# ratt-ru/tricolour

Hardware: AMD Instinct MI355X
Metric: Mvis/s flagged (bl x time x chan x corr) (higher is better)
Workload: dtype f32 data / f64 accumulators / u8 flags; 1 GPU; MeerKAT-64 slab: 252 of 2016 bl x 4 corr x 1024 time x 4096 chan per GPU (BASELINE configs[1] processed as HBM-resident baseline slabs), sum_threshold_flagger kwargs=stage1; params=stage1

## Files before the change

### tricolour_amd/csrc/kernels_boxline.hpp

```cpp
#pragma once

struct BoxDenom { float b, y; };
__device__ __forceinline__ float box_divide(float a, const BoxDenom dn, unsigned long long& okmask) {
    float q = a * dn.y;
    okmask &= __builtin_amdgcn_ballot_w64(__builtin_amdgcn_classf(q, 0x148));
    float r = __builtin_fmaf(-dn.b, q, a);
    q = __builtin_fmaf(r, dn.y, q);
    r = __builtin_fmaf(-dn.b, q, a);
    q = __builtin_fmaf(r, dn.y, q);
    return q;
}
__device__ __forceinline__ float box_divide_ieee(float a, const BoxDenom dn) { return a / dn.b; }
__device__ __forceinline__ float box_divide_checked(float a, const BoxDenom dn) {
    unsigned long long ok = ~0ull;
    const float q = box_divide(a, dn, ok);
    return ((ok >> (threadIdx.x & 63)) & 1ull) ? q : box_divide_ieee(a, dn);
}

template <int KS, typename V, typename A>
struct BoxLine {
    V R1[KS], R2[KS], R3[KS], R4[KS];
    A s1, s2, s3, s4;
    V o1, o2, o3;
    V old1, old2, old3, old4;
    __device__ __forceinline__ void init() {
#pragma unroll
        for (int k = 0; k < KS; k++) { R1[k] = 0; R2[k] = 0; R3[k] = 0; R4[k] = 0; }
        s1 = 0; s2 = 0; s3 = 0; s4 = 0;
        o1 = 0; o2 = 0; o3 = 0;
        old1 = 0; old2 = 0; old3 = 0; old4 = 0;
    }
};

template <int KS, typename V, typename A, bool HASL, bool FAST>
__device__ __forceinline__ float boxline_step(BoxLine<KS, V, A>& L, const int slot, const int m, const V xin,
                                              const int n, const int R2x, V* cell, const V* ncell, const int BT) {
    const V in4 = (FAST || m - 3 >= R2x) ? L.o3 : (V)0;
    const V in3 = L.o2;
    const V in2 = (FAST || m - 1 < n + R2x) ? L.o1 : (V)0;
    const V in1 = xin;
    V t1 = L.R1[slot], t2 = L.R2[slot], t3 = L.R3[slot], t4 = L.R4[slot];
    L.R1[slot] = in1; L.R2[slot] = in2; L.R3[slot] = in3; L.R4[slot] = in4;
    if (HASL) {
        const V n1 = ncell[0], n2 = ncell[BT], n3 = ncell[2 * (size_t)BT], n4 = ncell[3 * (size_t)BT];
        cell[0] = t1; cell[BT] = t2; cell[2 * (size_t)BT] = t3; cell[3 * (size_t)BT] = t4;
        t1 = L.old1; t2 = L.old2; t3 = L.old3; t4 = L.old4;
        L.old1 = n1; L.old2 = n2; L.old3 = n3; L.old4 = n4;
    }
    L.s4 += (A)in4;
    const float out = (float)L.s4;
    L.s4 -= (A)t4;
    L.s3 += (A)in3;
    L.o3 = (V)L.s3;
    L.s3 -= (A)t3;
    L.s2 += (A)in2;
    L.o2 = (V)L.s2;
    L.s2 -= (A)t2;
    L.s1 += (A)in1;
    L.o1 = (V)L.s1;
    L.s1 -= (A)t1;
    return out;
}

#ifndef BOXR_PF_SMALL
#define BOXR_PF_SMALL 16
#endif
#ifndef BOXR_PF_32
#define BOXR_PF_32 16
#endif
#ifndef BOXR_SCHED_EVERY
#define BOXR_SCHED_EVERY 1
#endif
#ifndef BOXR_WAVES_32
#define BOXR_WAVES_32 2
#endif
#ifndef BOXR_WAVES_16
#define BOXR_WAVES_16 3
#endif
#define BOXR_KS_MAX 80
#ifndef BOXR_WAVES_20
#define BOXR_WAVES_20 2
#endif
__host__ __device__ constexpr int boxr_pf(int ks) { return ks >= 64 ? 16 : (ks == 32 ? BOXR_PF_32 : (ks == 20 ? 20 : BOXR_PF_SMALL)); }
__host__ __device__ constexpr int boxr_waves(int ks) { return ks <= 16 ? BOXR_WAVES_16 : (ks == 20 ? BOXR_WAVES_20 : (ks <= 32 ? BOXR_WAVES_32 : 1)); }
#ifndef BOXR_WAVES_F32
#define BOXR_WAVES_F32 2
#endif
#ifndef BOXF_PF_SMALL
#define BOXF_PF_SMALL 16
#endif
__host__ __device__ constexpr int boxr_pf_f(int ks) { return ks <= 16 ? BOXF_PF_SMALL : boxr_pf(ks); }
#ifndef BOXR_WAVES_F16
#define BOXR_WAVES_F16 2
#endif
__host__ __device__ constexpr int boxr_waves_f(int ks) { return ks < 32 ? BOXR_WAVES_F16 : (ks == 32 ? BOXR_WAVES_F32 : 1); }
__host__ __device__ constexpr int boxr_lcm(int a, int b) {
    int x = a, y = b;
    while (y) { int t = x % y; x = y; y = t; }
    return a / x * b;
}

template <int KS, bool HASL, int IMG, bool PACKED, int PF>
__device__ __forceinline__ void boxt_body(const float* __restrict__ srcData, const uint8_t* __restrict__ srcFlags,
                                          float* __restrict__ dstImg, int n, int C, int r, float denom, size_t sws, size_t dws,
                                          const size_t win) {
    extern __shared__ float cf_ring[];
    const int c = blockIdx.x * 64 + threadIdx.x;
    if (c >= C) return;
    constexpr int BT = 64;
    const int R2x = 2 * r;
    const int d = R2x - KS;
    const unsigned rowb = (unsigned)C * 4u;
    const __amdgpu_buffer_rsrc_t drs = __builtin_amdgcn_make_buffer_rsrc(
        (void*)(srcData + win * sws), 0, (int)((unsigned)n * rowb), 0x00020000);
    const __amdgpu_buffer_rsrc_t frs = __builtin_amdgcn_make_buffer_rsrc(
        (void*)(srcFlags + win * sws), 0, PACKED ? (int)((unsigned)(n / 4) * rowb) : (int)((unsigned)n * (unsigned)C), 0x00020000);
    const __amdgpu_buffer_rsrc_t ors = __builtin_amdgcn_make_buffer_rsrc(
        (void*)(dstImg + win * dws), 0, (int)((unsigned)n * rowb), 0x00020000);
    const int coff = c * 4;
    float* ring = cf_ring + threadIdx.x;
    if (HASL)
        for (int k = 0; k < 4 * d; k++) ring[(size_t)k * BT] = 0.0f;
    const int total = n + 4 * r + 3;
    constexpr int UNR = boxr_lcm(KS, PF);
    constexpr bool SPLIT = KS <= 32;

    using V = typename std::conditional<IMG == 0, int, float>::type;
    using A = typename std::conditional<IMG == 0, int, double>::type;
    BoxLine<KS, V, A> L;
    L.init();
    V* cells = reinterpret_cast<V*>(ring);
    constexpr size_t BT4 = (size_t)4 * BT;
    int lslot = 0;
    float pre[PF];
    unsigned prew[PACKED ? PF / 4 : PF];
    auto issue = [&](int t0) {
        if (PACKED) {
#pragma unroll
            for (int q = 0; q < PF / 4; q++) {
                const int t = t0 + 4 * q;
                const unsigned w = (unsigned)__builtin_amdgcn_raw_buffer_load_b32(frs, coff, t < n ? (int)((unsigned)(t >> 2) * rowb) : 0, 0);
                prew[q] = (t < n) ? w : 0x01010101u;
            }
        } else {
#pragma unroll
            for (int u = 0; u < PF; u++) {
                const int t = t0 + u;
                const unsigned w = (unsigned)__builtin_amdgcn_raw_buffer_load_b8(frs, c, t < n ? (int)((unsigned)t * (unsigned)C) : 0, 0);
                prew[PACKED ? 0 : u] = (t < n) ? w : 1u;
            }
        }
        if (IMG == 1) {
#pragma unroll
            for (int u = 0; u < PF; u++)
                pre[u] = __builtin_bit_cast(float, __builtin_amdgcn_raw_buffer_load_b32(drs, coff, t0 + u < n ? (int)((unsigned)(t0 + u) * rowb) : 0, 0));
        }
    };
    auto store = [&](int i, float y) {
        __builtin_amdgcn_raw_buffer_store_b32(__builtin_bit_cast(unsigned, y), ors, coff, (int)((unsigned)i * rowb), 0);
    };
    issue(0);
    for (int mb = 0; mb < total; mb += UNR) {
#pragma unroll
        for (int b = 0; b < UNR / PF; b++) {
            const int m0 = mb + b * PF;
            if (m0 < total) {
                V cur[PF];
#pragma unroll
                for (int u = 0; u < PF; u++) {
                    const bool fl = PACKED ? ((prew[u >> 2] >> (8 * (u & 3))) & 0xFFu) != 0 : prew[PACKED ? 0 : u] != 0;
                    cur[u] = (IMG == 0) ? (fl ? (V)0 : (V)1) : (fl ? (V)0 : (V)pre[u]);
                }
                issue(m0 + PF);
                const bool fast = SPLIT && m0 >= 4 * r + 3 && m0 + PF <= n;
                if (fast) {
#pragma unroll
                    for (int u = 0; u < PF; u++) {
                        V* cell = cells + (size_t)lslot * BT4;
                        if (HASL) lslot = (lslot + 1 == d) ? 0 : lslot + 1;
                        const V* ncell = cells + (size_t)lslot * BT4;
                        const float out = boxline_step<KS, V, A, HASL, true>(L, (b * PF + u) % KS, m0 + u, cur[u], n, R2x, cell, ncell, BT);
                        store(m0 + u - 3 - 4 * r, out / denom);
                        if (BOXR_SCHED_EVERY > 0 && (u % (BOXR_SCHED_EVERY > 0 ? BOXR_SCHED_EVERY : 1)) == (BOXR_SCHED_EVERY > 0 ? BOXR_SCHED_EVERY : 1) - 1) __builtin_amdgcn_sched_barrier(0);
                    }
                } else {
#pragma unroll
                    for (int u = 0; u < PF; u++) {
                        V* cell = cells + (size_t)lslot * BT4;
                        if (HASL) lslot = (lslot + 1 == d) ? 0 : lslot + 1;
                        const V* ncell = cells + (size_t)lslot * BT4;
                        const float out = boxline_step<KS, V, A, HASL, false>(L, (b * PF + u) % KS, m0 + u, cur[u], n, R2x, cell, ncell, BT);
                        const int i = m0 + u - 3 - 4 * r;
                        if (i >= 0 && i < n) store(i, out / denom);
                        if (BOXR_SCHED_EVERY > 0 && (u % (BOXR_SCHED_EVERY > 0 ? BOXR_SCHED_EVERY : 1)) == (BOXR_SCHED_EVERY > 0 ? BOXR_SCHED_EVERY : 1) - 1) __builtin_amdgcn_sched_barrier(0);
                    }
                }
            }
        }
    }
}

template <int KS, bool HASL, int IMG>
__global__ void __launch_bounds__(64, boxr_waves(KS))
k_boxt(const float* __restrict__ srcData, const uint8_t* __restrict__ srcFlags,
       float* __restrict__ dstImg, int n, int C, int r, float denom, size_t sws, size_t dws) {
    boxt_body<KS, HASL, IMG, true, boxr_pf(KS)>(srcData, srcFlags, dstImg, n, C, r, denom, sws, dws, blockIdx.y);
}

__host__ __device__ constexpr int boxt_spec_pf(int ks) { return ks <= 16 ? 64 : (ks == 32 ? 32 : 16); }
template <int KS, bool HASL>
__global__ void __launch_bounds__(64, 1)
k_boxt_spec(const float* __restrict__ srcData, const uint8_t* __restrict__ srcFlags,
            float* __restrict__ dstW, float* __restrict__ dstO, int n, int C, int r, float denom) {
    if (blockIdx.y == 0) boxt_body<KS, HASL, 0, false, boxt_spec_pf(KS)>(srcData, srcFlags, dstW, n, C, r, denom, 0, 0, 0);
    else boxt_body<KS, HASL, 1, false, boxt_spec_pf(KS)>(srcData, srcFlags, dstO, n, C, r, denom, 0, 0, 0);
}

__host__ __device__ constexpr int boxf_ts(int pf) { return pf >= 32 ? 33 : 34; }
#ifndef BOXF_DOUBLE_STAGE
#define BOXF_DOUBLE_STAGE 1
#endif
__host__ __device__ constexpr int boxf_nsub(int ks) { return (BOXF_DOUBLE_STAGE && ks <= 16 && boxr_pf_f(ks) == 16) ? 2 : 1; }
#define BOXF_TS 34
#ifndef BOXF_STREAM_AUX
#define BOXF_STREAM_AUX 0
#endif
__host__ __device__ constexpr bool boxf_panel_ok(int ks, bool hasl) { return ks <= 8 || (ks == 16 && !hasl); }
template <int KS, bool HASL, int MODE, int WPS = boxr_waves_f(KS)>
__global__ void __launch_bounds__(64, WPS)
k_boxf(const float* __restrict__ srcW, unsigned img_gap,
       float* __restrict__ dstW, float* __restrict__ dstO, const float* __restrict__ data,
       int n, int C, int ld, int r, BoxDenom denom, size_t sws_img, size_t dws, size_t ws_data,
       uint8_t* __restrict__ nanflag, float* __restrict__ dstP, size_t pws) {
    extern __shared__ float cf_ring[];
    constexpr int PF = boxr_pf_f(KS);
    static_assert(MODE != 2 || (PF / 2) % 4 == 0, "panel output: groups of four positions per lane");
    constexpr int NSUB = boxf_nsub(KS);
    constexpr int PL = PF * NSUB;
    constexpr int UNR = boxr_lcm(boxr_lcm(KS, PF), PL);
    constexpr int BT = 64;
    constexpr int LPI = 32 / PL;
    constexpr int TS = boxf_ts(PL);
    const int lane = threadIdx.x;
    const int half = lane >> 5;
    const int hl = lane & 31;
    const int c0 = blockIdx.x * 32;
    const int c = c0 + hl;
    const bool colok = c < C;
    const size_t win = blockIdx.y;
    const int R2x = 2 * r;
    const int d = R2x - KS;
    float* ring = cf_ring + lane;
    float* tiles = cf_ring + (size_t)4 * d * BT;
    float* tile = tiles + (size_t)half * PL * TS;
    if (HASL)
        for (int k = 0; k < 4 * d; k++) ring[(size_t)k * BT] = 0.0f;

    const unsigned rowb = (unsigned)C * 4u;
    const __amdgpu_buffer_rsrc_t xrs = __builtin_amdgcn_make_buffer_rsrc(
        (void*)(data + win * ws_data), 0, (int)((unsigned)n * rowb), 0x00020000);
    const __amdgpu_buffer_rsrc_t ors = __builtin_amdgcn_make_buffer_rsrc(
        (void*)(dstO + win * dws), 0, (int)((unsigned)n * rowb), 0x00020000);
    const __amdgpu_buffer_rsrc_t wrs = __builtin_amdgcn_make_buffer_rsrc(
        (void*)(dstW + win * dws), 0, (int)((unsigned)n * rowb), 0x00020000);
    const bool panel = MODE == 2 && boxf_panel_ok(KS, HASL) && dstP != nullptr;
    const __amdgpu_buffer_rsrc_t prs = __builtin_amdgcn_make_buffer_rsrc(
        (void*)(panel ? dstP + win * pws : dstW), 0, panel ? (int)((unsigned)n * rowb) : 0, 0x00020000);

    const int s_pos = hl % PL;
    const int s_line0 = hl / PL;
    const unsigned ldb = (unsigned)ld * 4u;
    const __amdgpu_buffer_rsrc_t srs = __builtin_amdgcn_make_buffer_rsrc(
        (void*)(srcW + win * sws_img), 0, (int)((img_gap + (unsigned)C * (unsigned)ld) * 4u), 0x00020000);
    const int s_off = (int)((unsigned)s_line0 * ldb) + s_pos * 4 + (half ? (int)(img_gap * 4u) : 0);
    float pre[PL];
    auto issue = [&](int t0) {
        const int sbase = (int)((unsigned)c0 * ldb) + t0 * 4;
        if (t0 + PL <= n && c0 + 32 <= C) {
#pragma unroll
            for (int j = 0; j < PL; j++)
                pre[j] = __builtin_bit_cast(float, __builtin_amdgcn_raw_buffer_load_b32(srs, s_off, sbase + (int)((unsigned)(LPI * j) * ldb), 0));
        } else {
            const bool tok = t0 + s_pos < n;
#pragma unroll
            for (int j = 0; j < PL; j++) {
                const bool ok = tok && (c0 + LPI * j + s_line0 < C);
                const float v = __builtin_bit_cast(float, __builtin_amdgcn_raw_buffer_load_b32(srs, ok ? s_off + sbase + (int)((unsigned)(LPI * j) * ldb) : 0, 0, 0));
                pre[j] = ok ? v : 0.0f;
            }
        }
    };
    auto wave_sync = [] {
        __builtin_amdgcn_fence(__ATOMIC_RELEASE, "wavefront");
        __builtin_amdgcn_wave_barrier();
        __builtin_amdgcn_fence(__ATOMIC_ACQUIRE, "wavefront");
    };
    const int hrow = (PF / 2) * half;
    const int hoff = (colok ? c : 0) * 4 + (int)((unsigned)hrow * rowb);
    const float* eb = tiles + (size_t)hrow * TS + hl;
    float dpre[PF / 2];
    auto issue_data = [&](int m0, bool fast) {
        const int i0 = m0 - 3 - 4 * r;
        if (fast) {
#pragma unroll
            for (int k = 0; k < PF / 2; k++)
                dpre[k] = __builtin_bit_cast(float, __builtin_amdgcn_raw_buffer_load_b32(xrs, hoff, (int)((unsigned)(i0 + k) * rowb), BOXF_STREAM_AUX));
        } else {
#pragma unroll
            for (int k = 0; k < PF / 2; k++) {
                const int i = i0 + hrow + k;
                const bool ok = i >= 0 && i < n;
                const float v = __builtin_bit_cast(float, __builtin_amdgcn_raw_buffer_load_b32(xrs, ok ? (colok ? c : 0) * 4 + (int)((unsigned)i * rowb) : 0, 0, 0));
                dpre[k] = ok ? v : 0.0f;
            }
        }
    };

    BoxLine<KS, float, double> L;
    L.init();
    constexpr size_t BT4 = (size_t)4 * BT;
    int lslot = 0;
    const int total = n + 4 * r + 3;
    bool line_nan = false;
    issue(0);
    for (int mb = 0; mb < total; mb += UNR) {
#pragma unroll
        for (int b = 0; b < UNR / PF; b++) {
            const int m0 = mb + b * PF;
            if (m0 < total) {
                const int ro = (b % NSUB) * PF;
                if (b % NSUB == 0) {
                    wave_sync();
#pragma unroll
                    for (int j = 0; j < PL; j++) tile[s_pos * TS + LPI * j + s_line0] = pre[j];
                    wave_sync();
                    issue(m0 + PL);
                }
                const bool fast = m0 >= 4 * r + 3 && m0 + PF <= n;
                issue_data(m0, fast);
                float xin = tile[ro * TS + hl];
                if (fast) {
#pragma unroll
                    for (int u = 0; u < PF; u++) {
                        const float xnext = (u + 1 < PF) ? tile[(ro + u + 1) * TS + hl] : 0.0f;
                        float* cell = ring + (size_t)lslot * BT4;
                        if (HASL) lslot = (lslot + 1 == d) ? 0 : lslot + 1;
                        const float* ncell = ring + (size_t)lslot * BT4;
                        tile[(ro + u) * TS + hl] = boxline_step<KS, float, double, HASL, true>(L, (b * PF + u) % KS, m0 + u, xin, n, R2x, cell, ncell, BT);
                        xin = xnext;
                        if (BOXR_SCHED_EVERY > 0 && u % (BOXR_SCHED_EVERY > 0 ? BOXR_SCHED_EVERY : 1) == 0) __builtin_amdgcn_sched_barrier(0);
                    }
                } else {
#pragma unroll
                    for (int u = 0; u < PF; u++) {
                        const float xnext = (u + 1 < PF) ? tile[(ro + u + 1) * TS + hl] : 0.0f;
                        float* cell = ring + (size_t)lslot * BT4;
                        if (HASL) lslot = (lslot + 1 == d) ? 0 : lslot + 1;
                        const float* ncell = ring + (size_t)lslot * BT4;
                        tile[(ro + u) * TS + hl] = boxline_step<KS, float, double, HASL, false>(L, (b * PF + u) % KS, m0 + u, xin, n, R2x, cell, ncell, BT);
                        xin = xnext;
                        if (BOXR_SCHED_EVERY > 0 && u % (BOXR_SCHED_EVERY > 0 ? BOXR_SCHED_EVERY : 1) == 0) __builtin_amdgcn_sched_barrier(0);
                    }
                }
                if (m0 + PF - 1 - 3 - 4 * r >= 0) {
                    wave_sync();
                    const int i0 = m0 - 3 - 4 * r;
                    unsigned long long okmask = ~0ull, active = 0;
                    float res[MODE == 2 ? PF / 2 : 1];
                    auto finish = [&](auto ieee_tag) {
                        constexpr bool IEEE = decltype(ieee_tag)::value;
#pragma unroll
                        for (int k = 0; k < PF / 2; k++) {
                            const int i = i0 + hrow + k;
                            if ((fast || (i >= 0 && i < n)) && colok) {
                                if (!IEEE) active |= __builtin_amdgcn_ballot_w64(true);
                                const float wv = IEEE ? box_divide_ieee(eb[(ro + k) * TS], denom) : box_divide(eb[(ro + k) * TS], denom, okmask);
                                const float ov = IEEE ? box_divide_ieee(eb[(PL + ro + k) * TS], denom) : box_divide(eb[(PL + ro + k) * TS], denom, okmask);
                                const float bg = (wv == 0.0f) ? NAN : ov / wv;
                                const int vo = fast ? hoff : (c * 4 + (int)((unsigned)i * rowb));
                                const int so = fast ? (int)((unsigned)(i0 + k) * rowb) : 0;
                                if (MODE == 1) {
                                    __builtin_amdgcn_raw_buffer_store_b32(__builtin_bit_cast(unsigned, fabsf(dpre[k] - bg)), ors, vo, so, BOXF_STREAM_AUX);
                                } else {
                                    __builtin_amdgcn_raw_buffer_store_b32(__builtin_bit_cast(unsigned, bg), ors, vo, so, BOXF_STREAM_AUX);
                                    res[MODE == 2 ? k : 0] = dpre[k] - bg;
                                    __builtin_amdgcn_raw_buffer_store_b32(__builtin_bit_cast(unsigned, res[MODE == 2 ? k : 0]), wrs, vo, so, BOXF_STREAM_AUX);
                                    line_nan |= isnan(bg);
                                }
                            }
                            if (BOXR_SCHED_EVERY > 0) __builtin_amdgcn_sched_barrier(0);
                        }
                    };
                    finish(std::false_type{});
                    if ((okmask & active) != active) finish(std::true_type{});
                    if (MODE == 2 && panel && colok) {
                        auto paddr = [&](int i) { return (int)((((unsigned)(i >> 6) * (unsigned)C + (unsigned)c) << 8) + ((unsigned)(i & 63) << 2)); };
#pragma unroll
                        for (int g = 0; g < PF / 8; g++) {
                            const int ig = i0 + hrow + 4 * g;
                            if (fast && (ig & 63) <= 60) {
                                typedef unsigned u4 __attribute__((ext_vector_type(4)));
                                u4 y;
#pragma unroll
                                for (int e = 0; e < 4; e++) y[e] = __builtin_bit_cast(unsigned, res[MODE == 2 ? 4 * g + e : 0]);
                                __builtin_amdgcn_raw_buffer_store_b128(y, prs, paddr(ig), 0, BOXF_STREAM_AUX);
                            } else {
#pragma unroll
                                for (int e = 0; e < 4; e++)
                                    if (fast || (ig + e >= 0 && ig + e < n))
                                        __builtin_amdgcn_raw_buffer_store_b32(__builtin_bit_cast(unsigned, res[MODE == 2 ? 4 * g + e : 0]), prs, paddr(ig + e), 0, BOXF_STREAM_AUX);
                            }
                        }
                    }
                }
            }
        }
    }
    if (MODE == 2 && line_nan && colok) nanflag[win * (size_t)C + c] = 1;
}
```

### tricolour_amd/csrc/kernels_boxpipe.hpp

```cpp
#pragma once
#include <hip/hip_runtime.h>
#include <stdint.h>
#include <type_traits>

__host__ __device__ constexpr int boxp_lc(int r, int B) { return (2 * r + 2 * B + B - 1) / B * B; }
__host__ __device__ constexpr size_t boxp_lds_bytes(int r, int B) {
    return ((size_t)4 * (boxp_lc(r, B) + B) * 64 + (size_t)2 * B * 64) * 4;
}

template <int IMG, int B, int P>
__device__ __forceinline__ void boxp_body(const float* __restrict__ srcData, const uint8_t* __restrict__ srcFlags,
                                          float* __restrict__ dst, const int n, const int C, const int r, const float denom) {
    extern __shared__ float cf_ring[];
    using V = typename std::conditional<IMG == 0, int, float>::type;
    using A = typename std::conditional<IMG == 0, int, double>::type;
    constexpr int K = B / 4;
    static_assert(K == 2 || K == 4, "block length 8 or 16");
    constexpr unsigned OOB = 0x7ffffff0u;
    const int tid = threadIdx.x, lane = tid & 63;
    const int wave = __builtin_amdgcn_readfirstlane(tid >> 6);
    const int R2 = 2 * r;
    const int Lc = boxp_lc(r, B), LcP = Lc + B;
    V* bufs = reinterpret_cast<V*>(cf_ring);
    float* outb = cf_ring + (size_t)4 * LcP * 64;
    for (int k = tid; k < 4 * LcP * 64; k += 256) bufs[k] = 0;
    const int NB = (n + 4 * r + B - 1) / B;

    const int srow = tid / (64 / K);
    const int scol = (tid % (64 / K)) * K;
    const int gcol = blockIdx.x * 64 + scol;
    const bool colok = gcol < C;
    const __amdgpu_buffer_rsrc_t frs = __builtin_amdgcn_make_buffer_rsrc((void*)srcFlags, 0, (int)((unsigned)n * (unsigned)C), 0x00020000);
    const __amdgpu_buffer_rsrc_t ors = __builtin_amdgcn_make_buffer_rsrc((void*)dst, 0, (int)((unsigned)n * (unsigned)C * 4u), 0x00020000);

    unsigned pref[P];
    float prex[IMG == 1 ? P : 1][K];
    auto issue = [&](int blk, int q) {
        const int t = blk * B + srow;
        const unsigned e = (colok && t < n) ? (unsigned)t * (unsigned)C + (unsigned)gcol : OOB;
        if (K == 4) pref[q] = (unsigned)__builtin_amdgcn_raw_buffer_load_b32(frs, (int)e, 0, 0);
        else pref[q] = (unsigned)__builtin_amdgcn_raw_buffer_load_b16(frs, (int)e, 0, 0);
        if (IMG == 1) {
            const float* a = srcData + ((colok && t < n) ? (size_t)e : (size_t)0);
            if (K == 4) {
                const float4 v = *reinterpret_cast<const float4*>(a);
                prex[q][0] = v.x; prex[q][1] = v.y; prex[q][K - 2] = v.z; prex[q][K - 1] = v.w;
            } else {
                const float2 v = *reinterpret_cast<const float2*>(a);
                prex[q][0] = v.x; prex[q][1] = v.y;
            }
        }
    };
    auto staged = [&](int blk, int q, int k) -> V {
        const int t = blk * B + srow;
        const bool fl = t >= n || !colok || ((pref[q] >> (8 * k)) & 0xFFu) != 0;
        if (IMG == 0) return fl ? (V)0 : (V)1;
        return fl ? (V)0 : (V)prex[IMG == 1 ? q : 0][k];
    };
#pragma unroll
    for (int q = 0; q < P; q++) issue(q, q);

    int lpin = 0;
    int pin = 0, pold = Lc - R2;
    A acc = 0;
    V* bin = bufs + (size_t)wave * LcP * 64 + lane;
    V* bout = bufs + (size_t)(wave + 1) * LcP * 64 + lane;
    const int keep_lo = wave == 2 ? R2 : 0;
    const int keep_hi = wave == 0 ? n + R2 : 0x7fffffff;
    __syncthreads();

    for (int j0 = 0; j0 < NB + 5; j0 += P) {
#pragma unroll
        for (int q = 0; q < P; q++) {
            const int j = j0 + q;
            if (j < NB) {
                V* p = bufs + ((size_t)lpin + srow) * 64 + scol;
                V sv[K];
#pragma unroll
                for (int k = 0; k < K; k++) sv[k] = staged(j, q, k);
#pragma unroll
                for (int k = 0; k < K; k++) p[k] = sv[k];
                if (lpin == 0) {
#pragma unroll
                    for (int k = 0; k < K; k++) p[(size_t)Lc * 64 + k] = sv[k];
                }
                lpin = (lpin + B == Lc) ? 0 : lpin + B;
            }
            issue(j + P, q);
            const int b = j - wave - 1;
            if (b >= 0 && b < NB) {
                const V* pi = bin + (size_t)pin * 64;
                const V* po = bin + (size_t)pold * 64;
                V xin[B], xold[B];
#pragma unroll
                for (int u = 0; u < B; u++) { xin[u] = pi[u * 64]; xold[u] = po[u * 64]; }
                const int t0 = b * B;
                if (wave == 3) {
                    float* ob = outb + (size_t)(b & 1) * B * 64 + lane;
#pragma unroll
                    for (int u = 0; u < B; u++) {
                        acc += (A)xin[u];
                        ob[u * 64] = (float)acc;
                        acc -= (A)xold[u];
                    }
                } else {
                    V* po2 = bout + (size_t)pin * 64;
                    const bool whole = t0 >= keep_lo && t0 + B <= keep_hi;
                    V o[B];
#pragma unroll
                    for (int u = 0; u < B; u++) {
                        acc += (A)xin[u];
                        o[u] = (V)acc;
                        acc -= (A)xold[u];
                    }
                    if (whole) {
#pragma unroll
                        for (int u = 0; u < B; u++) po2[u * 64] = o[u];
                    } else {
#pragma unroll
                        for (int u = 0; u < B; u++) {
                            o[u] = (t0 + u >= keep_lo && t0 + u < keep_hi) ? o[u] : (V)0;
                            po2[u * 64] = o[u];
                        }
                    }
                    if (pin == 0) {
#pragma unroll
                        for (int u = 0; u < B; u++) po2[(Lc + u) * 64] = o[u];
                    }
                }
                pin = (pin + B == Lc) ? 0 : pin + B;
                pold = (pold + B >= Lc) ? pold + B - Lc : pold + B;
            }
            {
                const int bs = j - 5;
                const int i = bs * B + srow - 4 * r;
                const bool ok = bs >= 0 && bs < NB && i >= 0 && i < n && colok;
                const float* ob = outb + ((size_t)(bs & 1) * B + srow) * 64 + scol;
                const unsigned eb = ok ? ((unsigned)i * (unsigned)C + (unsigned)gcol) * 4u : OOB;
                if (K == 4) {
                    const float4 v = *reinterpret_cast<const float4*>(ob);
                    typedef unsigned u4 __attribute__((ext_vector_type(4)));
                    u4 y;
                    y[0] = __builtin_bit_cast(unsigned, v.x / denom); y[1] = __builtin_bit_cast(unsigned, v.y / denom);
                    y[2] = __builtin_bit_cast(unsigned, v.z / denom); y[3] = __builtin_bit_cast(unsigned, v.w / denom);
                    __builtin_amdgcn_raw_buffer_store_b128(y, ors, (int)eb, 0, 0);
                } else {
                    const float2 v = *reinterpret_cast<const float2*>(ob);
                    typedef unsigned u2 __attribute__((ext_vector_type(2)));
                    u2 y;
                    y[0] = __builtin_bit_cast(unsigned, v.x / denom); y[1] = __builtin_bit_cast(unsigned, v.y / denom);
                    __builtin_amdgcn_raw_buffer_store_b64(y, ors, (int)eb, 0, 0);
                }
            }
            __syncthreads();
        }
    }
}

template <int B, int P>
__global__ void __launch_bounds__(256, 1)
k_boxp_spec(const float* __restrict__ srcData, const uint8_t* __restrict__ srcFlags,
            float* __restrict__ dstW, float* __restrict__ dstO, int n, int C, int r, float denom) {
    if (blockIdx.y == 0) boxp_body<0, B, P>(srcData, srcFlags, dstW, n, C, r, denom);
    else boxp_body<1, B, P>(srcData, srcFlags, dstO, n, C, r, denom);
}

__host__ __device__ constexpr size_t boxq_lds_bytes(int B, int NF = 3) { return (size_t)(4 * (NF + 1) * B * 64 + 2 * B * 64) * 4; }
#define BOXQ_LDS_BYTES boxq_lds_bytes(16)
__host__ __device__ constexpr int boxq_prefetch(int ks) { return ks == 48 || ks == 96 ? 6 : (ks == 80 ? 5 : 4); }
#ifndef BOXQ_ABLATE
#define BOXQ_ABLATE 0
#endif
__host__ __device__ constexpr int boxq_lcm(int a, int b) {
    int x = a, y = b;
    while (y) { int t = x % y; x = y; y = t; }
    return a / x * b;
}

__host__ __device__ constexpr int boxq_prefetch8(int nblk) {
    return nblk == 6 ? 3 : (nblk == 8 ? 4 : (nblk == 9 ? 3 : (nblk == 10 ? 2 : (nblk == 12 ? 4 : nblk))));
}

template <int IMG, int KS, int P, int B = 16, int NF = 3>
__device__ __forceinline__ void boxq_body(const float* __restrict__ srcData, const uint8_t* __restrict__ srcFlags,
                                          float* __restrict__ dst, const int n, const int C, const int r, const BoxDenom denom,
                                          const size_t sws, const size_t dws, const size_t win) {
    using V = typename std::conditional<IMG == 0, int, float>::type;
    using A = typename std::conditional<IMG == 0, int, double>::type;
    constexpr int PPT = B / 4;
    constexpr int NBLK = KS / B;
    constexpr int U = boxq_lcm(NBLK, P);
    constexpr unsigned OOB = 0x7ffffff0u;
    static_assert(KS % B == 0 && KS >= B, "register part: whole blocks");
    static_assert(B == 8 || B == 16, "block length");
    extern __shared__ float cf_ring[];
    typedef V FifoT[(NF + 1) * B][64];
    typedef float OutT[B][64];
    FifoT* fifo = reinterpret_cast<FifoT*>(cf_ring);
    OutT* outb = reinterpret_cast<OutT*>(cf_ring + 4 * (NF + 1) * B * 64);
    const int tid = threadIdx.x, lane = tid & 63;
    const int wave = __builtin_amdgcn_readfirstlane(tid >> 6);
    const int R2 = 2 * r;
    const int d = R2 - KS;
    const int c = blockIdx.x * 64 + lane;
    const bool colok = c < C;
    const int NB = (n + 4 * r + B - 1) / B;
    const unsigned rowb = (unsigned)C * 4u;
    const __amdgpu_buffer_rsrc_t frs = __builtin_amdgcn_make_buffer_rsrc((void*)(srcFlags + win * sws), 0, (int)((unsigned)(n / 4) * rowb), 0x00020000);
    const __amdgpu_buffer_rsrc_t drs = __builtin_amdgcn_make_buffer_rsrc((void*)(srcData + win * sws), 0, (int)((unsigned)n * rowb), 0x00020000);
    const __amdgpu_buffer_rsrc_t ors = __builtin_amdgcn_make_buffer_rsrc((void*)(dst + win * dws), 0, (int)((unsigned)n * rowb), 0x00020000);
    const unsigned coff = (unsigned)c * 4u;
    for (int k = tid; k < 4 * (NF + 1) * B * 64; k += 256) reinterpret_cast<V*>(cf_ring)[k] = 0;

    unsigned pref[P];
    float prex[IMG == 1 ? P : 1][PPT];
    auto issue = [&](int blk, int q) {
        const int t = blk * B + PPT * wave;
        const bool ok = colok && t < n;
        pref[q] = (unsigned)__builtin_amdgcn_raw_buffer_load_b32(frs, (int)(ok ? (unsigned)(t >> 2) * rowb + coff : OOB), 0, 0);
        if (IMG == 1) {
#pragma unroll
            for (int k = 0; k < PPT; k++)
                prex[q][k] = __builtin_bit_cast(float, __builtin_amdgcn_raw_buffer_load_b32(drs, (int)(ok ? (unsigned)(t + k) * rowb + coff : OOB), 0, 0));
        }
    };
#pragma unroll
    for (int q = 0; q < P; q++) issue(q, q);

    V R[KS];
#pragma unroll
    for (int k = 0; k < KS; k++) R[k] = 0;
    A acc = 0;
    int lslot = 0;
    int slot = 0, s0 = NF * B - d;
    if (s0 >= NF * B) s0 -= NF * B;
    const int keep_lo = wave == 2 ? R2 : 0;
    const int keep_hi = wave == 0 ? n + R2 : 0x7fffffff;
    __syncthreads();

    for (int j0 = 0; j0 < NB + 5; j0 += U) {
#pragma unroll
        for (int qq = 0; qq < U; qq++) {
            const int j = j0 + qq;
            const int q = qq % P;
            const int sb = (qq % NBLK) * B;
#if !(BOXQ_ABLATE & 4)
            {
                const int t = j * B + PPT * wave;
                const bool tin = colok && t < n;
                const unsigned fw = PPT == 4 ? pref[q] : pref[q] >> (16 * (wave & 1));
                V sv[PPT];
#pragma unroll
                for (int k = 0; k < PPT; k++) {
                    const bool fl = !tin || ((fw >> (8 * k)) & 0xFFu) != 0;
                    if (IMG == 0) sv[k] = fl ? (V)0 : (V)1;
                    else sv[k] = fl ? (V)0 : (V)prex[IMG == 1 ? q : 0][k];
                }
                V* p = &fifo[0][lslot * B + PPT * wave][lane];
#pragma unroll
                for (int k = 0; k < PPT; k++) p[k * 64] = sv[k];
                if (lslot == 0) {
#pragma unroll
                    for (int k = 0; k < PPT; k++) p[(NF * B + k) * 64] = sv[k];
                }
                lslot = lslot == NF - 1 ? 0 : lslot + 1;
            }
            issue(j + P, q);
#endif
            const int b = j - wave - 1;
#if !(BOXQ_ABLATE & 2)
            if (b >= 0 && b < NB) {
                const int t0 = b * B;
                const V* pi = &fifo[wave][slot * B][lane];
                const V* pd = &fifo[wave][s0][lane];
                V xin[B], xdel[B], o[B];
#pragma unroll
                for (int u = 0; u < B; u++) { xin[u] = pi[u * 64]; xdel[u] = pd[u * 64]; }
#pragma unroll
                for (int u = 0; u < B; u++) {
                    const V old = R[sb + u];
                    R[sb + u] = xdel[u];
                    acc += (A)xin[u];
                    o[u] = (V)acc;
                    acc -= (A)old;
                }
                if (wave == 3) {
                    float* ob = &outb[b & 1][0][lane];
#pragma unroll
                    for (int u = 0; u < B; u++) ob[u * 64] = (float)o[u];
                } else {
                    const bool whole = t0 >= keep_lo && t0 + B <= keep_hi;
                    V* po = &fifo[wave + 1][slot * B][lane];
                    if (whole) {
#pragma unroll
                        for (int u = 0; u < B; u++) po[u * 64] = o[u];
                    } else {
#pragma unroll
                        for (int u = 0; u < B; u++) {
                            o[u] = (t0 + u >= keep_lo && t0 + u < keep_hi) ? o[u] : (V)0;
                            po[u * 64] = o[u];
                        }
                    }
                    if (slot == 0) {
#pragma unroll
                        for (int u = 0; u < B; u++) po[(NF * B + u) * 64] = o[u];
                    }
                }
                slot = slot == NF - 1 ? 0 : slot + 1;
                s0 = s0 + B >= NF * B ? s0 + B - NF * B : s0 + B;
            }
#endif
#if !(BOXQ_ABLATE & 1)
            {
                const int bs = j - 5;
                const int i0 = bs * B + PPT * wave - 4 * r;
                const float* ob = &outb[bs & 1][PPT * wave][lane];
                float a[PPT], y[PPT];
                unsigned long long okm = ~0ull;
#pragma unroll
                for (int k = 0; k < PPT; k++) { a[k] = ob[k * 64]; y[k] = box_divide(a[k], denom, okm); }
                if (okm != ~0ull) {
                    TRI_KEEP_BRANCH();
#pragma unroll
                    for (int k = 0; k < PPT; k++) y[k] = box_divide_ieee(a[k], denom);
                }
#pragma unroll
                for (int k = 0; k < PPT; k++) {
                    const int i = i0 + k;
                    const bool ok = bs >= 0 && bs < NB && i >= 0 && i < n && colok;
                    __builtin_amdgcn_raw_buffer_store_b32(__builtin_bit_cast(unsigned, y[k]), ors, (int)(ok ? (unsigned)i * rowb + coff : OOB), 0, 0);
                }
            }
#endif
            __syncthreads();
        }
    }
}

template <int KS, int IMG, int B = 16>
__global__ void __launch_bounds__(256, B == 8 ? 4 : 2)
k_boxq(const float* __restrict__ srcData, const uint8_t* __restrict__ srcFlags, float* __restrict__ dstImg,
       int n, int C, int r, BoxDenom denom, size_t sws, size_t dws) {
    boxq_body<IMG, KS, B == 8 ? boxq_prefetch8(KS / 8) : boxq_prefetch(KS), B>(srcData, srcFlags, dstImg, n, C, r, denom, sws, dws, blockIdx.y);
}
template <int KS, int IMG>
__global__ void __launch_bounds__(256, 3)
k_boxq_deep(const float* __restrict__ srcData, const uint8_t* __restrict__ srcFlags, float* __restrict__ dstImg,
            int n, int C, int r, BoxDenom denom, size_t sws, size_t dws) {
    boxq_body<IMG, KS, boxq_prefetch8(KS / 8), 8, 4>(srcData, srcFlags, dstImg, n, C, r, denom, sws, dws, blockIdx.y);
}

#ifndef BOXQF_LW
#define BOXQF_LW 64
#endif
#ifndef BOXQF_DBL
#define BOXQF_DBL 1
#endif
#ifndef BOXQF_PAIR
#define BOXQF_PAIR 1
#endif
#ifndef BOXQF_ABLATE_BARRIER
#define BOXQF_ABLATE_BARRIER 0
#endif
__host__ __device__ constexpr bool boxqf_dbl(int KS, int B) { return BOXQF_DBL && B == 8 && (KS / B) % 2 == 0; }
__host__ __device__ constexpr int boxqf_prefetch2(int nblk) { return nblk == 6 ? 3 : (nblk == 10 || nblk == 2 ? 1 : 2); }
__host__ __device__ constexpr size_t boxqf_lds_floats(int B, bool dbl) { return (size_t)(2 * ((dbl ? 5 : 4) + 3 * 4) * B * BOXQF_LW + 2 * 2 * B * BOXQF_LW); }
__host__ __device__ constexpr size_t boxqf_lds_bytes(int B, bool dbl = false) { return boxqf_lds_floats(B, dbl) * 4; }
#define BOXQF_LDS_BYTES boxqf_lds_bytes(16)
#ifndef BOXQF_P10
#define BOXQF_P10 2
#endif
__host__ __device__ constexpr int boxqf_prefetch8(int nblk) {
    return nblk == 6 ? 3 : (nblk == 8 ? 4 : (nblk == 9 ? 3 : (nblk == 10 ? BOXQF_P10 : (nblk == 12 ? 4 : nblk))));
}
#ifndef BOXQF_MINW8
#define BOXQF_MINW8 4
#endif
template <int KS, int MODE, int B = 16>
__global__ void __launch_bounds__(512, B == 8 ? BOXQF_MINW8 : 1)
k_boxqf(const float* __restrict__ srcW, unsigned img_gap, float* __restrict__ dstW, float* __restrict__ dstO,
        const float* __restrict__ data, int n, int C, int ld, int r, BoxDenom denom, size_t sws_img, size_t dws,
        size_t ws_data, uint8_t* __restrict__ nanflag) {
    constexpr int PP = B / 4;
    constexpr int FN = B / 8;
    constexpr int NBLK = KS / B;
    constexpr bool DBL = boxqf_dbl(KS, B);
    constexpr int P2 = boxqf_prefetch2(NBLK);
    constexpr int P = DBL ? 2 * P2 : (B == 8 ? boxqf_prefetch8(NBLK) : boxq_prefetch(KS));
    static_assert(KS % B == 0, "register part: whole blocks");
    static_assert(B == 8 || B == 16, "block length");
    constexpr int U = boxq_lcm(NBLK, P);
    static_assert(!DBL || U % 2 == 0, "double-block staging: an even number of iterations per trip");
    constexpr unsigned OOB = 0x7ffffff0u;
    extern __shared__ float cf_ring[];
    constexpr int LW = BOXQF_LW;
    constexpr int NF1 = DBL ? 4 : 3;
    constexpr int F1 = (NF1 + 1) * B * LW, FN3 = 4 * B * LW;
    typedef float OutT[B][LW];
    auto fifo_of = [&](int image, int stage) -> float* {
        return stage == 0 ? cf_ring + image * F1 : cf_ring + 2 * F1 + (image * 3 + stage - 1) * FN3;
    };
    OutT* outb = reinterpret_cast<OutT*>(cf_ring + 2 * F1 + 6 * FN3);
    constexpr bool PAIR = BOXQF_PAIR && B == 8 && KS <= 40;
    auto ld2 = [&](const float* fifo, int row) -> float2 {
        if (PAIR) return *reinterpret_cast<const float2*>(fifo + ((size_t)(row >> 1) * LW + (threadIdx.x & 63)) * 2);
        const float* p = fifo + (size_t)row * LW + (threadIdx.x & 63);
        return make_float2(p[0], p[LW]);
    };
    auto st2 = [&](float* fifo, int row, int line, float a, float b2) {
        if (PAIR) { *reinterpret_cast<float2*>(fifo + ((size_t)(row >> 1) * LW + line) * 2) = make_float2(a, b2); return; }
        float* p = fifo + (size_t)row * LW + line;
        p[0] = a;
        p[LW] = b2;
    };
    const int tid = threadIdx.x, lane = tid & 63;
    const int wave = __builtin_amdgcn_readfirstlane(tid >> 6);
    const int img = wave >> 2, st = wave & 3;
    const size_t win = blockIdx.y;
    const int c0 = blockIdx.x * 64;
    const int R2 = 2 * r;
    const int d = R2 - KS;
    const int NB = (n + 4 * r + B - 1) / B;
    for (int k = tid; k < 2 * F1 + 6 * FN3; k += 512) cf_ring[k] = 0.0f;

    const int s_line = (tid & 255) >> 2, s_q = tid & 3;
    const bool s_lok = c0 + s_line < C;
    const float* s_base = srcW + win * sws_img + (size_t)(img ? img_gap : 0u) + (size_t)(s_lok ? c0 + s_line : 0) * ld;
    float pre[DBL ? P2 : P][DBL ? 4 : PP];
    auto issue = [&](int blk, int q) {
        if (DBL) {
            const int p = blk * 16 + 4 * s_q;
            const float4 v = *reinterpret_cast<const float4*>(s_base + (p < n ? p : 0));
            pre[q][0] = v.x; pre[q][1] = v.y; pre[q][DBL ? 2 : 0] = v.z; pre[q][DBL ? 3 : 0] = v.w;
            return;
        }
        const int p = blk * B + PP * s_q;
        if (PP == 4) {
            const float4 v = *reinterpret_cast<const float4*>(s_base + (p < n ? p : 0));
            pre[q][0] = v.x; pre[q][1] = v.y; pre[q][PP - 2] = v.z; pre[q][PP - 1] = v.w;
        } else {
            const float2 v = *reinterpret_cast<const float2*>(s_base + (p < n ? p : 0));
            pre[q][0] = v.x; pre[q][1] = v.y;
        }
    };
    const int f_u = tid >> 6;
    const int c = c0 + lane;
    const bool colok = c < C;
    const unsigned rowb = (unsigned)C * 4u;
    const unsigned coff = (unsigned)c * 4u;
    const __amdgpu_buffer_rsrc_t xrs = __builtin_amdgcn_make_buffer_rsrc((void*)(data + win * ws_data), 0, (int)((unsigned)n * rowb), 0x00020000);
    const __amdgpu_buffer_rsrc_t ors = __builtin_amdgcn_make_buffer_rsrc((void*)(dstO + win * dws), 0, (int)((unsigned)n * rowb), 0x00020000);
    const __amdgpu_buffer_rsrc_t wrs = __builtin_amdgcn_make_buffer_rsrc((void*)(dstW + win * dws), 0, (int)((unsigned)n * rowb), 0x00020000);
    float dpre[P][FN];
    auto issue_data = [&](int blk, int q) {
#pragma unroll
        for (int h = 0; h < FN; h++) {
            const int i = blk * B + f_u + 8 * h - 4 * r;
            const bool ok = blk >= 0 && i >= 0 && i < n && colok;
            dpre[q][h] = __builtin_bit_cast(float, __builtin_amdgcn_raw_buffer_load_b32(xrs, (int)(ok ? (unsigned)i * rowb + coff : OOB), 0, 0));
        }
    };
#pragma unroll
    for (int q = 0; q < P; q++) { if (!DBL || q < P2) issue(q, q); issue_data(q - 5, q); }

    float R[KS];
#pragma unroll
    for (int k = 0; k < KS; k++) R[k] = 0.0f;
    double acc = 0.0;
    int lslot = 0;
    const int nf = st == 0 ? NF1 : 3;
    int slot = (nf * 8 - st - 1) % nf, s0 = (nf * B * 8 - (st + 1) * B - d) % (nf * B);
    int oslot = (3 * 8 - st - 1) % 3;
    float* const fin = fifo_of(img, st);
    float* const fout = fifo_of(img, st < 3 ? st + 1 : 3);
    const int keep_lo = st == 2 ? R2 : 0;
    const int keep_hi = st == 0 ? n + R2 : 0x7fffffff;
    bool line_nan = false;
    __syncthreads();

    for (int j0 = 0; j0 < NB + 5; j0 += U) {
#pragma unroll
        for (int qq = 0; qq < U; qq++) {
            const int j = j0 + qq;
            const int q = qq % P;
            const int sb = (qq % NBLK) * B;
            if (DBL) {
                if (qq % 2 == 0) {
                    const int q2 = (qq / 2) % P2;
                    const int p = j * B + 4 * s_q;
                    const bool ok = s_lok && p < n;
                    float* pf = fifo_of(img, 0);
                    const int r0 = lslot * B + 4 * s_q;
                    const float v0 = ok ? pre[q2][0] : 0.0f, v1 = ok ? pre[q2][1] : 0.0f, v2 = ok ? pre[q2][DBL ? 2 : 0] : 0.0f, v3 = ok ? pre[q2][DBL ? 3 : 0] : 0.0f;
                    st2(pf, r0, s_line, v0, v1);
                    st2(pf, r0 + 2, s_line, v2, v3);
                    if (lslot == 0 && s_q < 2) {
                        st2(pf, NF1 * B + r0, s_line, v0, v1);
                        st2(pf, NF1 * B + r0 + 2, s_line, v2, v3);
                    }
                    lslot = lslot == 0 ? 2 : 0;
                    issue(j / 2 + P2, q2);
                }
            } else {
                const int p = j * B + PP * s_q;
                const bool ok = s_lok && p < n;
                float* pf = fifo_of(img, 0);
                const int r0 = lslot * B + PP * s_q;
#pragma unroll
                for (int k = 0; k < PP; k += 2) {
                    const float va = ok ? pre[DBL ? 0 : q][k] : 0.0f, vb = ok ? pre[DBL ? 0 : q][k + 1] : 0.0f;
                    st2(pf, r0 + k, s_line, va, vb);
                    if (lslot == 0) st2(pf, 3 * B + r0 + k, s_line, va, vb);
                }
                lslot = lslot == 2 ? 0 : lslot + 1;
            }
            if (!DBL) issue(j + P, q);
            const int b = j - st - 1;
            {
                const int t0 = b * B;
                float xin[B], xdel[B], o[B];
#pragma unroll
                for (int u = 0; u < B; u += 2) {
                    const float2 a = ld2(fin, slot * B + u), d2 = ld2(fin, s0 + u);
                    xin[u] = a.x; xin[u + 1] = a.y; xdel[u] = d2.x; xdel[u + 1] = d2.y;
                }
#pragma unroll
                for (int u = 0; u < B; u++) {
                    const float old = R[sb + u];
                    R[sb + u] = xdel[u];
                    acc += (double)xin[u];
                    o[u] = (float)acc;
                    acc -= (double)old;
                }
                if (st == 3) {
                    float* ob = &outb[img * 2 + (b & 1)][0][lane];
#pragma unroll
                    for (int u = 0; u < B; u++) ob[u * LW] = o[u];
                } else {
                    const bool whole = t0 >= keep_lo && t0 + B <= keep_hi && b >= 0;
                    if (!whole) {
#pragma unroll
                        for (int u = 0; u < B; u++) o[u] = (t0 + u >= keep_lo && t0 + u < keep_hi) ? o[u] : 0.0f;
                    }
#pragma unroll
                    for (int u = 0; u < B; u += 2) st2(fout, oslot * B + u, lane, o[u], o[u + 1]);
                    if (oslot == 0) {
#pragma unroll
                        for (int u = 0; u < B; u += 2) st2(fout, 3 * B + u, lane, o[u], o[u + 1]);
                    }
                }
                slot = slot == nf - 1 ? 0 : slot + 1;
                oslot = oslot == 2 ? 0 : oslot + 1;
                s0 = s0 + B >= nf * B ? s0 + B - nf * B : s0 + B;
            }
            {
                const int bs = j - 5;
                float wq[FN], oq[FN], a0[FN], a1[FN];
                unsigned long long okm = ~0ull;
#pragma unroll
                for (int h = 0; h < FN; h++) {
                    a0[h] = outb[bs & 1][f_u + 8 * h][lane];
                    a1[h] = outb[2 + (bs & 1)][f_u + 8 * h][lane];
                    wq[h] = box_divide(a0[h], denom, okm);
                    oq[h] = box_divide(a1[h], denom, okm);
                }
                if (okm != ~0ull) {
                    TRI_KEEP_BRANCH();
#pragma unroll
                    for (int h = 0; h < FN; h++) { wq[h] = box_divide_ieee(a0[h], denom); oq[h] = box_divide_ieee(a1[h], denom); }
                }
#pragma unroll
                for (int h = 0; h < FN; h++) {
                    const int i = bs * B + f_u + 8 * h - 4 * r;
                    const bool ok = bs >= 0 && bs < NB && i >= 0 && i < n && colok;
                    const unsigned off = ok ? (unsigned)i * rowb + coff : OOB;
                    const float bg = (wq[h] == 0.0f) ? NAN : oq[h] / wq[h];
                    const float dv = dpre[q][h];
                    if (MODE == 1) {
                        __builtin_amdgcn_raw_buffer_store_b32(__builtin_bit_cast(unsigned, fabsf(dv - bg)), ors, (int)off, 0, 0);
                    } else {
                        __builtin_amdgcn_raw_buffer_store_b32(__builtin_bit_cast(unsigned, bg), ors, (int)off, 0, 0);
                        __builtin_amdgcn_raw_buffer_store_b32(__builtin_bit_cast(unsigned, dv - bg), wrs, (int)off, 0, 0);
                        line_nan |= ok && isnan(bg);
                    }
                }
            }
            issue_data(j + P - 5, q);
#if BOXQF_ABLATE_BARRIER
            asm volatile("" ::: "memory");
            __builtin_amdgcn_sched_barrier(0);
#else
            __syncthreads();
#endif
        }
    }
    if (MODE == 2 && line_nan) nanflag[win * (size_t)C + c] = 1;
}
```

### tricolour_amd/csrc/kernels_boxweight.hpp

```cpp
#pragma once
#include <type_traits>

__host__ __device__ constexpr int boxw_unroll(int r2) { return r2 % 4 == 0 ? r2 : 2 * r2; }
__host__ __device__ constexpr int boxw_regs(int r2) { return (r2 + 31) / 32 + (r2 + 3) / 4 + (r2 + 1) / 2 + r2 + 56; }
__host__ __device__ constexpr int boxw_waves(int r2) { return boxw_regs(r2) <= 128 ? 4 : (boxw_regs(r2) <= 168 ? 3 : 2); }
#ifndef BOXW_SCHED_EVERY
#define BOXW_SCHED_EVERY 2
#endif
#ifndef BOXW_PREFETCH
#define BOXW_PREFETCH 4
#endif

__device__ __forceinline__ float boxw_divide(float a, const BoxDenom dn) {
    float q = a * dn.y;
    float r = __builtin_fmaf(-dn.b, q, a);
    q = __builtin_fmaf(r, dn.y, q);
    r = __builtin_fmaf(-dn.b, q, a);
    q = __builtin_fmaf(r, dn.y, q);
    return q;
}

#define BOXW_LSHL_ADD(acc, x, SH) asm("v_lshl_add_u32 %0, %1, %2, %0" : "+v"(acc) : "v"(x), "n"(SH))

template <int R2>
__global__ void __launch_bounds__(64, boxw_waves(R2))
k_boxw(const uint8_t* __restrict__ srcFlags, float* __restrict__ dstW, int n, int C, BoxDenom denom, size_t sws, size_t dws) {
    constexpr int N1 = (R2 + 31) / 32, N2 = (R2 + 3) / 4, N3 = (R2 + 1) / 2;
    constexpr int P = BOXW_PREFETCH;
    constexpr unsigned OOB = 0x7ffffff0u;
    static_assert(R2 % 2 == 0 && R2 >= 8 && R2 <= 214, "2r even, stage sums within a byte / a halfword / int32");
    const int lane = threadIdx.x;
    const size_t win = blockIdx.y;
    const int c = blockIdx.x * 64 + lane;
    const bool colok = c < C;
    const unsigned rowb = (unsigned)C * 4u;
    const unsigned coff = colok ? (unsigned)c * 4u : OOB;
    const __amdgpu_buffer_rsrc_t frs = __builtin_amdgcn_make_buffer_rsrc((void*)(srcFlags + win * sws), 0, (int)((unsigned)(n / 4) * rowb), 0x00020000);
    const __amdgpu_buffer_rsrc_t ors = __builtin_amdgcn_make_buffer_rsrc((void*)(dstW + win * dws), 0, (int)((unsigned)n * rowb), 0x00020000);

    unsigned D1[N1], D2[N2], D3[N3], D4[R2];
#pragma unroll
    for (int k = 0; k < N1; k++) D1[k] = 0;
#pragma unroll
    for (int k = 0; k < N2; k++) D2[k] = 0;
#pragma unroll
    for (int k = 0; k < N3; k++) D3[k] = 0;
#pragma unroll
    for (int k = 0; k < R2; k++) D4[k] = 0;
    unsigned s1 = 0, s2 = 0, s3 = 0, s4 = 0;

    unsigned pf[P];
    const int ngrp = n / 4;
#pragma unroll
    for (int q = 0; q < P; q++)
        pf[q] = (unsigned)__builtin_amdgcn_raw_buffer_load_b32(frs, (int)((colok && q < ngrp) ? (unsigned)q * rowb + coff : OOB), 0, 0);

    const int nsteps = n + 2 * R2;
    unsigned wb = 0;
    auto block = [&](auto phase, const int t0, const unsigned head) {
        constexpr int PH = decltype(phase)::value;
#pragma unroll
        for (int u = 0; u < R2; u++) {
            const int t = t0 + u;
            const int slot = u;
            if ((u + PH) % 4 == 0) {
                const unsigned fw = pf[0];
#pragma unroll
                for (int q = 0; q + 1 < P; q++) pf[q] = pf[q + 1];
                const int g = (t >> 2) + P;
                pf[P - 1] = (unsigned)__builtin_amdgcn_raw_buffer_load_b32(frs, (int)(g < ngrp ? (unsigned)g * rowb + coff : OOB), 0, 0);
                const unsigned nz = ((((fw & 0x7f7f7f7fu) + 0x7f7f7f7fu) | fw) >> 7) & 0x01010101u;
                wb = t < n ? (nz ^ 0x01010101u) : 0u;
            }
            const unsigned in1 = (wb >> (8 * ((u + PH) % 4))) & 1u;
            const unsigned old1 = (D1[slot >> 5] >> (slot & 31)) & 1u;
            const unsigned o1 = s1 + in1;
            const unsigned d1 = in1 - old1;
            s1 = o1 - old1;
            BOXW_LSHL_ADD(D1[slot >> 5], d1, slot & 31);
            const unsigned old2 = (D2[slot >> 2] >> (8 * (slot & 3))) & 0xffu;
            const unsigned o2 = s2 + o1;
            s2 = o2 - old2;
            const unsigned d2 = o1 - old2;
            BOXW_LSHL_ADD(D2[slot >> 2], d2, 8 * (slot & 3));
            const unsigned old3 = (D3[slot >> 1] >> (16 * (slot & 1))) & 0xffffu;
            const unsigned o3 = s3 + o2;
            s3 = o3 - old3;
            const unsigned d3 = o2 - old3;
            BOXW_LSHL_ADD(D3[slot >> 1], d3, 16 * (slot & 1));
            const unsigned in4 = o3 & head;
            const unsigned old4 = D4[slot];
            D4[slot] = in4;
            const unsigned o4 = s4 + in4;
            s4 = o4 - old4;
            const int i = t - 2 * R2;
            const bool rowok = (unsigned)i < (unsigned)n;
            const float y = boxw_divide((float)o4, denom);
            __builtin_amdgcn_raw_buffer_store_b32(__builtin_bit_cast(unsigned, y), ors, (int)(rowok ? coff : OOB), (int)(rowok ? (unsigned)i * rowb : 0u), 0);
            if (BOXW_SCHED_EVERY > 0 && (u + 1) % BOXW_SCHED_EVERY == 0) __builtin_amdgcn_sched_barrier(0);
        }
    };
    for (int t0 = 0; t0 < nsteps; t0 += boxw_unroll(R2)) {
        block(std::integral_constant<int, 0>{}, t0, t0 == 0 ? 0u : ~0u);
        if constexpr (R2 % 4 != 0) block(std::integral_constant<int, 2>{}, t0 + R2, ~0u);
    }
}
```

### tricolour_amd/csrc/tricolour_amd.hip

```cpp
#include <unordered_set>
#include "tri_common.hpp"
#include "kernels_elementwise.hpp"
#include "kernels_median.hpp"
#include "kernels_reject.hpp"
#include "kernels_reject_tile.hpp"
#include "kernels_boxfilter.hpp"
#include "kernels_boxline.hpp"
#include "kernels_boxpipe.hpp"
#include "kernels_boxweight.hpp"
#include "kernels_boxexact.hpp"
#include "kernels_sumthreshold.hpp"
#include "kernels_scan.hpp"
#include "kernels_sir.hpp"
#include "kernels_linerms.hpp"

namespace {

static hipError_t lds_optin(const void* fn, hipFuncAttribute attr, int value) {
    thread_local std::unordered_set<uint64_t> done;
    int dev = 0;
    hipError_t e = hipGetDevice(&dev);
    if (e != hipSuccess) return e;
    const uint64_t key = (uint64_t)(uintptr_t)fn * 64u + (uint64_t)(dev & 63);
    if (done.count(key)) return hipSuccess;
// ... 184 lines not shown
    ws->colcnt = b.get<int>(W * F);
    ws->nanmask = b.get<uint16_t>(W * N / 16 + 8);
    ws->itab = b.get<int>(3 * W * (size_t)cdiv(Fa, INTERP_SEG) * std::max<size_t>(T, 1));
    ws->med = b.get<double>(W * std::max(Fa, T * G));
    size_t PS = (size_t)pl.PF;
    ws->sdata = b.get<float>(Fa * W);
    ws->sw = b.get<float>(PS * W);
    ws->so = b.get<float>(PS * W);
    ws->sres = b.get<float>(Fa * W);
    ws->sflags = b.get<uint8_t>(Fa * W);
    ws->sbgf = b.get<uint8_t>(Fa * W);
    ws->sout = b.get<uint8_t>(Fa * W);
    ws->srows = b.get<uint8_t>(Fa * W);
    ws->srowsf = b.get<float>(Fa * W);
    ws->srowsu = b.get<uint8_t>(Fa * W);
    ws->smed = b.get<double>(W * G);
    size_t thrT = W * Fa, thrF = W * T * G;
    size_t ringn = std::max(thrT * (size_t)pl.swT.ringtot, thrF * (size_t)pl.swF.ringtot);
    size_t accn = std::max(thrT * (size_t)pl.swT.acccap, thrF * (size_t)pl.swF.acccap);
    ws->ring = b.get<double>(ringn);
    ws->acc = b.get<uint8_t>(accn);
    ws->total = b.off;
}

static inline dim3 grid1(size_t n, size_t W) { return dim3((unsigned)cdiv((int64_t)n, 256), (unsigned)W, 1); }

}

__global__ void k_tables(ChunkTab ct, int T, int Fa, int64_t* chunk_ends, int64_t* tends,
                         int64_t* segC_start, int64_t* segC_len, int64_t* segB_start,
                         int64_t* segB_len, int64_t* segT_start, int64_t* segT_len,
                         int* chunk_of) {
    int i = blockIdx.x * blockDim.x + threadIdx.x;
    int G = ct.n - 1;
    if (i <= G) chunk_ends[i] = ct.ends[i];
    if (i < G) {
        segC_start[i] = ct.ends[i];
        segC_len[i] = ct.ends[i + 1] - ct.ends[i];
        segB_start[i] = ct.ends[i] * T;
        segB_len[i] = (ct.ends[i + 1] - ct.ends[i]) * T;
    }
    if (i == 0) { tends[0] = 0; tends[1] = T; segT_start[0] = 0; segT_len[0] = T; }
    if (i < Fa) {
        int g = 0;
        while (g < G - 1 && !(i >= ct.ends[g] && i < ct.ends[g + 1])) g++;
        chunk_of[i] = g;
    }
}

__global__ void k_gather_col_f32(const float* __restrict__ a, float* __restrict__ out, int L, int C, int col) {
    int i = blockIdx.x * blockDim.x + threadIdx.x;
    if (i < L) out[i] = a[(size_t)i * C + col];
}
__global__ void k_gather_col_u8(const uint8_t* __restrict__ a, uint8_t* __restrict__ out, int L, int C, int col) {
    int i = blockIdx.x * blockDim.x + threadIdx.x;
    if (i < L) out[i] = a[(size_t)i * C + col];
}
__global__ void k_normalise_flags(const uint8_t* __restrict__ a, uint8_t* __restrict__ b, size_t n) {
    size_t i = (size_t)blockIdx.x * blockDim.x + threadIdx.x;
    if (i < n) b[i] = a[i] ? 1 : 0;
}

extern "C" size_t tri_workspace_bytes(int64_t batch_windows, int64_t ntime, int64_t nchan,
                                      const tri_params* p) {
    Plan pl;
    if (!p || batch_windows <= 0 || make_plan(ntime, nchan, p, &pl) != TRI_OK) return 0;
    Ws ws;
    carve(pl, batch_windows, nullptr, 0, true, &ws);
    return ws.total;
}

extern "C" int tri_prepare_params(int64_t ntime, int64_t nchan, double outlier_nsigma,
                                  const double* windows_time, int64_t n_windows_time,
                                  const double* windows_freq, int64_t n_windows_freq,
                                  double background_reject, int64_t background_iterations,
                                  double spike_width_time, double spike_width_freq,
                                  int64_t time_extend, int64_t freq_extend, int64_t freq_chunks,
                                  int64_t average_freq, double flag_all_time_frac,
                                  double flag_all_freq_frac, double rho,
                                  int64_t num_major_iterations, int64_t* chunk_ends_buf,
                                  int64_t chunk_cap, tri_params* out) {
    if (!out || !chunk_ends_buf) return set_err(TRI_EINVAL, "NULL output");
    if (ntime <= 0 || nchan <= 0) return set_err(TRI_EINVAL, "empty window");
    if (average_freq < 1) return set_err(TRI_EINVAL, "average_freq must be >= 1");
    if (freq_chunks < 1) return set_err(TRI_EINVAL, "freq_chunks must be >= 1");
    if (chunk_cap < freq_chunks + 1) return set_err(TRI_EINVAL, "chunk_ends_buf too small");
    if (n_windows_time > TRI_MAX_WINDOWS || n_windows_freq > TRI_MAX_WINDOWS || n_windows_time < 0 || n_windows_freq < 0)
        return set_err(TRI_EINVAL, "at most %d windows per axis", TRI_MAX_WINDOWS);
    memset(out, 0, sizeof(*out));
    int64_t fa = (nchan + average_freq - 1) / average_freq;
    std::vector<int64_t> wf;
    for (int64_t i = 0; i < n_windows_freq; i++) {
        float v = std::ceil((float)windows_freq[i]) / (float)average_freq;
        wf.push_back((int64_t)v);
    }
    std::sort(wf.begin(), wf.end());
    wf.erase(std::unique(wf.begin(), wf.end()), wf.end());
    double step = (double)fa / (double)freq_chunks;
    for (int64_t i = 0; i <= freq_chunks; i++) chunk_ends_buf[i] = (int64_t)((double)i * step);
    chunk_ends_buf[freq_chunks] = fa;
    out->n_windows_time = 0;
    for (int64_t i = 0; i < n_windows_time; i++)
        if (windows_time[i] <= (double)ntime) out->windows_time[out->n_windows_time++] = (int64_t)windows_time[i];
    out->n_windows_freq = 0;
    for (size_t i = 0; i < wf.size(); i++)
        if (wf[i] <= fa) out->windows_freq[out->n_windows_freq++] = wf[i];
    for (int64_t i = 0; i < out->n_windows_freq; i++)
        if (out->windows_freq[i] <= 0)
            return set_err(TRI_EINVAL, "windows_freq / average_freq produced a window of size %lld; the reference fails here (operands could not be broadcast together, flagging.py:663)", (long long)out->windows_freq[i]);
    for (int64_t i = 0; i < out->n_windows_time; i++)
        if (out->windows_time[i] <= 0) return set_err(TRI_EINVAL, "windows_time must be positive");
    out->outlier_nsigma = outlier_nsigma;
    out->background_reject = background_reject;
    out->background_iterations = background_iterations;
    out->spike_width_time = spike_width_time;
    out->spike_width_freq = spike_width_freq;
    out->time_extend = time_extend;
    out->freq_extend = freq_extend;
    out->n_chunk_ends = freq_chunks + 1;
    out->chunk_ends = chunk_ends_buf;
    out->average_freq = average_freq;
    out->flag_all_time_frac = flag_all_time_frac;
    out->flag_all_freq_frac = flag_all_freq_frac;
    out->rho = rho;
    out->num_major_iterations = num_major_iterations;
    return TRI_OK;
}

namespace {

struct Debug {
    float* f32;
    uint8_t* u8;
};

struct Run {
    hipStream_t st;
    Plan pl;
    Ws ws;
    const tri_params* p;
    int64_t Wb;
    Debug* dbg;
    bool ampl_cached = false;
    const uint8_t* data_mask = nullptr;
    size_t data_mask_ws = 0;
};

bool st_use_fused(const StWin& sw) {
    static const bool force_generic = is1(getenv("TRI_ST_GENERIC"));
    if (force_generic) return false;
    return sw.nw == 4 && sw.w[0] == 1 && sw.w[1] == 2 && sw.w[2] == 4 && sw.w[3] == 8;
}

bool st_use_mask(int L, int C) {
    static const bool force_register = is1(getenv("TRI_ST_REGISTER"));
    return !force_register && (uint64_t)L * (uint64_t)C * 4u < (1ull << 31);
}

static bool median_no_predict() { static const bool v = is1(getenv("TRI_MEDIAN_NO_PREDICT")); return v; }

static bool median_takes_extra_flags(int64_t max_len) { return max_len <= 64 * MW_K; }

struct MedianJob {
    const float* data = nullptr; const uint8_t* flags = nullptr; double* med = nullptr;
    size_t WSd = 0, WSf = 0, RS = 0, ES = 1;
    const int64_t* seg_start = nullptr; const int64_t* seg_len = nullptr;
    int R = 0, G = 0;
    int64_t W = 0, max_len = 0;
    bool vec_ok = false;
    bool rows_aligned = false;
    bool segs_aligned = false;
    const uint8_t* flags2 = nullptr; const uint8_t* colflags = nullptr; size_t WScol = 0; int panel_rows = 0;
    unsigned* gcand = nullptr; size_t cand_ws = 0; unsigned cand_cap = 0;
};

enum class MedianKernel {
    Wave8, Wave8Vec,
    Wave16, Wave16Vec,
    Select, SelectVec,
    TwoPass, TwoPassVec,
    TwoPassVecLong,
};

template <int KS, bool VEC, int SPW>
static void median_wave(hipStream_t st, const MedianJob& j) {
    hipLaunchKernelGGL((k_median_wave<KS, VEC, SPW>), dim3((unsigned)cdiv((int64_t)cdiv((int64_t)j.R, SPW) * j.G, 4), (unsigned)j.W),
                       dim3(256), 0, st, j.data, j.flags, j.med, j.WSd, j.WSf, j.RS, j.ES, j.seg_start, j.seg_len, j.R, j.G,
                       j.flags2, j.colflags, j.WScol, j.panel_rows);
}
template <bool VEC>
static void median_select(hipStream_t st, const MedianJob& j) {
    hipLaunchKernelGGL(k_median<VEC>, dim3((unsigned)(j.R * j.G), (unsigned)j.W), dim3(256), 0, st,
                       j.data, j.flags, j.med, j.WSd, j.WSf, j.RS, j.ES, j.seg_start, j.seg_len, j.R, j.G);
}
template <bool VEC, int UNR = MED2_UNROLL>
static void median_two_pass(hipStream_t st, const MedianJob& j) {
    hipLaunchKernelGGL((k_median2<VEC, false, UNR>), dim3((unsigned)(j.R * j.G), (unsigned)j.W), dim3(256), 0, st,
                       j.data, j.flags, j.med, j.WSd, j.WSf, j.RS, j.ES, j.seg_start, j.seg_len, j.R, j.G, j.gcand, j.cand_ws, j.cand_cap);
}

static void launch_median_kernel(hipStream_t st, MedianKernel k, bool seg_per_wave, const MedianJob& j) {
    switch (k) {
    case MedianKernel::Wave8: seg_per_wave ? median_wave<8, false, 1>(st, j) : median_wave<8, false, MW_SPW>(st, j); break;
    case MedianKernel::Wave8Vec: seg_per_wave ? median_wave<8, true, 1>(st, j) : median_wave<8, true, MW_SPW>(st, j); break;
    case MedianKernel::Wave16: seg_per_wave ? median_wave<MW_K, false, 1>(st, j) : median_wave<MW_K, false, MW_SPW16>(st, j); break;
    case MedianKernel::Wave16Vec: seg_per_wave ? median_wave<MW_K, true, 1>(st, j) : median_wave<MW_K, true, MW_SPW16>(st, j); break;
    case MedianKernel::Select: median_select<false>(st, j); break;
    case MedianKernel::SelectVec: median_select<true>(st, j); break;
    case MedianKernel::TwoPass: median_two_pass<false>(st, j); break;
    case MedianKernel::TwoPassVec: median_two_pass<true>(st, j); break;
    case MedianKernel::TwoPassVecLong: median_two_pass<true, 16>(st, j); break;
    }
}

int launch_median(const Run& r, MedianJob j) {
    const int R = j.R, G = j.G;
    const int64_t W = j.W, max_len = j.max_len;
    if ((int64_t)R * G <= 0 || W <= 0) return TRI_OK;
    if (j.panel_rows > 0 && !(j.ES == 1 && j.RS % 64 == 0 && j.rows_aligned && max_len + (j.segs_aligned ? 0 : 3) <= 64 * MW_K &&
                              j.WSd % 4 == 0 && j.WSf % 4 == 0 && ((uintptr_t)j.data % 16 == 0) && ((uintptr_t)j.flags % 4 == 0)))
        return set_err(TRI_EUNSUPPORTED, "panel images need wave-sized segments of 64-column aligned rows");
    if ((j.flags2 || j.colflags) && (max_len > 64 * MW_K || (j.colflags && j.ES != 1) || ((uintptr_t)j.flags2 % 4 != 0) ||
                                     ((uintptr_t)j.colflags % 4 != 0) || j.WScol % 4 != 0))
        return set_err(TRI_EUNSUPPORTED, "extra flag sources need wave-sized segments of contiguous, 4-byte aligned rows");
    if ((int64_t)R * G > 0x7FFFFFFF || W > 65535) return set_err(TRI_EUNSUPPORTED, "median grid too large");
    const bool row4 = j.ES == 1 && j.RS % 4 == 0 && j.WSd % 4 == 0 && j.WSf % 4 == 0 &&
                      ((uintptr_t)j.data % 16 == 0) && ((uintptr_t)j.flags % 4 == 0) && j.rows_aligned &&
                      (uint64_t)j.RS * (uint64_t)std::max(R, j.panel_rows) * 4u < (1ull << 32);
    if (j.panel_rows > 0 && !row4) return set_err(TRI_EUNSUPPORTED, "panel images of 4 GB or more per window");
    const int64_t slack = j.segs_aligned ? 0 : 3;
    static const bool wave_old = is1(getenv("TRI_MEDIAN_WAVE_OLD"));
    MedianKernel k;
    if (max_len + slack <= 64 * 8 && row4) k = MedianKernel::Wave8Vec;
    else if (max_len <= 64 * 8 && j.panel_rows == 0) k = MedianKernel::Wave8;
    else if (max_len + slack <= 64 * MW_K && row4) k = MedianKernel::Wave16Vec;
    else if (max_len <= 64 * MW_K) k = MedianKernel::Wave16;
    else {
        static const bool three = is1(getenv("TRI_MEDIAN_3PASS"));
        if (three) k = j.vec_ok ? MedianKernel::SelectVec : MedianKernel::Select;
        else {
            if (median_no_predict() || j.cand_cap < max_len || j.cand_ws % 4 != 0 || j.cand_cap % 4 != 0 || ((uintptr_t)j.gcand % 16 != 0)) {
                j.gcand = nullptr; j.cand_ws = 0; j.cand_cap = 0;
            }
            if ((j.vec_ok || row4) && (int64_t)R * G * W < 1536 && max_len >= (int64_t)1 << 20) k = MedianKernel::TwoPassVecLong;
            else k = (j.vec_ok || row4) ? MedianKernel::TwoPassVec : MedianKernel::TwoPass;
        }
    }
    launch_median_kernel(r.st, k, wave_old, j);
    LAUNCHCHK();
    return TRI_OK;
}

#ifndef LDS_R_MAX
#define LDS_R_MAX 15
#endif
#ifndef LANE4_R_MAX
#define LANE4_R_MAX 160
#endif
static bool filter_no_lane4() { static const bool v = is1(getenv("TRI_FILTER_NO_LANE4")); return v; }
int colfilter_lds_block(int rad, int C) {
    static const bool disabled = is1(getenv("TRI_FILTER_MULTIPASS"));
    if (disabled || rad <= 0) return 0;
    if (filter_no_lane4()) {
        int bt = rad <= 10 ? 256 : (rad <= 20 ? 128 : (rad <= 40 ? 64 : 0));
        while (bt > 64 && bt / 2 >= C) bt /= 2;
        return bt;
    }
    if (rad <= LDS_R_MAX) {
        int bt = rad <= 10 ? 256 : 128;
        while (bt > 64 && bt / 2 >= C) bt /= 2;
        return bt;
    }
    return rad <= LANE4_R_MAX ? 64 : 0;
}
inline bool colfilter_use_lane4(int rad) { return !filter_no_lane4() && rad > LDS_R_MAX && rad <= LANE4_R_MAX; }

#ifndef BOXR_MAX_LDS_SLOTS
#define BOXR_MAX_LDS_SLOTS 60
#endif
thread_local int g_boxr_override = -1;
int boxr_pick_ks(int rad) {
    static const bool env_off = is1(getenv("TRI_FILTER_NO_REGRING"));
    const bool off = g_boxr_override >= 0 ? g_boxr_override == 0 : env_off;
    if (off || rad < 4 || rad > 107) return 0;
    const int ks = 2 * rad >= 80 ? 80 : (2 * rad >= 64 ? 64 : (2 * rad >= 32 ? 32 : (2 * rad >= 16 ? 16 : 8)));
    return 2 * rad - ks <= BOXR_MAX_LDS_SLOTS ? ks : 0;
}

#ifndef BOXT_MIN_2R
#define BOXT_MIN_2R 32
#endif
#ifndef BOXT_EXACT20
#define BOXT_EXACT20 1
#endif
int boxr_pick_ks_t(int rad) {
    if (BOXT_EXACT20 && 2 * rad == 20) return boxr_pick_ks(rad) > 0 ? 20 : 0;
    return 2 * rad >= BOXT_MIN_2R ? boxr_pick_ks(rad) : 0;
}
int boxr_pick_ks_f(int rad) {
    static const bool off = is1(getenv("TRI_FILTER_NO_REGRING_F"));
    return off ? 0 : boxr_pick_ks(rad);
}

thread_local int g_boxw_override = -1;
static bool boxw_usable(int rad, int n, int C) {
    static const bool off = is1(getenv("TRI_FILTER_NO_BOXW"));
    if (g_boxw_override == 0 || (off && g_boxw_override < 0)) return false;
    return 2 * rad >= 20 && 2 * rad <= 110 && n % 4 == 0 && (uint64_t)n * (uint64_t)C * 4u < (1ull << 31);
}
template <int R2>
int launch_boxw_r2(const Run& r, const uint8_t* srcFlags, float* dstW, int n, int C, float denom, size_t sws, size_t dws, int64_t W) {
    dim3 grid((unsigned)cdiv(C, 64), (unsigned)W);
    hipLaunchKernelGGL((k_boxw<R2>), grid, dim3(64), 0, r.st, srcFlags, dstW, n, C, box_reciprocal(denom), sws, dws);
    LAUNCHCHK();
    return TRI_OK;
}
int launch_boxw(const Run& r, const uint8_t* srcFlags, float* dstW, int n, int C, int rad, float denom, size_t sws, size_t dws, int64_t W) {
#define BOXW_CASE(R2) case R2: return launch_boxw_r2<R2>(r, srcFlags, dstW, n, C, denom, sws, dws, W);
#define BOXW_CASE5(A) BOXW_CASE(A) BOXW_CASE(A + 2) BOXW_CASE(A + 4) BOXW_CASE(A + 6) BOXW_CASE(A + 8)
    switch (2 * rad) {
        BOXW_CASE5(20) BOXW_CASE5(30) BOXW_CASE5(40) BOXW_CASE5(50) BOXW_CASE5(60) BOXW_CASE5(70) BOXW_CASE5(80) BOXW_CASE5(90) BOXW_CASE5(100)
        BOXW_CASE(110)
    }
#undef BOXW_CASE5
#undef BOXW_CASE
    return set_err(TRI_EINVAL, "no integer weight filter for radius %d", rad);
}

template <int KS>
int launch_boxt_ks(const Run& r, const float* srcData, const uint8_t* srcFlags, float* dstW, float* dstO,
                   int n, int C, int rad, float denom, size_t sws, size_t dws, int64_t W) {
    const int d = 2 * rad - KS;
    const size_t lds = (size_t)4 * d * 64 * sizeof(float);
    dim3 grid((unsigned)cdiv(C, 64), (unsigned)W);
    HIPCHK(lds_optin_all(160 * 1024, &k_boxt<KS, true, 0>, &k_boxt<KS, true, 1>));
    const bool wk = boxw_usable(rad, n, C);
    if (wk) { const int rc = launch_boxw(r, srcFlags, dstW, n, C, rad, denom, sws, dws, W); if (rc) return rc; }
    if (d > 0) {
        if (!wk) hipLaunchKernelGGL((k_boxt<KS, true, 0>), grid, dim3(64), lds, r.st, srcData, srcFlags, dstW, n, C, rad, denom, sws, dws);
        hipLaunchKernelGGL((k_boxt<KS, true, 1>), grid, dim3(64), lds, r.st, srcData, srcFlags, dstO, n, C, rad, denom, sws, dws);
    } else {
        if (!wk) hipLaunchKernelGGL((k_boxt<KS, false, 0>), grid, dim3(64), 0, r.st, srcData, srcFlags, dstW, n, C, rad, denom, sws, dws);
        hipLaunchKernelGGL((k_boxt<KS, false, 1>), grid, dim3(64), 0, r.st, srcData, srcFlags, dstO, n, C, rad, denom, sws, dws);
    }
    LAUNCHCHK();
    return TRI_OK;
}

template <int KS>
int launch_boxt_spec_ks(const Run& r, const float* srcData, const uint8_t* srcFlags, float* dstW, float* dstO,
                        int n, int C, int rad, float denom) {
    const int d = 2 * rad - KS;
    const size_t lds = (size_t)4 * d * 64 * sizeof(float);
    dim3 grid((unsigned)cdiv(C, 64), 2);
    HIPCHK(lds_optin_all(160 * 1024, &k_boxt_spec<KS, true>));
    if (d > 0) hipLaunchKernelGGL((k_boxt_spec<KS, true>), grid, dim3(64), lds, r.st, srcData, srcFlags, dstW, dstO, n, C, rad, denom);
    else hipLaunchKernelGGL((k_boxt_spec<KS, false>), grid, dim3(64), 0, r.st, srcData, srcFlags, dstW, dstO, n, C, rad, denom);
    LAUNCHCHK();
    return TRI_OK;
}

int launch_boxt_spec(const Run& r, int ks, const float* srcData, const uint8_t* srcFlags, float* dstW, float* dstO,
                     int n, int C, int rad, float denom) {
    switch (ks) {
        case 8: return launch_boxt_spec_ks<8>(r, srcData, srcFlags, dstW, dstO, n, C, rad, denom);
        case 16: return launch_boxt_spec_ks<16>(r, srcData, srcFlags, dstW, dstO, n, C, rad, denom);
        case 32: return launch_boxt_spec_ks<32>(r, srcData, srcFlags, dstW, dstO, n, C, rad, denom);
        case 64: return launch_boxt_spec_ks<64>(r, srcData, srcFlags, dstW, dstO, n, C, rad, denom);
        case 80: return launch_boxt_spec_ks<80>(r, srcData, srcFlags, dstW, dstO, n, C, rad, denom);
    }
    return set_err(TRI_EINVAL, "no register-ring kernel for %d slots", ks);
}

static thread_local int g_boxp_override = -1;
static int boxp_pick_block(int rad, int C) {
    static const bool off = is1(getenv("TRI_SPEC_NO_PIPE"));
    if (g_boxp_override == 0 || (off && g_boxp_override < 0)) return 0;
    if (g_boxp_override != 8 && 2 * rad >= 16 && C % 4 == 0 && boxp_lds_bytes(rad, 16) <= 160 * 1024) return 16;
    if (g_boxp_override == 16) return 0;
    if (2 * rad >= 8 && C % 2 == 0 && boxp_lds_bytes(rad, 8) <= 160 * 1024) return 8;
    return 0;
}

template <int B, int P>
int launch_boxp_spec_b(const Run& r, const float* srcData, const uint8_t* srcFlags, float* dstW, float* dstO,
                       int n, int C, int rad, float denom) {
    HIPCHK(lds_optin_all(160 * 1024, &k_boxp_spec<B, P>));
    dim3 grid((unsigned)cdiv(C, 64), 2);
    hipLaunchKernelGGL((k_boxp_spec<B, P>), grid, dim3(256), boxp_lds_bytes(rad, B), r.st, srcData, srcFlags, dstW, dstO, n, C, rad, denom);
    LAUNCHCHK();
    return TRI_OK;
}

#ifndef BOXQ_MIN_2R
#define BOXQ_MIN_2R 56
#endif
thread_local int g_boxq_override = -1;
static int boxq_pick_ks(int rad) {
    static const bool off = is1(getenv("TRI_FILTER_NO_PIPE_T"));
    if (g_boxq_override == 0 || (off && g_boxq_override < 0)) return 0;
    const int ks = 2 * rad / 16 * 16;
    return (ks >= 16 && ks <= 96) ? ks : 0;
}

template <int KS, int B = 16>
int launch_boxq_ks(const Run& r, const float* srcData, const uint8_t* srcFlags, float* dstW, float* dstO,
                   int n, int C, int rad, float denom, size_t sws, size_t dws, int64_t W) {
    HIPCHK(lds_optin_all(160 * 1024, &k_boxq<KS, 0, B>, &k_boxq<KS, 1, B>));
    dim3 grid((unsigned)cdiv(C, 64), (unsigned)W);
    const BoxDenom dn = box_reciprocal(denom);
    if (boxw_usable(rad, n, C)) { const int rc = launch_boxw(r, srcFlags, dstW, n, C, rad, denom, sws, dws, W); if (rc) return rc; }
    else hipLaunchKernelGGL((k_boxq<KS, 0, B>), grid, dim3(256), boxq_lds_bytes(B), r.st, srcData, srcFlags, dstW, n, C, rad, dn, sws, dws);
    hipLaunchKernelGGL((k_boxq<KS, 1, B>), grid, dim3(256), boxq_lds_bytes(B), r.st, srcData, srcFlags, dstO, n, C, rad, dn, sws, dws);
    LAUNCHCHK();
    return TRI_OK;
}

#ifndef BOXQ_B8_MIN_2R
#define BOXQ_B8_MIN_2R 32
#endif
#ifndef BOXQ_B8_MAX2R
#define BOXQ_B8_MAX2R 88
#endif
thread_local int g_boxq_b8_override = -1;
static int boxq_pick_ks8(int rad) {
    static const int b8 = [] { const char* e = getenv("TRI_FILTER_PIPE_T_B8"); return e ? atoi(e) : 1; }();
    if (!b8 || g_boxq_b8_override == 0 || 2 * rad < BOXQ_B8_MIN_2R || 2 * rad >= BOXQ_B8_MAX2R) return 0;
    return 2 * rad / 8 * 8;
}

template <int KS>
int launch_boxq_deep(const Run& r, const float* srcData, const uint8_t* srcFlags, float* dstW, float* dstO,
                     int n, int C, int rad, float denom, size_t sws, size_t dws, int64_t W) {
    HIPCHK(lds_optin_all(160 * 1024, &k_boxq_deep<KS, 0>, &k_boxq_deep<KS, 1>));
    dim3 grid((unsigned)cdiv(C, 64), (unsigned)W);
    const BoxDenom dn = box_reciprocal(denom);
    if (boxw_usable(rad, n, C)) { const int rc = launch_boxw(r, srcFlags, dstW, n, C, rad, denom, sws, dws, W); if (rc) return rc; }
    else hipLaunchKernelGGL((k_boxq_deep<KS, 0>), grid, dim3(256), boxq_lds_bytes(8, 4), r.st, srcData, srcFlags, dstW, n, C, rad, dn, sws, dws);
    hipLaunchKernelGGL((k_boxq_deep<KS, 1>), grid, dim3(256), boxq_lds_bytes(8, 4), r.st, srcData, srcFlags, dstO, n, C, rad, dn, sws, dws);
    LAUNCHCHK();
    return TRI_OK;
}
#ifndef BOXQ_DEEP
#define BOXQ_DEEP 1
#endif

int launch_boxq(const Run& r, int ks, const float* srcData, const uint8_t* srcFlags, float* dstW, float* dstO,
                int n, int C, int rad, float denom, size_t sws, size_t dws, int64_t W) {
    if (BOXQ_DEEP && boxq_pick_ks8(40) > 0) {
        if (2 * rad >= 88 && 2 * rad < 96) return launch_boxq_deep<80>(r, srcData, srcFlags, dstW, dstO, n, C, rad, denom, sws, dws, W);
        if (2 * rad >= 104 && 2 * rad < 112) return launch_boxq_deep<96>(r, srcData, srcFlags, dstW, dstO, n, C, rad, denom, sws, dws, W);
    }
    switch (boxq_pick_ks8(rad)) {
        case 32: return launch_boxq_ks<32, 8>(r, srcData, srcFlags, dstW, dstO, n, C, rad, denom, sws, dws, W);
        case 40: return launch_boxq_ks<40, 8>(r, srcData, srcFlags, dstW, dstO, n, C, rad, denom, sws, dws, W);
        case 48: return launch_boxq_ks<48, 8>(r, srcData, srcFlags, dstW, dstO, n, C, rad, denom, sws, dws, W);
        case 56: return launch_boxq_ks<56, 8>(r, srcData, srcFlags, dstW, dstO, n, C, rad, denom, sws, dws, W);
        case 64: return launch_boxq_ks<64, 8>(r, srcData, srcFlags, dstW, dstO, n, C, rad, denom, sws, dws, W);
        case 80: return launch_boxq_ks<80, 8>(r, srcData, srcFlags, dstW, dstO, n, C, rad, denom, sws, dws, W);
    }
    switch (ks) {
        case 16: return launch_boxq_ks<16>(r, srcData, srcFlags, dstW, dstO, n, C, rad, denom, sws, dws, W);
        case 32: return launch_boxq_ks<32>(r, srcData, srcFlags, dstW, dstO, n, C, rad, denom, sws, dws, W);
        case 48: return launch_boxq_ks<48>(r, srcData, srcFlags, dstW, dstO, n, C, rad, denom, sws, dws, W);
        case 64: return launch_boxq_ks<64>(r, srcData, srcFlags, dstW, dstO, n, C, rad, denom, sws, dws, W);
        case 80: return launch_boxq_ks<80>(r, srcData, srcFlags, dstW, dstO, n, C, rad, denom, sws, dws, W);
        case 96: return launch_boxq_ks<96>(r, srcData, srcFlags, dstW, dstO, n, C, rad, denom, sws, dws, W);
    }
    return set_err(TRI_EINVAL, "no stage-pipeline kernel for %d slots", ks);
}

int launch_boxt(const Run& r, int ks, const float* srcData, const uint8_t* srcFlags, float* dstW, float* dstO,
                int n, int C, int rad, float denom, size_t sws, size_t dws, int64_t W) {
    switch (ks) {
        case 16: return launch_boxt_ks<16>(r, srcData, srcFlags, dstW, dstO, n, C, rad, denom, sws, dws, W);
        case 20: return launch_boxt_ks<20>(r, srcData, srcFlags, dstW, dstO, n, C, rad, denom, sws, dws, W);
        case 32: return launch_boxt_ks<32>(r, srcData, srcFlags, dstW, dstO, n, C, rad, denom, sws, dws, W);
        case 64: return launch_boxt_ks<64>(r, srcData, srcFlags, dstW, dstO, n, C, rad, denom, sws, dws, W);
        case 80: return launch_boxt_ks<80>(r, srcData, srcFlags, dstW, dstO, n, C, rad, denom, sws, dws, W);
    }
    return set_err(TRI_EINVAL, "no register-ring kernel for %d slots", ks);
}

enum class ColSrc {
    ByteFlags,
    Images,
    PackedFlags
};
enum ColFlag : unsigned {
    COL_TRANSPOSED_OUT = 1,
    COL_WEIGHTS_01 = 2
};
enum class ColFamily { SpecPipe, SpecRing, StagePipe, RegRing, Lane4, LdsRing, MultiPass };
thread_local bool g_colfilter_unpadded = false;

int launch_colfilter(const Run& r, ColSrc src, float* bufW, float* bufO, const float* srcData,
                     const uint8_t* srcFlags, float* dstW, float* dstO, int n, int C, int rad,
                     size_t bws, size_t sws, size_t dws, int64_t W, unsigned flags = 0, float* deferred_denom = nullptr) {
    const bool transposed_out = flags & COL_TRANSPOSED_OUT, weights_are_01 = flags & COL_WEIGHTS_01;
    const float denom = box_denominator(rad);
    const int intw = (weights_are_01 && rad <= 31) ? 1 : 0;
    int bt = colfilter_lds_block(rad, C);
    if (deferred_denom) *deferred_denom = 0.0f;
    const bool regs_ok = !deferred_denom && !transposed_out && weights_are_01 && (uint64_t)n * (uint64_t)C * 4u < (1ull << 31);
    const bool spectrum = regs_ok && src == ColSrc::ByteFlags && W == 1;
    const bool packed = regs_ok && src == ColSrc::PackedFlags && n % 4 == 0;
    ColFamily fam;
    if (spectrum && boxp_pick_block(rad, C) > 0 && rad <= 107 && ((uintptr_t)srcData % 16 == 0) && ((uintptr_t)srcFlags % 4 == 0) &&
        ((uintptr_t)dstW % 16 == 0) && ((uintptr_t)dstO % 16 == 0))
        fam = ColFamily::SpecPipe;
    else if (spectrum && boxr_pick_ks(rad) > 0) fam = ColFamily::SpecRing;
    else if (packed && boxq_pick_ks(rad) > 0 && rad <= 107 && (g_boxq_override == 1 || 2 * rad >= BOXQ_MIN_2R)) fam = ColFamily::StagePipe;
    else if (packed && boxr_pick_ks_t(rad) > 0) fam = ColFamily::RegRing;
    else if (bt > 0 && colfilter_use_lane4(rad) && !transposed_out && src != ColSrc::ByteFlags) fam = ColFamily::Lane4;
    else {
        if (bt > 0 && colfilter_use_lane4(rad) && src == ColSrc::ByteFlags) {
            bt = rad <= 20 ? 128 : (rad <= 40 ? 64 : 0);
            while (bt > 64 && bt / 2 >= C) bt /= 2;
        }
        fam = bt > 0 ? ColFamily::LdsRing : ColFamily::MultiPass;
    }
    if (fam == ColFamily::MultiPass && g_colfilter_unpadded)
        return set_err(TRI_EUNSUPPORTED, "radius %d takes the in-place multi-pass filter, which needs images padded to n + 4r rows", rad);
    const bool built = src != ColSrc::Images, divide = !deferred_denom;
    const float *const inW = built ? nullptr : bufW, *const inO = built ? nullptr : bufO;
    const size_t in_ws = built ? 0 : bws;
    switch (fam) {
        case ColFamily::SpecPipe:
            if (boxp_pick_block(rad, C) == 16) return launch_boxp_spec_b<16, 16>(r, srcData, srcFlags, dstW, dstO, n, C, rad, denom);
            return launch_boxp_spec_b<8, 16>(r, srcData, srcFlags, dstW, dstO, n, C, rad, denom);
        case ColFamily::SpecRing:
            return launch_boxt_spec(r, boxr_pick_ks(rad), srcData, srcFlags, dstW, dstO, n, C, rad, denom);
        case ColFamily::StagePipe:
            return launch_boxq(r, boxq_pick_ks(rad), srcData, srcFlags, dstW, dstO, n, C, rad, denom, sws, dws, W);
        case ColFamily::RegRing:
            return launch_boxt(r, boxr_pick_ks_t(rad), srcData, srcFlags, dstW, dstO, n, C, rad, denom, sws, dws, W);
        case ColFamily::Lane4: {
            HIPCHK(lds_optin_all(160 * 1024, &k_colfilter_lane4<0, true>, &k_colfilter_lane4<1, true>, &k_colfilter_lane4<1, false>,
                                 &k_colfilter_lane4<2, false>, &k_colfilter_lane4<2, true>));
            const auto k = src == ColSrc::PackedFlags ? (divide ? &k_colfilter_lane4<2, true> : &k_colfilter_lane4<2, false>)
                                                      : (divide ? &k_colfilter_lane4<1, true> : &k_colfilter_lane4<1, false>);
            if (!divide) *deferred_denom = denom;
            hipLaunchKernelGGL(k, dim3((unsigned)cdiv(C, 16), (unsigned)W, 2), dim3(64), (size_t)lane4_ring_capacity(rad) * 64 * sizeof(float), r.st,
                               inW, inO, srcData, srcFlags, dstW, dstO, n, C, rad, denom, in_ws, sws, dws);
            break;
        }
        case ColFamily::LdsRing: {
            HIPCHK(lds_optin_all(160 * 1024, &k_colfilter_lds<0, true, false>, &k_colfilter_lds<1, true, false>, &k_colfilter_lds<1, false, false>,
                                 &k_colfilter_lds<1, true, true>, &k_colfilter_lds<2, false, false>, &k_colfilter_lds<2, true, false>));
            auto k = &k_colfilter_lds<0, true, false>;
            bool div = true;
            if (src == ColSrc::PackedFlags) { div = divide; k = div ? &k_colfilter_lds<2, true, false> : &k_colfilter_lds<2, false, false>; }
            else if (transposed_out) k = &k_colfilter_lds<1, true, true>;
            else if (src == ColSrc::Images) { div = divide; k = div ? &k_colfilter_lds<1, true, false> : &k_colfilter_lds<1, false, false>; }
            if (!div) *deferred_denom = denom;
            hipLaunchKernelGGL(k, dim3((unsigned)cdiv(C, bt), (unsigned)W, 2), dim3(bt), (size_t)4 * 2 * rad * bt * sizeof(float), r.st,
                               inW, inO, srcData, srcFlags, dstW, dstO, n, C, rad, denom, in_ws, sws, dws, intw);
            break;
        }
        case ColFamily::MultiPass: {
            const int blk = C >= 256 ? 256 : (C >= 128 ? 128 : 64);
            const auto k = src == ColSrc::ByteFlags ? &k_colfilter<0> : &k_colfilter<1>;
            hipLaunchKernelGGL(k, dim3((unsigned)cdiv(C, blk), (unsigned)W, 2), dim3(blk), 0, r.st, bufW, bufO, srcData, srcFlags,
                               dstW, dstO, n, C, rad, denom, bws, sws, dws);
            break;
        }
    }
    LAUNCHCHK();
    return TRI_OK;
}

bool st_use_pipe(const StWin& sw) {
    static const bool off = is1(getenv("TRI_ST_NO_PIPE"));
    return !off && sw.nw >= 1 && sw.nw <= 8 && stp_lds_bytes(sw) <= 160 * 1024;
}

enum class StKernel { Dyn, Fused, Mask, MaskPanel, Pipe };

int st_launch(hipStream_t st, StKernel k, const StWin& sw, const float* data, const double* med, uint8_t* out,
              const int64_t* d_chunk_ends, double thr_scale, int L, int C, int G, size_t ws_data, size_t ws_out, int64_t W,
              double* ring, uint8_t* acc) {
    int blk = C >= 256 ? 256 : (C >= 128 ? 128 : 64);
    if (const char* e = getenv("TRI_ST_BLK")) { int b = atoi(e); if (b >= 64 && b <= ST_MAXBLK && C >= b) blk = b; }
    const dim3 grid((unsigned)cdiv(C, blk), (unsigned)G, (unsigned)W);
    StFusedArgs fa;
    for (int j = 0; j < 4; j++) fa.tf[j] = sw.tf[j < sw.nw ? j : 0];
    if (k == StKernel::MaskPanel)
        hipLaunchKernelGGL((k_colst_mask<1, 2, 4, 8, true>), grid, dim3(blk), 0, st, data, med, out, d_chunk_ends, fa, thr_scale, L, C, G, ws_data, ws_out);
    else if (k == StKernel::Mask)
        hipLaunchKernelGGL((k_colst_mask<1, 2, 4, 8>), grid, dim3(blk), 0, st, data, med, out, d_chunk_ends, fa, thr_scale, L, C, G, ws_data, ws_out);
    else if (k == StKernel::Fused)
        hipLaunchKernelGGL((k_colst_fused<1, 2, 4, 8>), grid, dim3(blk), 0, st, data, med, out, d_chunk_ends, fa, thr_scale, L, C, G, ws_data, ws_out);
    else if (k == StKernel::Pipe) {
        HIPCHK(lds_optin_all(160 * 1024, &k_colst_pipe));
        hipLaunchKernelGGL(k_colst_pipe, dim3((unsigned)cdiv(C, 64), (unsigned)G, (unsigned)W), dim3(64 * sw.nw), stp_lds_bytes(sw), st,
                           data, med, out, d_chunk_ends, sw, stp_plan(sw), thr_scale, L, C, G, ws_data, ws_out);
    } else
        hipLaunchKernelGGL(k_colst_dyn, grid, dim3(blk), 0, st, data, med, out, ring, acc, d_chunk_ends, sw, thr_scale, L, C, G, ws_data, ws_out);
    LAUNCHCHK();
    return TRI_OK;
}

int launch_colst(const Run& r, const StWin& sw, const float* data, const double* med,
                 uint8_t* out, const int64_t* d_chunk_ends, int L, int C, int G, size_t ws_data,
                 size_t ws_out, int64_t W, bool panel = false) {
    StKernel k;
    if (st_use_fused(sw)) {
        if (panel && !(st_use_mask(L, C) && C % 64 == 0)) return set_err(TRI_EUNSUPPORTED, "panel images: lane-mask SumThreshold kernel on 64-column panels only");
        k = panel ? StKernel::MaskPanel : (st_use_mask(L, C) ? StKernel::Mask : StKernel::Fused);
    } else if (panel) {
        return set_err(TRI_EUNSUPPORTED, "panel images: windows (1, 2, 4, 8) only");
    } else {
        k = st_use_pipe(sw) ? StKernel::Pipe : StKernel::Dyn;
    }
    const double thr_scale = r.p->outlier_nsigma * TRI_MAD_NORMAL;
    return st_launch(r.st, k, sw, data, med, out, d_chunk_ends, thr_scale, L, C, G, ws_data, ws_out, W, r.ws.ring, r.ws.acc);
}

int launch_interp(const Run& r, float* a, int L, int C, size_t ws, int64_t W, const uint8_t* nanflag,
                  const float* data, size_t ws_data, float* resid, float* panel = nullptr, size_t ws_panel = 0) {
    static const bool one_pass = is1(getenv("TRI_INTERP_ONE_PASS"));
    const int nseg = (int)cdiv(L, INTERP_SEG);
    if (one_pass || nseg < 2 || nseg > 65535) {
        hipLaunchKernelGGL(k_colinterp, dim3((unsigned)cdiv(C, 256), (unsigned)W), dim3(256), 0, r.st, a, L, C, ws, nanflag, data, ws_data, resid, panel, ws_panel);
    } else {
        dim3 grid((unsigned)cdiv(C, 64), (unsigned)nseg, (unsigned)W);
        hipLaunchKernelGGL(k_interp_scan, grid, dim3(64), 0, r.st, (const float*)a, L, C, ws, nanflag, r.ws.itab);
        hipLaunchKernelGGL(k_interp_fix, grid, dim3(64), 0, r.st, a, L, C, ws, (const int*)r.ws.itab, data, ws_data, resid, panel, ws_panel);
    }
    LAUNCHCHK();
    return TRI_OK;
}

template <typename T>
int launch_transpose(const Run& r, const T* src, T* dst, int R, int C, size_t sws, size_t dws,
                     int64_t W, float denom = 0.0f, bool panel = false) {
    dim3 grid((unsigned)cdiv(C, 64), (unsigned)cdiv(R, 64), (unsigned)W);
    if (panel) {
        if (R % 64 != 0) return set_err(TRI_EUNSUPPORTED, "panel output needs a multiple of 64 columns");
        hipLaunchKernelGGL((k_transpose<T, true>), grid, dim3(64, 4), 0, r.st, src, dst, R, C, sws, dws, denom);
        LAUNCHCHK();
        return TRI_OK;
    }
    if (sizeof(T) == 1 && R % 4 == 0 && C % 4 == 0 && sws % 4 == 0 && dws % 4 == 0 &&
        ((uintptr_t)src % 4 == 0) && ((uintptr_t)dst % 4 == 0)) {
        dim3 gridw((unsigned)cdiv(C, 64), (unsigned)cdiv(R, 128), (unsigned)W);
        hipLaunchKernelGGL((k_transpose_u8w<false, false>), gridw, dim3(256), 0, r.st, (const uint8_t*)src, (uint8_t*)dst,
                           (uint8_t*)nullptr, (float*)nullptr, R, C, sws, dws, (size_t)0, (size_t)0);
        LAUNCHCHK();
        return TRI_OK;
    }
    hipLaunchKernelGGL(k_transpose<T>, grid, dim3(64, 4), 0, r.st, src, dst, R, C, sws, dws, denom);
    LAUNCHCHK();
    return TRI_OK;
}


template <int OP>
int launch_u8(const Run& r, const uint8_t* a, uint8_t* b, size_t nper, size_t ws_a, size_t ws_b, int64_t W) {
    if (r.pl.vec && nper % 16 == 0 && ws_a % 16 == 0 && ws_b % 16 == 0) {
        hipLaunchKernelGGL(k_u8_op16<OP>, grid1(nper / 16, W), dim3(256), 0, r.st, a, b, nper / 16, ws_a, ws_b);
    } else if (OP == 0) {
        for (int64_t w = 0; w < W; w++)
            hipLaunchKernelGGL(k_copy_u8, dim3((unsigned)cdiv(nper, 256)), dim3(256), 0, r.st, a + w * ws_a, b + w * ws_b, nper);
    } else if (OP == 1) {
        hipLaunchKernelGGL(k_or, grid1(nper, W), dim3(256), 0, r.st, b, a, nper, ws_b, ws_a);
    } else {
        for (int64_t w = 0; w < W; w++)
            hipLaunchKernelGGL(k_normalise_flags, dim3((unsigned)cdiv(nper, 256)), dim3(256), 0, r.st, a + w * ws_a, b + w * ws_b, nper);
    }
    LAUNCHCHK();
    return TRI_OK;
}

template <int MODE>
int launch_masked_div(const Run& r, const float* w, float* o, const float* data, size_t nper, size_t ws_wo, size_t ws_data, int64_t W, float denom = 0.0f,
                      uint8_t* nanflag = nullptr, int C = 1) {
    if (nper % 4 == 0 && ws_wo % 4 == 0 && ws_data % 4 == 0 && (nanflag == nullptr || C % 4 == 0) && ((uintptr_t)w % 16 == 0) && ((uintptr_t)o % 16 == 0))
        hipLaunchKernelGGL(k_masked_div4<MODE>, grid1(nper / 4, W), dim3(256), 0, r.st, w, o, data, nper / 4, ws_wo, ws_data, denom, nanflag, C);
    else
        hipLaunchKernelGGL(k_masked_div<MODE>, grid1(nper, W), dim3(256), 0, r.st, w, o, data, nper, ws_wo, ws_data, denom, nanflag, C);
    LAUNCHCHK();
    return TRI_OK;
}

int launch_sub(const Run& r, const float* a, const float* b, float* out, size_t nper, size_t ws_a, size_t ws_b, size_t ws_o, int64_t W) {
    if (nper % 4 == 0 && ws_a % 4 == 0 && ws_b % 4 == 0 && ws_o % 4 == 0 && ((uintptr_t)a % 16 == 0) && ((uintptr_t)b % 16 == 0) && ((uintptr_t)out % 16 == 0))
        hipLaunchKernelGGL(k_sub4, grid1(nper / 4, W), dim3(256), 0, r.st, a, b, out, nper / 4, ws_a, ws_b, ws_o);
    else
        hipLaunchKernelGGL(k_sub, grid1(nper, W), dim3(256), 0, r.st, a, b, out, nper, ws_a, ws_b, ws_o);
    LAUNCHCHK();
    return TRI_OK;
}

static bool filter_no_tin() { static const bool v = is1(getenv("TRI_FILTER_NO_TIN")); return v; }
bool colfilter_t_usable(int rad) { return !filter_no_tin() && rad > 0 && rad <= 16; }

int launch_colfilter_t(const Run& r, const float* srcW, const float* srcO, float* dstW, float* dstO,
                       int n, int C, int ld, int rad, size_t sws_img, size_t dws, int64_t W, float* deferred_denom) {
    float denom = box_denominator(rad);
    size_t lds = ((size_t)4 * 2 * rad * CFT_BT + (size_t)CFT_PF * (CFT_BT + 1)) * sizeof(float);
    HIPCHK(lds_optin_all(160 * 1024, &k_colfilter_lds_t<false>, &k_colfilter_lds_t<true>));
    dim3 grid((unsigned)cdiv(C, CFT_BT), (unsigned)W, 2);
    if (deferred_denom) *deferred_denom = denom;
    const auto k = deferred_denom ? &k_colfilter_lds_t<false> : &k_colfilter_lds_t<true>;
    hipLaunchKernelGGL(k, grid, dim3(CFT_BT), lds, r.st, srcW, srcO, dstW, dstO, n, C, ld, rad, denom, sws_img, dws);
    LAUNCHCHK();
    return TRI_OK;
}

bool colfilter_tf_usable(int rad) {
    static const bool off = is1(getenv("TRI_FILTER_NO_FUSED_DIV"));
    return !off && colfilter_t_usable(rad);
}

template <int MODE>
int launch_colfilter_tf(const Run& r, const float* srcW, const float* srcO, float* dstW, float* dstO, const float* data,
                        int n, int C, int ld, int rad, size_t sws_img, size_t dws, size_t ws_data, int64_t W, uint8_t* nanflag) {
    float denom = box_denominator(rad);
    size_t lds = (size_t)2 * ((size_t)4 * 2 * rad * CFF_BT + (size_t)CFT_PF * (CFF_BT + 1)) * sizeof(float);
    HIPCHK(lds_optin_all(160 * 1024, &k_colfilter_lds_tf<MODE>));
    dim3 grid((unsigned)cdiv(C, CFF_BT), (unsigned)W);
    hipLaunchKernelGGL(k_colfilter_lds_tf<MODE>, grid, dim3(2 * CFF_BT), lds, r.st, srcW, srcO, dstW, dstO, data, n, C, ld, rad,
                       denom, sws_img, dws, ws_data, nanflag);
    LAUNCHCHK();
    return TRI_OK;
}

template <int KS, int MODE>
int launch_boxf_ks(const Run& r, const float* srcW, const float* srcO, float* dstW, float* dstO, const float* data,
                   int n, int C, int ld, int rad, size_t sws_img, size_t dws, size_t ws_data, int64_t W, uint8_t* nanflag,
                   float* dstP, size_t pws, bool* wroteP) {
    const BoxDenom denom = box_reciprocal(box_denominator(rad));
    const int d = 2 * rad - KS;
    if (!(MODE == 2 && boxf_panel_ok(KS, d > 0))) dstP = nullptr;
    if (dstP && wroteP) *wroteP = true;
    const size_t lds = ((size_t)4 * d * 64 + (size_t)2 * boxr_pf_f(KS) * boxf_nsub(KS) * boxf_ts(boxr_pf_f(KS) * boxf_nsub(KS))) * sizeof(float);
    if (srcO <= srcW || ((uint64_t)(srcO - srcW) + (uint64_t)C * ld) * 4u >= (1ull << 31))
        return set_err(TRI_EUNSUPPORTED, "fused frequency stage: the data image must follow the weight image within 2^31 bytes");
    const unsigned gap = (unsigned)(srcO - srcW);
    HIPCHK(lds_optin_all(160 * 1024, &k_boxf<KS, true, MODE>));
    dim3 grid((unsigned)cdiv(C, 32), (unsigned)W);
    auto k = d > 0 ? &k_boxf<KS, true, MODE> : &k_boxf<KS, false, MODE>;
    if constexpr (KS == 32) {
        if (d > 14) { k = &k_boxf<KS, true, MODE, 1>; HIPCHK(lds_optin_all(160 * 1024, k)); }
    }
    hipLaunchKernelGGL(k, grid, dim3(64), lds, r.st, srcW, gap, dstW, dstO, data, n, C, ld, rad, denom, sws_img, dws, ws_data, nanflag, dstP, pws);
    LAUNCHCHK();
    return TRI_OK;
}

#ifndef BOXQF_MIN_2R
#define BOXQF_MIN_2R 34
#endif
#ifndef BOXQF_FEW_WAVES
#define BOXQF_FEW_WAVES 2048
#endif
#ifndef BOXQF_B8_DEFAULT
#define BOXQF_B8_DEFAULT 1
#endif
#ifndef BOXQF_B8_MAX2R
#define BOXQF_B8_MAX2R 88
#endif
template <int KS, int MODE, int B = 16>
int launch_boxqf_ks(const Run& r, const float* srcW, unsigned gap, float* dstW, float* dstO, const float* data,
                    int n, int C, int ld, int rad, size_t sws_img, size_t dws, size_t ws_data, int64_t W, uint8_t* nanflag) {
    HIPCHK(lds_optin_all(160 * 1024, &k_boxqf<KS, MODE, B>));
    const BoxDenom denom = box_reciprocal(box_denominator(rad));
    dim3 grid((unsigned)cdiv(C, 64), (unsigned)W);
    hipLaunchKernelGGL((k_boxqf<KS, MODE, B>), grid, dim3(512), boxqf_lds_bytes(B, boxqf_dbl(KS, B)), r.st, srcW, gap, dstW, dstO, data, n, C, ld, rad,
                       denom, sws_img, dws, ws_data, nanflag);
    LAUNCHCHK();
    return TRI_OK;
}

template <int MODE>
int launch_boxf(const Run& r, int ks, const float* srcW, const float* srcO, float* dstW, float* dstO, const float* data,
                int n, int C, int ld, int rad, size_t sws_img, size_t dws, size_t ws_data, int64_t W, uint8_t* nanflag,
                float* dstP = nullptr, size_t pws = 0, bool* wroteP = nullptr) {
    if (MODE != 2 || n % 64 != 0) dstP = nullptr;
    {
        static const bool off = is1(getenv("TRI_FILTER_NO_PIPE_F"));
        const int kq = boxq_pick_ks(rad);
        const bool few = (int64_t)W * cdiv(C, 32) < BOXQF_FEW_WAVES;
        const bool want = g_boxq_override == 1 || (g_boxq_override < 0 && !off && (2 * rad >= BOXQF_MIN_2R || (few && 2 * rad >= 16)));
        if (want && kq > 0 && srcO > srcW && n % 4 == 0 && ld % 4 == 0 && sws_img % 4 == 0 && (uint64_t)(srcO - srcW) % 4 == 0 &&
            ((uintptr_t)srcW % 16 == 0) && ((uint64_t)(srcO - srcW) + (uint64_t)C * ld) * 4u < (1ull << 31) &&
            (uint64_t)n * (uint64_t)C * 4u < (1ull << 31)) {
            const unsigned gap = (unsigned)(srcO - srcW);
            static const int b8 = [] { const char* e = getenv("TRI_FILTER_PIPE_F_B8"); return e ? atoi(e) : BOXQF_B8_DEFAULT; }();
            if (b8 && g_boxq_b8_override != 0 && 2 * rad >= 16 && 2 * rad < BOXQF_B8_MAX2R) {
                switch (2 * rad / 8 * 8) {
                    case 16: return launch_boxqf_ks<16, MODE, 8>(r, srcW, gap, dstW, dstO, data, n, C, ld, rad, sws_img, dws, ws_data, W, nanflag);
                    case 24: return launch_boxqf_ks<24, MODE, 8>(r, srcW, gap, dstW, dstO, data, n, C, ld, rad, sws_img, dws, ws_data, W, nanflag);
                    case 32: return launch_boxqf_ks<32, MODE, 8>(r, srcW, gap, dstW, dstO, data, n, C, ld, rad, sws_img, dws, ws_data, W, nanflag);
                    case 40: return launch_boxqf_ks<40, MODE, 8>(r, srcW, gap, dstW, dstO, data, n, C, ld, rad, sws_img, dws, ws_data, W, nanflag);
                    case 48: return launch_boxqf_ks<48, MODE, 8>(r, srcW, gap, dstW, dstO, data, n, C, ld, rad, sws_img, dws, ws_data, W, nanflag);
#if BOXQF_B8_MAX2R > 56
                    case 56: return launch_boxqf_ks<56, MODE, 8>(r, srcW, gap, dstW, dstO, data, n, C, ld, rad, sws_img, dws, ws_data, W, nanflag);
                    case 64: return launch_boxqf_ks<64, MODE, 8>(r, srcW, gap, dstW, dstO, data, n, C, ld, rad, sws_img, dws, ws_data, W, nanflag);
#endif
#if BOXQF_B8_MAX2R > 72
                    case 72: return launch_boxqf_ks<72, MODE, 8>(r, srcW, gap, dstW, dstO, data, n, C, ld, rad, sws_img, dws, ws_data, W, nanflag);
                    case 80:
                        if (MODE == 1) return launch_boxqf_ks<80, 1, 8>(r, srcW, gap, dstW, dstO, data, n, C, ld, rad, sws_img, dws, ws_data, W, nanflag);
                        break;
#endif
#if BOXQF_B8_MAX2R > 88
                    case 96: return launch_boxqf_ks<96, MODE, 8>(r, srcW, gap, dstW, dstO, data, n, C, ld, rad, sws_img, dws, ws_data, W, nanflag);
#endif
                }
            }
            switch (kq) {
                case 16: return launch_boxqf_ks<16, MODE>(r, srcW, gap, dstW, dstO, data, n, C, ld, rad, sws_img, dws, ws_data, W, nanflag);
                case 32: return launch_boxqf_ks<32, MODE>(r, srcW, gap, dstW, dstO, data, n, C, ld, rad, sws_img, dws, ws_data, W, nanflag);
                case 48: return launch_boxqf_ks<48, MODE>(r, srcW, gap, dstW, dstO, data, n, C, ld, rad, sws_img, dws, ws_data, W, nanflag);
                case 64: return launch_boxqf_ks<64, MODE>(r, srcW, gap, dstW, dstO, data, n, C, ld, rad, sws_img, dws, ws_data, W, nanflag);
                case 80: return launch_boxqf_ks<80, MODE>(r, srcW, gap, dstW, dstO, data, n, C, ld, rad, sws_img, dws, ws_data, W, nanflag);
                case 96: return launch_boxqf_ks<96, MODE>(r, srcW, gap, dstW, dstO, data, n, C, ld, rad, sws_img, dws, ws_data, W, nanflag);
            }
        }
    }
    switch (ks) {
        case 8: return launch_boxf_ks<8, MODE>(r, srcW, srcO, dstW, dstO, data, n, C, ld, rad, sws_img, dws, ws_data, W, nanflag, dstP, pws, wroteP);
        case 16: return launch_boxf_ks<16, MODE>(r, srcW, srcO, dstW, dstO, data, n, C, ld, rad, sws_img, dws, ws_data, W, nanflag, dstP, pws, wroteP);
        case 32: return launch_boxf_ks<32, MODE>(r, srcW, srcO, dstW, dstO, data, n, C, ld, rad, sws_img, dws, ws_data, W, nanflag, dstP, pws, wroteP);
        case 64: return launch_boxf_ks<64, MODE>(r, srcW, srcO, dstW, dstO, data, n, C, ld, rad, sws_img, dws, ws_data, W, nanflag, dstP, pws, wroteP);
        case 80: return launch_boxf_ks<80, MODE>(r, srcW, srcO, dstW, dstO, data, n, C, ld, rad, sws_img, dws, ws_data, W, nanflag, dstP, pws, wroteP);
    }
    return set_err(TRI_EINVAL, "no register-ring kernel for %d slots", ks);
}

thread_local int g_boxx_override = -1;
thread_local unsigned long long g_boxx_last_stats[2] = {0, 0};
#ifndef BOXX_MIN_R
#define BOXX_MIN_R 56
#endif
int boxx_pick_l(int rad, int n) {
    static const bool env_off = is1(getenv("TRI_FILTER_NO_EXACT"));
    static const int force_nti = [] { const char* e = getenv("TRI_BOXX_NTI"); return e ? atoi(e) : 0; }();
    if (g_boxx_override == 0 || (g_boxx_override < 0 && (env_off || rad < BOXX_MIN_R))) return 0;
    if (rad < 1 || n % 4 != 0) return 0;
    const int64_t P = (int64_t)n + 4 * (int64_t)rad;
    struct Cand { int nti, l; };
    static const Cand cands[] = {{128, 37}, {128, 41}, {256, 17}, {256, 19}, {256, 21}, {256, 25}};
    for (const Cand& c : cands) {
        if (force_nti && c.nti != force_nti) continue;
        if (c.nti == 128 && (P <= 128 * 17 || rad < 64)) continue;
        if ((int64_t)c.nti * c.l < P || c.l > 2 * rad + 1 || (2 * rad + 1) / c.l > BOXX_AMAX) continue;
        if (boxx_lds_bytes(c.nti, c.l, rad) > 159 * 1024) continue;
        return c.l | (c.nti << 8);
    }
    return 0;
}
static bool boxx_recip_ok(int rad) { return rad <= 128 || rad == 166 || rad == 221 || rad == 277 || rad == 397 || rad == 795; }

template <int NTI, int L, int MODE>
int launch_boxx_l(const Run& r, const float* srcW, unsigned gap, const float* data, const uint8_t* mask, float* outA, float* outB,
                  int n, int C, int ld, int rad, size_t sws_img, size_t ws_data, size_t ws_mask, size_t ws_outA, size_t ws_outB,
                  int64_t W, uint8_t* nanflag, unsigned long long* stats) {
    const BoxDenom denom = box_reciprocal(box_denominator(rad));
    const size_t lds = boxx_lds_bytes(NTI, L, rad);
    dim3 grid((unsigned)C, (unsigned)W);
    const auto k = boxx_recip_ok(rad) ? &k_boxx<NTI, L, MODE, true> : &k_boxx<NTI, L, MODE, false>;
    HIPCHK(lds_optin_all(159 * 1024, k));
    hipLaunchKernelGGL(k, grid, dim3(2 * NTI), lds, r.st, srcW, gap, data, mask, outA, outB, n, ld, rad, denom, sws_img,
                       ws_data, ws_mask, ws_outA, ws_outB, nanflag, stats);
    LAUNCHCHK();
    return TRI_OK;
}
template <int MODE>
int launch_boxx(const Run& r, int L, const float* srcW, const float* srcO, const float* data, const uint8_t* mask, float* outA, float* outB,
                int n, int C, int ld, int rad, size_t sws_img, size_t ws_data, size_t ws_mask, size_t ws_outA, size_t ws_outB,
                int64_t W, uint8_t* nanflag, unsigned long long* stats = nullptr) {
    if (srcO <= srcW || ld % 4 != 0 || sws_img % 4 != 0 || (uint64_t)(srcO - srcW) % 4 != 0 || ((uintptr_t)srcW % 16 != 0) ||
        ((uintptr_t)data % 16 != 0) || ws_data % 4 != 0 || ((uintptr_t)outA % 16 != 0) || ws_outA % 4 != 0 ||
        (mask && (((uintptr_t)mask % 4 != 0) || ws_mask % 4 != 0)) || (uint64_t)(srcO - srcW) > 0xffffffffull ||
        (MODE == 2 && (((uintptr_t)outB % 16 != 0) || ws_outB % 4 != 0)) || C > 65535 * 1024)
        return set_err(TRI_EUNSUPPORTED, "exact row filter: unaligned images");
    const unsigned gap = (unsigned)(srcO - srcW);
#define BOXX_CASE(NTI, LL) case ((NTI) << 8 | (LL)): return launch_boxx_l<NTI, LL, MODE>(r, srcW, gap, data, mask, outA, outB, n, C, ld, rad, sws_img, ws_data, ws_mask, ws_outA, ws_outB, W, nanflag, stats);
    switch (L) {
        BOXX_CASE(128, 37) BOXX_CASE(128, 41)
        BOXX_CASE(256, 17) BOXX_CASE(256, 19) BOXX_CASE(256, 21) BOXX_CASE(256, 25)
    }
#undef BOXX_CASE
    return set_err(TRI_EINVAL, "no exact row filter for code %d", L);
}

bool colfilter_t4_usable(int rad) { return !filter_no_tin() && colfilter_use_lane4(rad); }

int launch_colfilter_t4(const Run& r, const float* srcW, const float* srcO, float* dstW, float* dstO,
                        int n, int C, int ld, int rad, size_t sws_img, size_t dws, int64_t W, float* deferred_denom) {
    float denom = box_denominator(rad);
    size_t lds = ((size_t)lane4_ring_capacity(rad) * 64 + 32 * 17) * sizeof(float);
    HIPCHK(lds_optin_all(160 * 1024, &k_colfilter_lane4<3, false>, &k_colfilter_lane4<3, true>));
    dim3 grid((unsigned)cdiv(C, 16), (unsigned)W, 2);
    if (deferred_denom) *deferred_denom = denom;
    const auto k = deferred_denom ? &k_colfilter_lane4<3, false> : &k_colfilter_lane4<3, true>;
    hipLaunchKernelGGL(k, grid, dim3(64), lds, r.st, srcW, srcO, (const float*)nullptr, (const uint8_t*)nullptr,
                       dstW, dstO, n, C, rad, denom, sws_img, (size_t)ld, dws);
    LAUNCHCHK();
    return TRI_OK;
}

int spectrum_medians(const Run& r, const float* img, const uint8_t* flg) {
    const Plan& pl = r.pl;
    const Ws& ws = r.ws;
    const int Fa = (int)pl.Fa, Wn = (int)r.Wb, G = (int)pl.G;
    int rc = launch_transpose<float>(r, img, ws.srowsf, Fa, Wn, 0, 0, 1);
    if (rc) return rc;
    rc = launch_transpose<uint8_t>(r, flg, ws.srowsu, Fa, Wn, 0, 0, 1);
    if (rc) return rc;
    bool seg4 = Fa % 4 == 0;
    for (int64_t g = 0; g < pl.G + 1 && seg4; g++) seg4 = r.p->chunk_ends[g] % 4 == 0;
    MedianJob j;
    j.data = ws.srowsf; j.flags = ws.srowsu; j.med = ws.smed; j.RS = (size_t)Fa;
    j.seg_start = ws.segC_start; j.seg_len = ws.segC_len; j.R = Wn; j.G = G; j.W = 1; j.max_len = pl.maxchunk;
    j.vec_ok = j.segs_aligned = seg4; j.rows_aligned = Fa % 4 == 0;
    return launch_median(r, j);
}

int spectrum_background(const Run& r) {
    const Plan& pl = r.pl;
    const Ws& ws = r.ws;
    int Fa = (int)pl.Fa, Wn = (int)r.Wb, G = (int)pl.G;
    size_t nS = (size_t)Fa * Wn;
    hipLaunchKernelGGL(k_copy_u8, dim3((unsigned)cdiv(nS, 256)), dim3(256), 0, r.st, ws.sflags, ws.sbgf, nS);
    LAUNCHCHK();
    double rej = TRI_MAD_NORMAL * r.p->background_reject;
    bool rowD_valid = false;
    for (int ext = pl.nit; ext >= 0; ext--) {
        bool final_pass = ext == 0;
        double sigma = (double)(final_pass ? 1 : ext) * r.p->spike_width_freq;
        int rad = (int)box_radius(sigma);
        const int xl = (rad > 0 && 2 * (size_t)pl.PT >= 4) ? boxx_pick_l(rad, Fa) : 0;
        if (xl > 0) {
            float* rowW = ws.Aw;
            float* rowO = ws.Aw + nS;
            float* rowD = ws.Aw + 2 * nS;
            float* rowR = ws.Aw + 3 * nS;
            hipLaunchKernelGGL(k_build_wo, grid1(nS, 1), dim3(256), 0, r.st, ws.sdata, ws.sbgf, ws.sw, ws.so, nS, (size_t)0, (size_t)0);
            LAUNCHCHK();
            int rc = launch_transpose<float>(r, ws.sw, rowW, Fa, Wn, 0, 0, 1);
            if (!rc) rc = launch_transpose<float>(r, ws.so, rowO, Fa, Wn, 0, 0, 1);
            if (!rc && !rowD_valid) rc = launch_transpose<float>(r, ws.sdata, rowD, Fa, Wn, 0, 0, 1);
            if (rc) return rc;
            rowD_valid = true;
            if (final_pass)
                rc = launch_boxx<2>(r, xl, rowW, rowO, rowD, nullptr, rowR, rowW, Fa, Wn, Fa, rad, 0, 0, 0, 0, 0, 1, reinterpret_cast<uint8_t*>(ws.rowcnt));
            else
                rc = launch_boxx<1>(r, xl, rowW, rowO, rowD, nullptr, rowR, nullptr, Fa, Wn, Fa, rad, 0, 0, 0, 0, 0, 1, nullptr);
            if (!rc) rc = launch_transpose<float>(r, rowR, ws.so, Wn, Fa, 0, 0, 1);
            if (rc) return rc;
            if (!final_pass) {
                rc = spectrum_medians(r, ws.so, ws.sbgf);
                if (rc) return rc;
                hipLaunchKernelGGL(k_reject<false>, grid1(nS, 1), dim3(256), 0, r.st, ws.so, ws.sbgf, ws.smed, ws.d_chunk_of, rej, Fa, Wn, G, (size_t)0, (size_t)0);
                LAUNCHCHK();
            }
            continue;
        }
        if (rad > 0) {
            int rc = launch_colfilter(r, ColSrc::ByteFlags, ws.sw, ws.so, ws.sdata, ws.sbgf, ws.sw, ws.so, Fa, Wn, rad, 0, 0, 0, 1, COL_WEIGHTS_01);
            if (rc) return rc;
        } else {
            hipLaunchKernelGGL(k_build_wo, grid1(nS, 1), dim3(256), 0, r.st, ws.sdata, ws.sbgf, ws.sw, ws.so, nS, (size_t)0, (size_t)0);
            LAUNCHCHK();
        }
        if (final_pass) {
            { int rc2 = launch_masked_div<0>(r, ws.sw, ws.so, ws.sdata, nS, 0, 0, 1); if (rc2) return rc2; }
        } else {
            { int rc2 = launch_masked_div<1>(r, ws.sw, ws.so, ws.sdata, nS, 0, 0, 1); if (rc2) return rc2; }
            int rc = spectrum_medians(r, ws.so, ws.sbgf);
            if (rc) return rc;
            hipLaunchKernelGGL(k_reject<false>, grid1(nS, 1), dim3(256), 0, r.st, ws.so, ws.sbgf, ws.smed, ws.d_chunk_of, rej, Fa, Wn, G, (size_t)0, (size_t)0);
            LAUNCHCHK();
        }
    }
    return launch_interp(r, ws.so, Fa, Wn, (size_t)0, 1, (const uint8_t*)nullptr, (const float*)nullptr, (size_t)0, (float*)nullptr);
}

static bool bg_flags_packed(int T, size_t N) {
    static const bool no_pack = is1(getenv("TRI_NO_PACKED_FLAGS"));
    return !no_pack && (T % 4 == 0) && (N % 4 == 0);
}


enum class TimeStage {
    BuildOnly,
    PackedSweep,
    Prebuilt,
    PrebuiltDirectFT,
    ByteFlags
};
enum class FreqStage {
    ExactRows,
    FusedRing,
    FusedLds,
    LdsDiv,
    Lane4Div,
    Transposed
};
enum class Reject {
    None,
    InRows,
    Tile,
    OnePass,
    MedianReject4T,
    MedianReject4,
    MedianReject
};

struct FreqPick {
    FreqStage route;
    int ks;
    int xl;
    size_t off;
};
static FreqPick pick_freq_unfused(int rad, int C) {
    return {FreqStage::Transposed, 0, 0, colfilter_lds_block(rad, C) > 0 ? 0 : (size_t)4 * rad * C};
}
static FreqPick pick_freq_stage(int rad, int n, int C, size_t gap, bool exact_rows) {
    const int ks = ((uint64_t)gap + (uint64_t)n * C) * 4u < (1ull << 31) ? boxr_pick_ks_f(rad) : 0;
    const int xl = (rad > 0 && (!ks || rad >= BOXX_MIN_R) && exact_rows) ? boxx_pick_l(rad, n) : 0;
    if (xl > 0) return {FreqStage::ExactRows, 0, xl, 0};
    if (ks > 0) return {FreqStage::FusedRing, ks, 0, 0};
    if (colfilter_tf_usable(rad)) return {FreqStage::FusedLds, 0, 0, 0};
    if (colfilter_t_usable(rad)) return {FreqStage::LdsDiv, 0, 0, 0};
    if (colfilter_t4_usable(rad)) return {FreqStage::Lane4Div, 0, 0, 0};
    return pick_freq_unfused(rad, C);
}

struct TileRoute { bool use; size_t ccap, ucap; int ytiles; };
static int medrej_force_fallback() { static const int v = [] { const char* e = getenv("TRI_MEDREJ_FORCE_FALLBACK"); return e ? atoi(e) : 0; }(); return v; }
static bool no_fused_reject() { static const bool v = is1(getenv("TRI_NO_FUSED_REJECT")); return v; }
static bool fused_medrej() { static const bool v = is1(getenv("TRI_FUSED_MEDREJ")); return v; }
static TileRoute pick_tile_route(const Run& r, bool packed) {
    const Plan& pl = r.pl;
    static const bool no_tile = is1(getenv("TRI_NO_TILE_MEDREJ"));
    const int T = (int)pl.T, G = (int)pl.G;
    const size_t wsA = 2 * (size_t)pl.PT * pl.Fa, wsB = (size_t)pl.PF * T;
    const size_t mr_nb = (size_t)pl.maxchunk * T;
    TileRoute t = {false, (mr_nb / 4) & ~(size_t)3, (mr_nb / 8) & ~(size_t)3, 0};
    for (int g = 0; g < G; g++) t.ytiles += (int)cdiv(r.p->chunk_ends[g + 1] - r.p->chunk_ends[g], 64);
    t.use = pl.vec && wsB % 4 == 0 && wsA % 4 == 0 && packed && !no_fused_reject() && !no_tile && !fused_medrej() && G <= 65535 &&
            mrt_scratch_words(G, t.ccap, t.ucap) <= wsA && (medrej_force_fallback() || (pl.maxchunk - 1) * (int64_t)T >= 65536) &&
            t.ytiles > 0 && t.ytiles <= 65535;
    return t;
}
static unsigned medrej_capq(size_t wsA, int G) {
    const size_t per_block = (wsA / (size_t)G) & ~(size_t)7;
    return (unsigned)std::min<size_t>(per_block / 2, 0x3ffffffcu);
}

struct BgStep {
    int r0, r1;
    bool final_pass;
    TimeStage time;
    bool time_needs_bytes;
    bool time_defers;
    FreqPick freq;
    bool freq_transposes;
    Reject reject;
    bool reads_ft_flags;
};

static BgStep pick_bg_step(const Run& r, bool packed, bool tile_route, int ext) {
    const Plan& pl = r.pl;
    const int T = (int)pl.T, Fa = (int)pl.Fa, G = (int)pl.G;
    const size_t wsA = 2 * (size_t)pl.PT * Fa, wsB = (size_t)pl.PF * T;
    BgStep s;
    s.final_pass = ext == 0;
    const double e = (double)(s.final_pass ? 1 : ext);
    s.r0 = (int)box_radius(e * r.p->spike_width_time);
    s.r1 = (int)box_radius(e * r.p->spike_width_freq);

    static const bool prebuild = [] { const char* e = getenv("TRI_TIME_PREBUILD"); return !(e && e[0] == '0'); }();
    const bool sweep = s.r0 > 0 && colfilter_lds_block(s.r0, Fa) > 0;
    if (s.r0 == 0) s.time = TimeStage::BuildOnly;
    else if (sweep && packed) s.time = TimeStage::PackedSweep;
    else if (sweep && prebuild) {
        static const bool want_direct = is1(getenv("TRI_FILTER_DIRECT_FT"));
        s.time = (want_direct && T % 4 == 0 && wsB % 4 == 0) ? TimeStage::PrebuiltDirectFT : TimeStage::Prebuilt;
    } else s.time = TimeStage::ByteFlags;
    s.time_needs_bytes = packed && (s.time == TimeStage::BuildOnly || s.time == TimeStage::ByteFlags);

    s.freq = s.time == TimeStage::PrebuiltDirectFT ? pick_freq_unfused(s.r1, T)
                                                   : pick_freq_stage(s.r1, Fa, T, (size_t)(r.ws.Ao - r.ws.Aw), !r.ampl_cached || r.data_mask);
    s.freq_transposes = s.time != TimeStage::PrebuiltDirectFT;
    s.time_defers = s.freq.route == FreqStage::Transposed;

    static const bool no_tfr = is1(getenv("TRI_FILTER_NO_TF_REJECT"));
    const bool vec4 = pl.vec && wsB % 4 == 0;
    if (s.final_pass) s.reject = Reject::None;
    else if (s.freq.route == FreqStage::ExactRows && packed && !no_tfr && G <= 65535 && (uint64_t)T * Fa * 4u < (1ull << 31))
        s.reject = Reject::InRows;
    else if (tile_route) s.reject = Reject::Tile;
    else if (vec4 && wsA % 4 == 0 && packed && !no_fused_reject() && fused_medrej() && medrej_capq(wsA, G) >= 1024 && G <= 65535 &&
             (uint64_t)T * Fa * 4u < (1ull << 32))
        s.reject = Reject::OnePass;
    else if (vec4 && packed && !no_fused_reject()) s.reject = Reject::MedianReject4T;
    else s.reject = vec4 ? Reject::MedianReject4 : Reject::MedianReject;
    s.reads_ft_flags = s.time_needs_bytes || (!s.final_pass && s.reject != Reject::InRows);
    return s;
}

struct BgImages {
    int T, Fa;
    int64_t W;
    const float *dataTF, *dataFT;
    const uint8_t* flagsTF;
    uint8_t* comb;
    float *Aw, *Ao; size_t wsA;
    float *Bw, *Bo; size_t wsB;
    float* rows; size_t ws_rows;
    const uint8_t* mask; size_t ws_mask;
    uint8_t* nanflag;
    float* residP;
    unsigned long long* xstats;
};

struct BgState {
    uint8_t *cur_ft, *alt_ft;
    bool bgf_ft_stale;
    bool wrote_panel;
};

static int bg_time_stage(const Run& r, const BgStep& s, const BgImages& im, const BgState& st, float* den_t) {
    const int T = im.T, Fa = im.Fa;
    const size_t N = (size_t)T * Fa;
    const int64_t W = im.W;
    int rc = TRI_OK;
    *den_t = 0.0f;
    float* const defer = s.time_defers ? den_t : nullptr;
    const uint8_t* fl = im.flagsTF;
    if (s.time_needs_bytes) {
        rc = launch_transpose<uint8_t>(r, st.cur_ft, im.comb, Fa, T, N, N, W);
        if (rc) return rc;
        fl = im.comb;
    }
    switch (s.time) {
        case TimeStage::BuildOnly:
            hipLaunchKernelGGL(k_build_wo, grid1(N, W), dim3(256), 0, r.st, im.dataTF, fl, im.Aw, im.Ao, N, N, im.wsA);
            LAUNCHCHK();
            return TRI_OK;
        case TimeStage::PackedSweep:
            return launch_colfilter(r, ColSrc::PackedFlags, im.Aw, im.Ao, im.dataTF, fl, im.Aw, im.Ao, T, Fa, s.r0, im.wsA, N, im.wsA, W, COL_WEIGHTS_01, defer);
        case TimeStage::Prebuilt:
        case TimeStage::PrebuiltDirectFT:
            if (N % 4 == 0 && im.wsA % 4 == 0)
                hipLaunchKernelGGL(k_build_wo4, grid1(N / 4, W), dim3(256), 0, r.st, im.dataTF, fl, im.Aw, im.Ao, N / 4, N, im.wsA);
            else
                hipLaunchKernelGGL(k_build_wo, grid1(N, W), dim3(256), 0, r.st, im.dataTF, fl, im.Aw, im.Ao, N, N, im.wsA);
            LAUNCHCHK();
            if (s.time == TimeStage::Prebuilt)
                return launch_colfilter(r, ColSrc::Images, im.Aw, im.Ao, nullptr, nullptr, im.Aw, im.Ao, T, Fa, s.r0, im.wsA, 0, im.wsA, W, COL_WEIGHTS_01, defer);
            return launch_colfilter(r, ColSrc::Images, im.Aw, im.Ao, nullptr, nullptr, im.Bw + s.freq.off, im.Bo + s.freq.off, T, Fa, s.r0, im.wsA, 0, im.wsB, W, COL_TRANSPOSED_OUT);
        case TimeStage::ByteFlags:
            return launch_colfilter(r, ColSrc::ByteFlags, im.Aw, im.Ao, im.dataTF, fl, im.Aw, im.Ao, T, Fa, s.r0, im.wsA, N, im.wsA, W);
    }
    return set_err(TRI_EINVAL, "internal: no such time stage");
}

template <int MODE>
static int bg_freq_stage_mode(const Run& r, const BgStep& s, const BgImages& im, BgState& st, float den_t) {
    const int T = im.T, Fa = im.Fa, r1 = s.r1;
    const size_t N = (size_t)T * Fa, wsA = im.wsA, wsB = im.wsB;
    const int64_t W = im.W;
    uint8_t* const nan = MODE == 2 ? im.nanflag : nullptr;
    float den_f = 0.0f;
    int rc = TRI_OK;
    if (MODE == 2) HIPCHK(hipMemsetAsync(im.nanflag, 0, (size_t)W * T, r.st));
    switch (s.freq.route) {
        case FreqStage::ExactRows:
            rc = launch_boxx<MODE>(r, s.freq.xl, im.Aw, im.Ao, im.dataTF, im.mask, im.rows, MODE == 2 ? im.Aw : nullptr, Fa, T, Fa, r1, wsA, N,
                                   im.ws_mask, im.ws_rows, MODE == 2 ? wsA : 0, W, nan, im.xstats);
            if (!rc && MODE == 2) rc = launch_transpose<float>(r, im.Aw, im.Bw, T, Fa, wsA, wsB, W);
            if (rc || s.reject == Reject::InRows) return rc;
            return launch_transpose<float>(r, im.rows, im.Bo, T, Fa, im.ws_rows, wsB, W);
        case FreqStage::FusedRing:
            return launch_boxf<MODE>(r, s.freq.ks, im.Aw, im.Ao, im.Bw, im.Bo, im.dataFT, Fa, T, Fa, r1, wsA, wsB, N, W, nan,
                                     MODE == 2 ? im.residP : nullptr, MODE == 2 ? N : 0, &st.wrote_panel);
        case FreqStage::FusedLds:
            return launch_colfilter_tf<MODE>(r, im.Aw, im.Ao, im.Bw, im.Bo, im.dataFT, Fa, T, Fa, r1, wsA, wsB, N, W, nan);
        case FreqStage::LdsDiv:
            rc = launch_colfilter_t(r, im.Aw, im.Ao, im.Bw, im.Bo, Fa, T, Fa, r1, wsA, wsB, W, &den_f);
            break;
        case FreqStage::Lane4Div:
            rc = launch_colfilter_t4(r, im.Aw, im.Ao, im.Bw, im.Bo, Fa, T, Fa, r1, wsA, wsB, W, &den_f);
            break;
        case FreqStage::Transposed:
            if (s.freq_transposes) {
                rc = launch_transpose<float>(r, im.Aw, im.Bw + s.freq.off, T, Fa, wsA, wsB, W, den_t);
                if (!rc) rc = launch_transpose<float>(r, im.Ao, im.Bo + s.freq.off, T, Fa, wsA, wsB, W, den_t);
            }
            if (!rc && r1 > 0) rc = launch_colfilter(r, ColSrc::Images, im.Bw, im.Bo, nullptr, nullptr, im.Bw, im.Bo, Fa, T, r1, wsB, 0, wsB, W, 0, &den_f);
            break;
    }
    if (rc) return rc;
    return launch_masked_div<MODE>(r, im.Bw, im.Bo, im.dataFT, N, wsB, N, W, den_f, nan, MODE == 2 ? T : 1);
}
static int bg_freq_stage(const Run& r, const BgStep& s, const BgImages& im, BgState& st, float den_t) {
    return s.final_pass ? bg_freq_stage_mode<2>(r, s, im, st, den_t) : bg_freq_stage_mode<1>(r, s, im, st, den_t);
}

static int bg_reject_stage(const Run& r, const BgStep& s, const TileRoute& tile, bool packed, BgState& st) {
    const Plan& pl = r.pl;
    const Ws& ws = r.ws;
    const int T = (int)pl.T, Fa = (int)pl.Fa, G = (int)pl.G;
    const int64_t W = r.Wb;
    const size_t N = (size_t)T * Fa, wsA = 2 * (size_t)pl.PT * Fa, wsB = (size_t)pl.PF * T;
    const double rej = TRI_MAD_NORMAL * r.p->background_reject;
    if (s.reject == Reject::None) return TRI_OK;
    if (s.reject != Reject::Tile && st.cur_ft == ws.flagsFT)
        return set_err(TRI_EUNSUPPORTED, "internal: background flags read in place on a route that rewrites them");
    switch (s.reject) {
        case Reject::InRows: {
            unsigned* gc = reinterpret_cast<unsigned*>(ws.Aw);
            unsigned cap = (unsigned)(std::min<size_t>((wsA / 2) / (size_t)G, 0x7fffffffu) & ~(size_t)3);
            if (median_no_predict() || (int64_t)cap < pl.maxchunk * pl.T || wsA % 4 != 0) { gc = nullptr; cap = 0; }
            hipLaunchKernelGGL((k_median2<false, true>), dim3((unsigned)G, (unsigned)W), dim3(256), 0, r.st, (const float*)ws.Ao,
                               (const uint8_t*)ws.bgfTF, ws.med, wsA, N, (size_t)0, (size_t)1, ws.segC_start, ws.segC_len, 1, G,
                               gc, gc ? wsA : (size_t)0, cap, T / 4, Fa);
            hipLaunchKernelGGL(k_reject_tf, dim3((unsigned)cdiv(Fa, 256), (unsigned)(T / 4), (unsigned)W), dim3(256), 0, r.st,
                               (const float*)ws.Ao, reinterpret_cast<unsigned*>(ws.bgfTF), ws.med, ws.d_chunk_of, rej, T / 4, Fa, Fa, G,
                               wsA, N / 4);
            LAUNCHCHK();
            st.bgf_ft_stale = true;
            return TRI_OK;
        }
        case Reject::Tile: {
            unsigned* sc = reinterpret_cast<unsigned*>(ws.Aw);
            hipLaunchKernelGGL(k_mr_predict, dim3((unsigned)G, (unsigned)W), dim3(256), 0, r.st, (const float*)ws.Bo, (const uint8_t*)st.cur_ft,
                               ws.d_chunk_ends, rej, T / 4, G, wsB, N, sc, wsA, tile.ccap, tile.ucap, medrej_force_fallback());
            for (unsigned round = 1; round <= 2; round++) {
                hipLaunchKernelGGL(k_mr_pass, dim3((unsigned)cdiv(T / 4, 64), (unsigned)tile.ytiles, (unsigned)W), dim3(256), 0, r.st, (const float*)ws.Bo,
                                   (const uint8_t*)st.cur_ft, st.alt_ft, ws.bgfTF, ws.d_chunk_ends, Fa, T / 4, G, wsB, N, sc, wsA, tile.ccap, tile.ucap, round);
                hipLaunchKernelGGL(k_mr_finish, dim3((unsigned)G, (unsigned)W), dim3(256), 0, r.st, (const float*)ws.Bo, (const uint8_t*)st.cur_ft, st.alt_ft,
                                   ws.bgfTF, ws.med, ws.d_chunk_ends, rej, Fa, T / 4, G, wsB, N, sc, wsA, tile.ccap, tile.ucap, round);
            }
            hipLaunchKernelGGL(k_median_reject, dim3((unsigned)G, (unsigned)W), dim3(256), 0, r.st, (const float*)ws.Bo, (const uint8_t*)st.cur_ft,
                               st.alt_ft, ws.bgfTF, ws.med, ws.d_chunk_ends, rej, Fa, T / 4, G, wsB, N, sc, wsA, 0u, 0u, 1,
                               (const unsigned*)sc, wsA, (int)MRT_PARW, 11);
            LAUNCHCHK();
            std::swap(st.cur_ft, st.alt_ft);
            if (st.alt_ft == ws.flagsFT) st.alt_ft = ws.fflFT;
            return TRI_OK;
        }
        case Reject::OnePass: {
            const unsigned capq = medrej_capq(wsA, G);
            hipLaunchKernelGGL(k_median_reject, dim3((unsigned)G, (unsigned)W), dim3(256), 0, r.st, (const float*)ws.Bo, (const uint8_t*)st.cur_ft,
                               st.alt_ft, ws.bgfTF, ws.med, ws.d_chunk_ends, rej, Fa, T / 4, G, wsB, N,
                               reinterpret_cast<unsigned*>(ws.Aw), wsA, capq, capq, medrej_force_fallback());
            LAUNCHCHK();
            std::swap(st.cur_ft, st.alt_ft);
            return TRI_OK;
        }
        default:
            break;
    }
    MedianJob j;
    j.data = ws.Bo; j.flags = st.cur_ft; j.med = ws.med; j.WSd = wsB; j.WSf = N;
    j.seg_start = ws.segB_start; j.seg_len = ws.segB_len; j.R = 1; j.G = G; j.W = W; j.max_len = pl.maxchunk * pl.T;
    j.vec_ok = T % 4 == 0 && wsB % 4 == 0 && N % 4 == 0;
    j.gcand = reinterpret_cast<unsigned*>(ws.Aw); j.cand_ws = wsA;
    j.cand_cap = (unsigned)(std::min<size_t>(wsA / (size_t)G, 0x7fffffffu) & ~(size_t)3);
    const int rc = launch_median(r, j);
    if (rc) return rc;
    if (s.reject == Reject::MedianReject4T) {
        hipLaunchKernelGGL(k_reject4_t, dim3((unsigned)cdiv(T / 4, 64), (unsigned)cdiv(Fa, 64), (unsigned)W), dim3(64, 4), 0, r.st,
                           ws.Bo, st.cur_ft, ws.bgfTF, ws.med, ws.d_chunk_of, rej, Fa, T / 4, G, wsB, N);
        LAUNCHCHK();
        return TRI_OK;
    }
    if (s.reject == Reject::MedianReject4)
        hipLaunchKernelGGL(k_reject4, grid1(N / 4, W), dim3(256), 0, r.st, ws.Bo, st.cur_ft, ws.med, ws.d_chunk_of, rej, T / 4, G, N / 4, wsB, N);
    else
        hipLaunchKernelGGL(k_reject<true>, grid1(N, W), dim3(256), 0, r.st, ws.Bo, st.cur_ft, ws.med, ws.d_chunk_of, rej, Fa, T, G, wsB, N);
    LAUNCHCHK();
    if (packed) return launch_transpose<float>(r, reinterpret_cast<const float*>(st.cur_ft), reinterpret_cast<float*>(ws.bgfTF), Fa, T / 4, N / 4, N / 4, W);
    return launch_transpose<uint8_t>(r, st.cur_ft, ws.bgfTF, Fa, T, N, N, W);
}

int background2d(const Run& r, bool flagsFT_current, float* residP = nullptr, bool* wroteP = nullptr) {
    const Plan& pl = r.pl;
    const Ws& ws = r.ws;
    const int T = (int)pl.T, Fa = (int)pl.Fa;
    const int64_t W = r.Wb;
    const size_t N = (size_t)T * Fa;
    const bool packed = bg_flags_packed(T, N);
    const TileRoute tile = pick_tile_route(r, packed);
    static const bool copy_flags = is1(getenv("TRI_BG_COPY_FLAGS"));
    bool flags_in_place = flagsFT_current && !copy_flags && packed && tile.use;
    for (int ext = pl.nit; ext >= 1 && flags_in_place; ext--)
        if (pick_bg_step(r, packed, tile.use, ext).freq.route == FreqStage::ExactRows) flags_in_place = false;
    int rc = TRI_OK;
    if (!flags_in_place)
        rc = flagsFT_current ? launch_u8<0>(r, ws.flagsFT, ws.bgfFT, N, N, N, W)
                             : launch_transpose<uint8_t>(r, ws.flagsTF, ws.bgfFT, T, Fa, N, N, W);
    if (rc) return rc;
    if (packed)
        rc = launch_transpose<float>(r, reinterpret_cast<const float*>(flags_in_place ? ws.flagsFT : ws.bgfFT), reinterpret_cast<float*>(ws.bgfTF), Fa, T / 4, N / 4, N / 4, W);
    else
        rc = launch_u8<0>(r, ws.flagsTF, ws.bgfTF, N, N, N, W);
    if (rc) return rc;

    BgImages im;
    im.T = T; im.Fa = Fa; im.W = W;
    im.dataTF = ws.dataTF; im.dataFT = ws.dataFT;
    im.flagsTF = ws.bgfTF; im.comb = ws.comb;
    im.Aw = ws.Aw; im.Ao = ws.Ao; im.wsA = 2 * (size_t)pl.PT * Fa;
    im.Bw = ws.Bw; im.Bo = ws.Bo; im.wsB = (size_t)pl.PF * T;
    im.rows = ws.Ao; im.ws_rows = im.wsA;
    im.mask = r.ampl_cached ? r.data_mask : nullptr; im.ws_mask = r.data_mask_ws;
    im.nanflag = reinterpret_cast<uint8_t*>(ws.rowcnt);
    im.residP = residP; im.xstats = nullptr;
    BgState st = {flags_in_place ? ws.flagsFT : ws.bgfFT, flags_in_place ? ws.bgfFT : ws.fflFT, false, false};
    for (int ext = pl.nit; ext >= 0; ext--) {
        const BgStep s = pick_bg_step(r, packed, tile.use, ext);
        if (st.bgf_ft_stale && s.reads_ft_flags) {
            rc = launch_transpose<float>(r, reinterpret_cast<const float*>(ws.bgfTF), reinterpret_cast<float*>(st.cur_ft), T / 4, Fa, N / 4, N / 4, W);
            if (rc) return rc;
            st.bgf_ft_stale = false;
        }
        float den_t = 0.0f;
        rc = bg_time_stage(r, s, im, st, &den_t);
        if (!rc) rc = bg_freq_stage(r, s, im, st, den_t);
        if (!rc) rc = bg_reject_stage(r, s, tile, packed, st);
        if (rc) return rc;
    }
    if (wroteP) *wroteP = st.wrote_panel;
    return launch_interp(r, ws.Bo, Fa, T, im.wsB, W, reinterpret_cast<const uint8_t*>(ws.rowcnt), (const float*)ws.dataFT, N, ws.Bw,
                         st.wrote_panel ? residP : nullptr, N);
}


enum class Begin {
    FusedCached,
    Cached,
    Prepare4,
    Prepare
};
enum class SpecOr {
    Scalar,
    Rows16,
    FtInPlace,
    FtInPlaceDeferTf
};
enum class ChunkFlags {
    ExtraSources,
    OrMore16,
    OrBytes
};
enum class Finish {
    FusedDilate,
    Combine16Dilate,
    Combine16,
    Combine
};
enum class FinalKernel {
    NanMask16,
    Vis16,
    Scalar
};
struct IterStep {
    Begin begin; SpecOr spec_or; ChunkFlags chunk_flags; Finish finish; FinalKernel final_kernel;
    bool panel;
    bool fused_resid;
    int lo, hi, flo, fhi;
    bool ft_current() const { return spec_or == SpecOr::FtInPlace || spec_or == SpecOr::FtInPlaceDeferTf; }
};

static void smear_extents(int64_t e, int* lo, int* hi) {
    const int64_t half = e >= 0 ? e / 2 : -((-e + 1) / 2);
    *lo = (int)-half; *hi = (int)(-half + e);
}
static bool st_no_panel() { static const bool off = is1(getenv("TRI_ST_NO_PANEL")); return off; }

static IterStep pick_iteration(const Run& r) {
    const Plan& pl = r.pl;
    const int T = (int)pl.T, F = (int)pl.F, Fa = (int)pl.Fa;
    const size_t N = (size_t)T * Fa;
    static const bool no_fused_begin = is1(getenv("TRI_NO_FUSED_BEGIN"));
    static const bool no_ft_or = is1(getenv("TRI_NO_FT_SPEC_OR"));
    static const bool no_fused_or = is1(getenv("TRI_NO_FUSED_OR"));
    static const bool no_fused_dilate = is1(getenv("TRI_NO_FUSED_DILATE"));
    static const bool no_fused_resid = [] { const char* e = getenv("TRI_NO_FUSED_RESID_TF"); return !(e && e[0] == '0'); }();
    IterStep s;
    smear_extents(r.p->time_extend, &s.lo, &s.hi);
    smear_extents(r.p->freq_extend, &s.flo, &s.fhi);
    if (!r.ampl_cached) s.begin = pl.vec ? Begin::Prepare4 : Begin::Prepare;
    else s.begin = (!no_fused_begin && T % 4 == 0 && Fa % 4 == 0 && N % 4 == 0 && (uintptr_t)r.ws.iter % 4 == 0) ? Begin::FusedCached : Begin::Cached;
    if (!pl.vec) s.spec_or = SpecOr::Scalar;
    else if (no_ft_or || T % 16 != 0) s.spec_or = SpecOr::Rows16;
    else s.spec_or = bg_flags_packed(T, N) ? SpecOr::FtInPlaceDeferTf : SpecOr::FtInPlace;
    const bool defer_tf = s.spec_or == SpecOr::FtInPlaceDeferTf;
    if (defer_tf && !no_fused_or && median_takes_extra_flags(pl.maxchunk) && Fa % 4 == 0) s.chunk_flags = ChunkFlags::ExtraSources;
    else s.chunk_flags = defer_tf ? ChunkFlags::OrMore16 : ChunkFlags::OrBytes;
    if (!pl.vec) s.finish = Finish::Combine;
    else if (s.flo != -1 || s.fhi != 2) s.finish = Finish::Combine16;
    else s.finish = no_fused_dilate ? Finish::Combine16Dilate : Finish::FusedDilate;
    s.final_kernel = !pl.vec ? FinalKernel::Scalar : r.ampl_cached ? FinalKernel::NanMask16 : FinalKernel::Vis16;
    s.panel = !st_no_panel() && s.chunk_flags == ChunkFlags::ExtraSources && s.finish == Finish::FusedDilate && Fa % 64 == 0 && Fa == F &&
              median_takes_extra_flags(pl.maxchunk + 3) && st_use_fused(pl.swT) && st_use_mask(T, Fa);
    s.fused_resid = s.panel && !no_fused_resid;
    return s;
}

template <int VD>
static int launch_prepare(const Run& r, const IterStep& s, const void* vis) {
    const Plan& pl = r.pl;
    const Ws& ws = r.ws;
    const size_t N = (size_t)pl.T * pl.Fa, W = (size_t)r.Wb;
    if (s.begin == Begin::Prepare4)
        hipLaunchKernelGGL(k_prepare4<VD>, dim3((unsigned)cdiv(N * W / 4, 256)), dim3(256), 0, r.st, vis, ws.iter, ws.dataTF, ws.flagsTF, N * W / 4);
    else
        hipLaunchKernelGGL(k_prepare<VD>, grid1(N, W), dim3(256), 0, r.st, vis, ws.iter, ws.dataTF, ws.flagsTF, (int)pl.T, (int)pl.F, (int)pl.Fa, (int)pl.avg);
    LAUNCHCHK();
    return TRI_OK;
}
template <int VD>
static int launch_final(const Run& r, const IterStep& s, const void* vis, uint8_t* out_flags, bool update_iter) {
    const Ws& ws = r.ws;
    const int T = (int)r.pl.T, F = (int)r.pl.F, upd = update_iter ? 1 : 0;
    const size_t NF = (size_t)T * F, W = (size_t)r.Wb;
    const double row_limit = r.p->flag_all_freq_frac * (double)F, col_limit = (double)T * r.p->flag_all_time_frac;
    if (s.final_kernel == FinalKernel::NanMask16)
        hipLaunchKernelGGL(k_final16<TRI_VIS_NANMASK>, grid1(NF / 16, W), dim3(256), 0, r.st, ws.dil, ws.rowcnt, ws.colcnt, (const void*)ws.nanmask, out_flags, ws.iter, T, F / 16, row_limit, col_limit, upd);
    else if (s.final_kernel == FinalKernel::Vis16)
        hipLaunchKernelGGL(k_final16<VD>, grid1(NF / 16, W), dim3(256), 0, r.st, ws.dil, ws.rowcnt, ws.colcnt, vis, out_flags, ws.iter, T, F / 16, row_limit, col_limit, upd);
    else
        hipLaunchKernelGGL(k_final<VD>, grid1(NF, W), dim3(256), 0, r.st, ws.dil, ws.rowcnt, ws.colcnt, vis, out_flags, ws.iter, T, F, row_limit, col_limit, upd);
    LAUNCHCHK();
    return TRI_OK;
}
#define BY_VIS_DTYPE(FN, ...) \
    (vis_dtype == TRI_VIS_C64 ? FN<TRI_VIS_C64>(__VA_ARGS__) : vis_dtype == TRI_VIS_F64 ? FN<TRI_VIS_F64>(__VA_ARGS__) : FN<TRI_VIS_F32>(__VA_ARGS__))

static int iter_begin(const Run& r, const IterStep& s, const void* vis, int vis_dtype) {
    const Ws& ws = r.ws;
    const int T = (int)r.pl.T, Fa = (int)r.pl.Fa;
    const size_t N = (size_t)T * Fa;
    const int64_t W = r.Wb;
    int rc = TRI_OK;
    switch (s.begin) {
        case Begin::FusedCached:
            hipLaunchKernelGGL((k_transpose_u8w<true, true>), dim3((unsigned)cdiv(Fa, 64), (unsigned)cdiv(T, 128), (unsigned)W), dim3(256), 0, r.st,
                               ws.iter, ws.flagsFT, ws.flagsTF, ws.dataFT, T, Fa, N, N, N, N);
            break;
        case Begin::Cached:
            rc = launch_u8<0>(r, ws.iter, ws.flagsTF, N, N, N, W);
            if (!rc) rc = launch_transpose<uint8_t>(r, ws.flagsTF, ws.flagsFT, T, Fa, N, N, W);
            if (rc) return rc;
            hipLaunchKernelGGL(k_zero_flagged4, grid1(N / 4, W), dim3(256), 0, r.st, ws.flagsFT, ws.dataFT, N / 4, N, N);
            break;
        case Begin::Prepare4:
        case Begin::Prepare:
            rc = BY_VIS_DTYPE(launch_prepare, r, s, vis);
            if (!rc) rc = launch_transpose<float>(r, ws.dataTF, ws.dataFT, T, Fa, N, N, W);
            if (!rc) rc = launch_transpose<uint8_t>(r, ws.flagsTF, ws.flagsFT, T, Fa, N, N, W);
            return rc;
    }
    LAUNCHCHK();
    return TRI_OK;
}

static int time_medians(const Run& r, const float* dataFT, size_t ws_data) {
    const Ws& ws = r.ws;
    const int T = (int)r.pl.T, Fa = (int)r.pl.Fa;
    MedianJob j;
    j.data = dataFT; j.flags = ws.flagsFT; j.med = ws.med; j.WSd = ws_data; j.WSf = (size_t)T * Fa; j.RS = (size_t)T;
    j.seg_start = ws.segT_start; j.seg_len = ws.segT_len; j.R = Fa; j.G = 1; j.W = r.Wb; j.max_len = r.pl.T;
    j.rows_aligned = T % 4 == 0; j.segs_aligned = true;
    return launch_median(r, j);
}

static int iter_spectrum(const Run& r, const IterStep& s) {
    const Ws& ws = r.ws;
    const int T = (int)r.pl.T, Fa = (int)r.pl.Fa, Wn = (int)r.Wb;
    const size_t N = (size_t)T * Fa, nS = (size_t)Fa * Wn;
    const int64_t W = r.Wb;
    int rc = time_medians(r, ws.dataFT, N);
    if (rc) return rc;
    hipLaunchKernelGGL(k_spec_from_med, dim3((unsigned)cdiv(nS, 256)), dim3(256), 0, r.st, ws.med, ws.sdata, ws.sflags, Fa, Wn);
    LAUNCHCHK();
// ... 1413 lines not shown
```

Baseline: 3110 Mvis/s.

## Write time-filter images as 64-channel panels for coalesced frequency-pass reads

Adds an optional panel layout for the intermediate weight and amplitude images. The time-direction box kernels write each 64-column block contiguously (row stride 64, panel stride 64*n), and the frequency-direction kernels read through matching panel addressing. The aim is to turn the frequency pass's strided line reads into contiguous panel reads without a separate transpose. It is gated to the packed-sweep plus fused-ring route with Fa divisible by 64, and adds address arithmetic and layout coupling between stages.

```diff
diff --git a/tricolour_amd/csrc/kernels_boxline.hpp b/tricolour_amd/csrc/kernels_boxline.hpp
--- a/tricolour_amd/csrc/kernels_boxline.hpp
+++ b/tricolour_amd/csrc/kernels_boxline.hpp
@@ -103,7 +103,7 @@
 template <int KS, bool HASL, int IMG, bool PACKED, int PF>
 __device__ __forceinline__ void boxt_body(const float* __restrict__ srcData, const uint8_t* __restrict__ srcFlags,
                                           float* __restrict__ dstImg, int n, int C, int r, float denom, size_t sws, size_t dws,
-                                          const size_t win) {
+                                          const size_t win, const int ols, const int ows) {
     extern __shared__ float cf_ring[];
     const int c = blockIdx.x * 64 + threadIdx.x;
     if (c >= C) return;
@@ -115,6 +115,8 @@
         (void*)(srcData + win * sws), 0, (int)((unsigned)n * rowb), 0x00020000);
     const __amdgpu_buffer_rsrc_t frs = __builtin_amdgcn_make_buffer_rsrc(
         (void*)(srcFlags + win * sws), 0, PACKED ? (int)((unsigned)(n / 4) * rowb) : (int)((unsigned)n * (unsigned)C), 0x00020000);
+    const unsigned orowb = (unsigned)ols * 4u;
+    const unsigned oshift = blockIdx.x * (unsigned)(ows - 64) * 4u;
     const __amdgpu_buffer_rsrc_t ors = __builtin_amdgcn_make_buffer_rsrc(
         (void*)(dstImg + win * dws), 0, (int)((unsigned)n * rowb), 0x00020000);
     const int coff = c * 4;
@@ -157,7 +159,7 @@
         }
     };
     auto store = [&](int i, float y) {
-        __builtin_amdgcn_raw_buffer_store_b32(__builtin_bit_cast(unsigned, y), ors, coff, (int)((unsigned)i * rowb), 0);
+        __builtin_amdgcn_raw_buffer_store_b32(__builtin_bit_cast(unsigned, y), ors, coff, (int)((unsigned)i * orowb + oshift), 0);
     };
     issue(0);
     for (int mb = 0; mb < total; mb += UNR) {
@@ -203,8 +205,8 @@
 template <int KS, bool HASL, int IMG>
 __global__ void __launch_bounds__(64, boxr_waves(KS))
 k_boxt(const float* __restrict__ srcData, const uint8_t* __restrict__ srcFlags,
-       float* __restrict__ dstImg, int n, int C, int r, float denom, size_t sws, size_t dws) {
-    boxt_body<KS, HASL, IMG, true, boxr_pf(KS)>(srcData, srcFlags, dstImg, n, C, r, denom, sws, dws, blockIdx.y);
+       float* __restrict__ dstImg, int n, int C, int r, float denom, size_t sws, size_t dws, int ols, int ows) {
+    boxt_body<KS, HASL, IMG, true, boxr_pf(KS)>(srcData, srcFlags, dstImg, n, C, r, denom, sws, dws, blockIdx.y, ols, ows);
 }
 
 __host__ __device__ constexpr int boxt_spec_pf(int ks) { return ks <= 16 ? 64 : (ks == 32 ? 32 : 16); }
@@ -212,8 +214,8 @@
 __global__ void __launch_bounds__(64, 1)
 k_boxt_spec(const float* __restrict__ srcData, const uint8_t* __restrict__ srcFlags,
             float* __restrict__ dstW, float* __restrict__ dstO, int n, int C, int r, float denom) {
-    if (blockIdx.y == 0) boxt_body<KS, HASL, 0, false, boxt_spec_pf(KS)>(srcData, srcFlags, dstW, n, C, r, denom, 0, 0, 0);
-    else boxt_body<KS, HASL, 1, false, boxt_spec_pf(KS)>(srcData, srcFlags, dstO, n, C, r, denom, 0, 0, 0);
+    if (blockIdx.y == 0) boxt_body<KS, HASL, 0, false, boxt_spec_pf(KS)>(srcData, srcFlags, dstW, n, C, r, denom, 0, 0, 0, C, 64);
+    else boxt_body<KS, HASL, 1, false, boxt_spec_pf(KS)>(srcData, srcFlags, dstO, n, C, r, denom, 0, 0, 0, C, 64);
 }
 
 __host__ __device__ constexpr int boxf_ts(int pf) { return pf >= 32 ? 33 : 34; }
@@ -231,7 +233,7 @@
 k_boxf(const float* __restrict__ srcW, unsigned img_gap,
        float* __restrict__ dstW, float* __restrict__ dstO, const float* __restrict__ data,
        int n, int C, int ld, int r, BoxDenom denom, size_t sws_img, size_t dws, size_t ws_data,
-       uint8_t* __restrict__ nanflag, float* __restrict__ dstP, size_t pws) {
+       uint8_t* __restrict__ nanflag, float* __restrict__ dstP, size_t pws, int sls, int sps) {
     extern __shared__ float cf_ring[];
     constexpr int PF = boxr_pf_f(KS);
     static_assert(MODE != 2 || (PF / 2) % 4 == 0, "panel output: groups of four positions per lane");
@@ -269,13 +271,13 @@
 
     const int s_pos = hl % PL;
     const int s_line0 = hl / PL;
-    const unsigned ldb = (unsigned)ld * 4u;
+    const unsigned ldb = (unsigned)sls * 4u;
     const __amdgpu_buffer_rsrc_t srs = __builtin_amdgcn_make_buffer_rsrc(
         (void*)(srcW + win * sws_img), 0, (int)((img_gap + (unsigned)C * (unsigned)ld) * 4u), 0x00020000);
     const int s_off = (int)((unsigned)s_line0 * ldb) + s_pos * 4 + (half ? (int)(img_gap * 4u) : 0);
     float pre[PL];
     auto issue = [&](int t0) {
-        const int sbase = (int)((unsigned)c0 * ldb) + t0 * 4;
+        const int sbase = (int)((unsigned)c0 * ldb) + ((t0 >> 6) * sps + (t0 & 63)) * 4;
         if (t0 + PL <= n && c0 + 32 <= C) {
 #pragma unroll
             for (int j = 0; j < PL; j++)
diff --git a/tricolour_amd/csrc/kernels_boxpipe.hpp b/tricolour_amd/csrc/kernels_boxpipe.hpp
--- a/tricolour_amd/csrc/kernels_boxpipe.hpp
+++ b/tricolour_amd/csrc/kernels_boxpipe.hpp
@@ -184,7 +184,7 @@
 template <int IMG, int KS, int P, int B = 16, int NF = 3>
 __device__ __forceinline__ void boxq_body(const float* __restrict__ srcData, const uint8_t* __restrict__ srcFlags,
                                           float* __restrict__ dst, const int n, const int C, const int r, const BoxDenom denom,
-                                          const size_t sws, const size_t dws, const size_t win) {
+                                          const size_t sws, const size_t dws, const size_t win, const int ols, const int ows) {
     using V = typename std::conditional<IMG == 0, int, float>::type;
     using A = typename std::conditional<IMG == 0, int, double>::type;
     constexpr int PPT = B / 4;
@@ -208,7 +208,9 @@
     const unsigned rowb = (unsigned)C * 4u;
     const __amdgpu_buffer_rsrc_t frs = __builtin_amdgcn_make_buffer_rsrc((void*)(srcFlags + win * sws), 0, (int)((unsigned)(n / 4) * rowb), 0x00020000);
     const __amdgpu_buffer_rsrc_t drs = __builtin_amdgcn_make_buffer_rsrc((void*)(srcData + win * sws), 0, (int)((unsigned)n * rowb), 0x00020000);
-    const __amdgpu_buffer_rsrc_t ors = __builtin_amdgcn_make_buffer_rsrc((void*)(dst + win * dws), 0, (int)((unsigned)n * rowb), 0x00020000);
+    const unsigned orowb = (unsigned)ols * 4u;
+    const unsigned oshift = blockIdx.x * (unsigned)(ows - 64);
+    const __amdgpu_buffer_rsrc_t ors = __builtin_amdgcn_make_buffer_rsrc((void*)(dst + win * dws + oshift), 0, (int)((unsigned)n * rowb - oshift * 4u), 0x00020000);
     const unsigned coff = (unsigned)c * 4u;
     for (int k = tid; k < 4 * (NF + 1) * B * 64; k += 256) reinterpret_cast<V*>(cf_ring)[k] = 0;
 
@@ -328,7 +330,7 @@
                 for (int k = 0; k < PPT; k++) {
                     const int i = i0 + k;
                     const bool ok = bs >= 0 && bs < NB && i >= 0 && i < n && colok;
-                    __builtin_amdgcn_raw_buffer_store_b32(__builtin_bit_cast(unsigned, y[k]), ors, (int)(ok ? (unsigned)i * rowb + coff : OOB), 0, 0);
+                    __builtin_amdgcn_raw_buffer_store_b32(__builtin_bit_cast(unsigned, y[k]), ors, (int)(ok ? (unsigned)i * orowb + coff : OOB), 0, 0);
                 }
             }
 #endif
@@ -340,14 +342,14 @@
 template <int KS, int IMG, int B = 16>
 __global__ void __launch_bounds__(256, B == 8 ? 4 : 2)
 k_boxq(const float* __restrict__ srcData, const uint8_t* __restrict__ srcFlags, float* __restrict__ dstImg,
-       int n, int C, int r, BoxDenom denom, size_t sws, size_t dws) {
-    boxq_body<IMG, KS, B == 8 ? boxq_prefetch8(KS / 8) : boxq_prefetch(KS), B>(srcData, srcFlags, dstImg, n, C, r, denom, sws, dws, blockIdx.y);
+       int n, int C, int r, BoxDenom denom, size_t sws, size_t dws, int ols, int ows) {
+    boxq_body<IMG, KS, B == 8 ? boxq_prefetch8(KS / 8) : boxq_prefetch(KS), B>(srcData, srcFlags, dstImg, n, C, r, denom, sws, dws, blockIdx.y, ols, ows);
 }
 template <int KS, int IMG>
 __global__ void __launch_bounds__(256, 3)
 k_boxq_deep(const float* __restrict__ srcData, const uint8_t* __restrict__ srcFlags, float* __restrict__ dstImg,
-            int n, int C, int r, BoxDenom denom, size_t sws, size_t dws) {
-    boxq_body<IMG, KS, boxq_prefetch8(KS / 8), 8, 4>(srcData, srcFlags, dstImg, n, C, r, denom, sws, dws, blockIdx.y);
+            int n, int C, int r, BoxDenom denom, size_t sws, size_t dws, int ols, int ows) {
+    boxq_body<IMG, KS, boxq_prefetch8(KS / 8), 8, 4>(srcData, srcFlags, dstImg, n, C, r, denom, sws, dws, blockIdx.y, ols, ows);
 }
 
 #ifndef BOXQF_LW
@@ -380,7 +382,7 @@
 __global__ void __launch_bounds__(512, B == 8 ? BOXQF_MINW8 : 1)
 k_boxqf(const float* __restrict__ srcW, unsigned img_gap, float* __restrict__ dstW, float* __restrict__ dstO,
         const float* __restrict__ data, int n, int C, int ld, int r, BoxDenom denom, size_t sws_img, size_t dws,
-        size_t ws_data, uint8_t* __restrict__ nanflag) {
+        size_t ws_data, uint8_t* __restrict__ nanflag, int sps) {
     constexpr int PP = B / 4;
     constexpr int FN = B / 8;
     constexpr int NBLK = KS / B;
@@ -425,21 +427,26 @@
 
     const int s_line = (tid & 255) >> 2, s_q = tid & 3;
     const bool s_lok = c0 + s_line < C;
-    const float* s_base = srcW + win * sws_img + (size_t)(img ? img_gap : 0u) + (size_t)(s_lok ? c0 + s_line : 0) * ld;
+    const char* const s_img = reinterpret_cast<const char*>(srcW + win * sws_img);
+    const unsigned s_lineb = ((img ? img_gap : 0u) + (unsigned)(s_lok ? c0 + s_line : 0) * (unsigned)ld) * 4u;
+    auto s_at = [&](int pb, int p) {
+        if (PAIR) return s_img + (size_t)(unsigned)((pb < n ? (pb >> 6) * (sps - 64) : 0) * 4) + (s_lineb + (p < n ? (unsigned)p * 4u : 0u));
+        return s_img + (s_lineb + (p < n ? (unsigned)((pb >> 6) * (sps - 64) + p) * 4u : 0u));
+    };
     float pre[DBL ? P2 : P][DBL ? 4 : PP];
     auto issue = [&](int blk, int q) {
         if (DBL) {
             const int p = blk * 16 + 4 * s_q;
-            const float4 v = *reinterpret_cast<const float4*>(s_base + (p < n ? p : 0));
+            const float4 v = *reinterpret_cast<const float4*>(s_at(blk * 16, p));
             pre[q][0] = v.x; pre[q][1] = v.y; pre[q][DBL ? 2 : 0] = v.z; pre[q][DBL ? 3 : 0] = v.w;
             return;
         }
         const int p = blk * B + PP * s_q;
         if (PP == 4) {
-            const float4 v = *reinterpret_cast<const float4*>(s_base + (p < n ? p : 0));
+            const float4 v = *reinterpret_cast<const float4*>(s_at(blk * B, p));
             pre[q][0] = v.x; pre[q][1] = v.y; pre[q][PP - 2] = v.z; pre[q][PP - 1] = v.w;
         } else {
-            const float2 v = *reinterpret_cast<const float2*>(s_base + (p < n ? p : 0));
+            const float2 v = *reinterpret_cast<const float2*>(s_at(blk * B, p));
             pre[q][0] = v.x; pre[q][1] = v.y;
         }
     };
diff --git a/tricolour_amd/csrc/kernels_boxweight.hpp b/tricolour_amd/csrc/kernels_boxweight.hpp
--- a/tricolour_amd/csrc/kernels_boxweight.hpp
+++ b/tricolour_amd/csrc/kernels_boxweight.hpp
@@ -24,7 +24,7 @@
 
 template <int R2>
 __global__ void __launch_bounds__(64, boxw_waves(R2))
-k_boxw(const uint8_t* __restrict__ srcFlags, float* __restrict__ dstW, int n, int C, BoxDenom denom, size_t sws, size_t dws) {
+k_boxw(const uint8_t* __restrict__ srcFlags, float* __restrict__ dstW, int n, int C, BoxDenom denom, size_t sws, size_t dws, int ols, int ows) {
     constexpr int N1 = (R2 + 31) / 32, N2 = (R2 + 3) / 4, N3 = (R2 + 1) / 2;
     constexpr int P = BOXW_PREFETCH;
     constexpr unsigned OOB = 0x7ffffff0u;
@@ -36,7 +36,9 @@
     const unsigned rowb = (unsigned)C * 4u;
     const unsigned coff = colok ? (unsigned)c * 4u : OOB;
     const __amdgpu_buffer_rsrc_t frs = __builtin_amdgcn_make_buffer_rsrc((void*)(srcFlags + win * sws), 0, (int)((unsigned)(n / 4) * rowb), 0x00020000);
-    const __amdgpu_buffer_rsrc_t ors = __builtin_amdgcn_make_buffer_rsrc((void*)(dstW + win * dws), 0, (int)((unsigned)n * rowb), 0x00020000);
+    const unsigned orowb = (unsigned)ols * 4u;
+    const unsigned oshift = blockIdx.x * (unsigned)(ows - 64);
+    const __amdgpu_buffer_rsrc_t ors = __builtin_amdgcn_make_buffer_rsrc((void*)(dstW + win * dws + oshift), 0, (int)((unsigned)n * rowb - oshift * 4u), 0x00020000);
 
     unsigned D1[N1], D2[N2], D3[N3], D4[R2];
 #pragma unroll
@@ -96,7 +98,7 @@
             const int i = t - 2 * R2;
             const bool rowok = (unsigned)i < (unsigned)n;
             const float y = boxw_divide((float)o4, denom);
-            __builtin_amdgcn_raw_buffer_store_b32(__builtin_bit_cast(unsigned, y), ors, (int)(rowok ? coff : OOB), (int)(rowok ? (unsigned)i * rowb : 0u), 0);
+            __builtin_amdgcn_raw_buffer_store_b32(__builtin_bit_cast(unsigned, y), ors, (int)(rowok ? coff : OOB), (int)(rowok ? (unsigned)i * orowb : 0u), 0);
             if (BOXW_SCHED_EVERY > 0 && (u + 1) % BOXW_SCHED_EVERY == 0) __builtin_amdgcn_sched_barrier(0);
         }
     };
diff --git a/tricolour_amd/csrc/tricolour_amd.hip b/tricolour_amd/csrc/tricolour_amd.hip
--- a/tricolour_amd/csrc/tricolour_amd.hip
+++ b/tricolour_amd/csrc/tricolour_amd.hip
@@ -510,6 +510,16 @@
     return off ? 0 : boxr_pick_ks(rad);
 }
 
+#ifndef TRI_FILTER_PANELS
+#define TRI_FILTER_PANELS 1
+#endif
+struct ImgLayout {
+    int ls;
+    int ws;
+};
+static ImgLayout img_rows(int C) { return {C, 64}; }
+static ImgLayout img_panels(int n) { return {64, 64 * n}; }
+
 thread_local int g_boxw_override = -1;
 static bool boxw_usable(int rad, int n, int C) {
     static const bool off = is1(getenv("TRI_FILTER_NO_BOXW"));
@@ -517,14 +527,14 @@
     return 2 * rad >= 20 && 2 * rad <= 110 && n % 4 == 0 && (uint64_t)n * (uint64_t)C * 4u < (1ull << 31);
 }
 template <int R2>
-int launch_boxw_r2(const Run& r, const uint8_t* srcFlags, float* dstW, int n, int C, float denom, size_t sws, size_t dws, int64_t W) {
+int launch_boxw_r2(const Run& r, const uint8_t* srcFlags, float* dstW, int n, int C, float denom, size_t sws, size_t dws, int64_t W, ImgLayout lay) {
     dim3 grid((unsigned)cdiv(C, 64), (unsigned)W);
-    hipLaunchKernelGGL((k_boxw<R2>), grid, dim3(64), 0, r.st, srcFlags, dstW, n, C, box_reciprocal(denom), sws, dws);
-    LAUNCHCHK();
-    return TRI_OK;
-}
-int launch_boxw(const Run& r, const uint8_t* srcFlags, float* dstW, int n, int C, int rad, float denom, size_t sws, size_t dws, int64_t W) {
-#define BOXW_CASE(R2) case R2: return launch_boxw_r2<R2>(r, srcFlags, dstW, n, C, denom, sws, dws, W);
+    hipLaunchKernelGGL((k_boxw<R2>), grid, dim3(64), 0, r.st, srcFlags, dstW, n, C, box_reciprocal(denom), sws, dws, lay.ls, lay.ws);
+    LAUNCHCHK();
+    return TRI_OK;
+}
+int launch_boxw(const Run& r, const uint8_t* srcFlags, float* dstW, int n, int C, int rad, float denom, size_t sws, size_t dws, int64_t W, ImgLayout lay) {
+#define BOXW_CASE(R2) case R2: return launch_boxw_r2<R2>(r, srcFlags, dstW, n, C, denom, sws, dws, W, lay);
 #define BOXW_CASE5(A) BOXW_CASE(A) BOXW_CASE(A + 2) BOXW_CASE(A + 4) BOXW_CASE(A + 6) BOXW_CASE(A + 8)
     switch (2 * rad) {
         BOXW_CASE5(20) BOXW_CASE5(30) BOXW_CASE5(40) BOXW_CASE5(50) BOXW_CASE5(60) BOXW_CASE5(70) BOXW_CASE5(80) BOXW_CASE5(90) BOXW_CASE5(100)
@@ -537,19 +547,19 @@
 
 template <int KS>
 int launch_boxt_ks(const Run& r, const float* srcData, const uint8_t* srcFlags, float* dstW, float* dstO,
-                   int n, int C, int rad, float denom, size_t sws, size_t dws, int64_t W) {
+                   int n, int C, int rad, float denom, size_t sws, size_t dws, int64_t W, ImgLayout lay) {
     const int d = 2 * rad - KS;
     const size_t lds = (size_t)4 * d * 64 * sizeof(float);
     dim3 grid((unsigned)cdiv(C, 64), (unsigned)W);
     HIPCHK(lds_optin_all(160 * 1024, &k_boxt<KS, true, 0>, &k_boxt<KS, true, 1>));
     const bool wk = boxw_usable(rad, n, C);
-    if (wk) { const int rc = launch_boxw(r, srcFlags, dstW, n, C, rad, denom, sws, dws, W); if (rc) return rc; }
+    if (wk) { const int rc = launch_boxw(r, srcFlags, dstW, n, C, rad, denom, sws, dws, W, lay); if (rc) return rc; }
     if (d > 0) {
-        if (!wk) hipLaunchKernelGGL((k_boxt<KS, true, 0>), grid, dim3(64), lds, r.st, srcData, srcFlags, dstW, n, C, rad, denom, sws, dws);
-        hipLaunchKernelGGL((k_boxt<KS, true, 1>), grid, dim3(64), lds, r.st, srcData, srcFlags, dstO, n, C, rad, denom, sws, dws);
+        if (!wk) hipLaunchKernelGGL((k_boxt<KS, true, 0>), grid, dim3(64), lds, r.st, srcData, srcFlags, dstW, n, C, rad, denom, sws, dws, lay.ls, lay.ws);
+        hipLaunchKernelGGL((k_boxt<KS, true, 1>), grid, dim3(64), lds, r.st, srcData, srcFlags, dstO, n, C, rad, denom, sws, dws, lay.ls, lay.ws);
     } else {
-        if (!wk) hipLaunchKernelGGL((k_boxt<KS, false, 0>), grid, dim3(64), 0, r.st, srcData, srcFlags, dstW, n, C, rad, denom, sws, dws);
-        hipLaunchKernelGGL((k_boxt<KS, false, 1>), grid, dim3(64), 0, r.st, srcData, srcFlags, dstO, n, C, rad, denom, sws, dws);
+        if (!wk) hipLaunchKernelGGL((k_boxt<KS, false, 0>), grid, dim3(64), 0, r.st, srcData, srcFlags, dstW, n, C, rad, denom, sws, dws, lay.ls, lay.ws);
+        hipLaunchKernelGGL((k_boxt<KS, false, 1>), grid, dim3(64), 0, r.st, srcData, srcFlags, dstO, n, C, rad, denom, sws, dws, lay.ls, lay.ws);
     }
     LAUNCHCHK();
     return TRI_OK;
@@ -613,13 +623,13 @@
 
 template <int KS, int B = 16>
 int launch_boxq_ks(const Run& r, const float* srcData, const uint8_t* srcFlags, float* dstW, float* dstO,
-                   int n, int C, int rad, float denom, size_t sws, size_t dws, int64_t W) {
+                   int n, int C, int rad, float denom, size_t sws, size_t dws, int64_t W, ImgLayout lay) {
     HIPCHK(lds_optin_all(160 * 1024, &k_boxq<KS, 0, B>, &k_boxq<KS, 1, B>));
     dim3 grid((unsigned)cdiv(C, 64), (unsigned)W);
     const BoxDenom dn = box_reciprocal(denom);
-    if (boxw_usable(rad, n, C)) { const int rc = launch_boxw(r, srcFlags, dstW, n, C, rad, denom, sws, dws, W); if (rc) return rc; }
-    else hipLaunchKernelGGL((k_boxq<KS, 0, B>), grid, dim3(256), boxq_lds_bytes(B), r.st, srcData, srcFlags, dstW, n, C, rad, dn, sws, dws);
-    hipLaunchKernelGGL((k_boxq<KS, 1, B>), grid, dim3(256), boxq_lds_bytes(B), r.st, srcData, srcFlags, dstO, n, C, rad, dn, sws, dws);
+    if (boxw_usable(rad, n, C)) { const int rc = launch_boxw(r, srcFlags, dstW, n, C, rad, denom, sws, dws, W, lay); if (rc) return rc; }
+    else hipLaunchKernelGGL((k_boxq<KS, 0, B>), grid, dim3(256), boxq_lds_bytes(B), r.st, srcData, srcFlags, dstW, n, C, rad, dn, sws, dws, lay.ls, lay.ws);
+    hipLaunchKernelGGL((k_boxq<KS, 1, B>), grid, dim3(256), boxq_lds_bytes(B), r.st, srcData, srcFlags, dstO, n, C, rad, dn, sws, dws, lay.ls, lay.ws);
     LAUNCHCHK();
     return TRI_OK;
 }
@@ -639,13 +649,13 @@
 
 template <int KS>
 int launch_boxq_deep(const Run& r, const float* srcData, const uint8_t* srcFlags, float* dstW, float* dstO,
-                     int n, int C, int rad, float denom, size_t sws, size_t dws, int64_t W) {
+                     int n, int C, int rad, float denom, size_t sws, size_t dws, int64_t W, ImgLayout lay) {
     HIPCHK(lds_optin_all(160 * 1024, &k_boxq_deep<KS, 0>, &k_boxq_deep<KS, 1>));
     dim3 grid((unsigned)cdiv(C, 64), (unsigned)W);
     const BoxDenom dn = box_reciprocal(denom);
-    if (boxw_usable(rad, n, C)) { const int rc = launch_boxw(r, srcFlags, dstW, n, C, rad, denom, sws, dws, W); if (rc) return rc; }
-    else hipLaunchKernelGGL((k_boxq_deep<KS, 0>), grid, dim3(256), boxq_lds_bytes(8, 4), r.st, srcData, srcFlags, dstW, n, C, rad, dn, sws, dws);
-    hipLaunchKernelGGL((k_boxq_deep<KS, 1>), grid, dim3(256), boxq_lds_bytes(8, 4), r.st, srcData, srcFlags, dstO, n, C, rad, dn, sws, dws);
+    if (boxw_usable(rad, n, C)) { const int rc = launch_boxw(r, srcFlags, dstW, n, C, rad, denom, sws, dws, W, lay); if (rc) return rc; }
+    else hipLaunchKernelGGL((k_boxq_deep<KS, 0>), grid, dim3(256), boxq_lds_bytes(8, 4), r.st, srcData, srcFlags, dstW, n, C, rad, dn, sws, dws, lay.ls, lay.ws);
+    hipLaunchKernelGGL((k_boxq_deep<KS, 1>), grid, dim3(256), boxq_lds_bytes(8, 4), r.st, srcData, srcFlags, dstO, n, C, rad, dn, sws, dws, lay.ls, lay.ws);
     LAUNCHCHK();
     return TRI_OK;
 }
@@ -654,38 +664,38 @@
 #endif
 
 int launch_boxq(const Run& r, int ks, const float* srcData, const uint8_t* srcFlags, float* dstW, float* dstO,
-                int n, int C, int rad, float denom, size_t sws, size_t dws, int64_t W) {
+                int n, int C, int rad, float denom, size_t sws, size_t dws, int64_t W, ImgLayout lay) {
     if (BOXQ_DEEP && boxq_pick_ks8(40) > 0) {
-        if (2 * rad >= 88 && 2 * rad < 96) return launch_boxq_deep<80>(r, srcData, srcFlags, dstW, dstO, n, C, rad, denom, sws, dws, W);
-        if (2 * rad >= 104 && 2 * rad < 112) return launch_boxq_deep<96>(r, srcData, srcFlags, dstW, dstO, n, C, rad, denom, sws, dws, W);
+        if (2 * rad >= 88 && 2 * rad < 96) return launch_boxq_deep<80>(r, srcData, srcFlags, dstW, dstO, n, C, rad, denom, sws, dws, W, lay);
+        if (2 * rad >= 104 && 2 * rad < 112) return launch_boxq_deep<96>(r, srcData, srcFlags, dstW, dstO, n, C, rad, denom, sws, dws, W, lay);
     }
     switch (boxq_pick_ks8(rad)) {
-        case 32: return launch_boxq_ks<32, 8>(r, srcData, srcFlags, dstW, dstO, n, C, rad, denom, sws, dws, W);
-        case 40: return launch_boxq_ks<40, 8>(r, srcData, srcFlags, dstW, dstO, n, C, rad, denom, sws, dws, W);
-        case 48: return launch_boxq_ks<48, 8>(r, srcData, srcFlags, dstW, dstO, n, C, rad, denom, sws, dws, W);
-        case 56: return launch_boxq_ks<56, 8>(r, srcData, srcFlags, dstW, dstO, n, C, rad, denom, sws, dws, W);
-        case 64: return launch_boxq_ks<64, 8>(r, srcData, srcFlags, dstW, dstO, n, C, rad, denom, sws, dws, W);
-        case 80: return launch_boxq_ks<80, 8>(r, srcData, srcFlags, dstW, dstO, n, C, rad, denom, sws, dws, W);
+        case 32: return launch_boxq_ks<32, 8>(r, srcData, srcFlags, dstW, dstO, n, C, rad, denom, sws, dws, W, lay);
+        case 40: return launch_boxq_ks<40, 8>(r, srcData, srcFlags, dstW, dstO, n, C, rad, denom, sws, dws, W, lay);
+        case 48: return launch_boxq_ks<48, 8>(r, srcData, srcFlags, dstW, dstO, n, C, rad, denom, sws, dws, W, lay);
+        case 56: return launch_boxq_ks<56, 8>(r, srcData, srcFlags, dstW, dstO, n, C, rad, denom, sws, dws, W, lay);
+        case 64: return launch_boxq_ks<64, 8>(r, srcData, srcFlags, dstW, dstO, n, C, rad, denom, sws, dws, W, lay);
+        case 80: return launch_boxq_ks<80, 8>(r, srcData, srcFlags, dstW, dstO, n, C, rad, denom, sws, dws, W, lay);
     }
     switch (ks) {
-        case 16: return launch_boxq_ks<16>(r, srcData, srcFlags, dstW, dstO, n, C, rad, denom, sws, dws, W);
-        case 32: return launch_boxq_ks<32>(r, srcData, srcFlags, dstW, dstO, n, C, rad, denom, sws, dws, W);
-        case 48: return launch_boxq_ks<48>(r, srcData, srcFlags, dstW, dstO, n, C, rad, denom, sws, dws, W);
-        case 64: return launch_boxq_ks<64>(r, srcData, srcFlags, dstW, dstO, n, C, rad, denom, sws, dws, W);
-        case 80: return launch_boxq_ks<80>(r, srcData, srcFlags, dstW, dstO, n, C, rad, denom, sws, dws, W);
-        case 96: return launch_boxq_ks<96>(r, srcData, srcFlags, dstW, dstO, n, C, rad, denom, sws, dws, W);
+        case 16: return launch_boxq_ks<16>(r, srcData, srcFlags, dstW, dstO, n, C, rad, denom, sws, dws, W, lay);
+        case 32: return launch_boxq_ks<32>(r, srcData, srcFlags, dstW, dstO, n, C, rad, denom, sws, dws, W, lay);
+        case 48: return launch_boxq_ks<48>(r, srcData, srcFlags, dstW, dstO, n, C, rad, denom, sws, dws, W, lay);
+        case 64: return launch_boxq_ks<64>(r, srcData, srcFlags, dstW, dstO, n, C, rad, denom, sws, dws, W, lay);
+        case 80: return launch_boxq_ks<80>(r, srcData, srcFlags, dstW, dstO, n, C, rad, denom, sws, dws, W, lay);
+        case 96: return launch_boxq_ks<96>(r, srcData, srcFlags, dstW, dstO, n, C, rad, denom, sws, dws, W, lay);
     }
     return set_err(TRI_EINVAL, "no stage-pipeline kernel for %d slots", ks);
 }
 
 int launch_boxt(const Run& r, int ks, const float* srcData, const uint8_t* srcFlags, float* dstW, float* dstO,
-                int n, int C, int rad, float denom, size_t sws, size_t dws, int64_t W) {
+                int n, int C, int rad, float denom, size_t sws, size_t dws, int64_t W, ImgLayout lay) {
     switch (ks) {
-        case 16: return launch_boxt_ks<16>(r, srcData, srcFlags, dstW, dstO, n, C, rad, denom, sws, dws, W);
-        case 20: return launch_boxt_ks<20>(r, srcData, srcFlags, dstW, dstO, n, C, rad, denom, sws, dws, W);
-        case 32: return launch_boxt_ks<32>(r, srcData, srcFlags, dstW, dstO, n, C, rad, denom, sws, dws, W);
-        case 64: return launch_boxt_ks<64>(r, srcData, srcFlags, dstW, dstO, n, C, rad, denom, sws, dws, W);
-        case 80: return launch_boxt_ks<80>(r, srcData, srcFlags, dstW, dstO, n, C, rad, denom, sws, dws, W);
+        case 16: return launch_boxt_ks<16>(r, srcData, srcFlags, dstW, dstO, n, C, rad, denom, sws, dws, W, lay);
+        case 20: return launch_boxt_ks<20>(r, srcData, srcFlags, dstW, dstO, n, C, rad, denom, sws, dws, W, lay);
+        case 32: return launch_boxt_ks<32>(r, srcData, srcFlags, dstW, dstO, n, C, rad, denom, sws, dws, W, lay);
+        case 64: return launch_boxt_ks<64>(r, srcData, srcFlags, dstW, dstO, n, C, rad, denom, sws, dws, W, lay);
+        case 80: return launch_boxt_ks<80>(r, srcData, srcFlags, dstW, dstO, n, C, rad, denom, sws, dws, W, lay);
     }
     return set_err(TRI_EINVAL, "no register-ring kernel for %d slots", ks);
 }
@@ -702,9 +712,17 @@
 enum class ColFamily { SpecPipe, SpecRing, StagePipe, RegRing, Lane4, LdsRing, MultiPass };
 thread_local bool g_colfilter_unpadded = false;
 
+static ColFamily colfilter_packed_family(int n, int C, int rad) {
+    if (n % 4 != 0 || (uint64_t)n * (uint64_t)C * 4u >= (1ull << 31)) return ColFamily::MultiPass;
+    if (boxq_pick_ks(rad) > 0 && rad <= 107 && (g_boxq_override == 1 || 2 * rad >= BOXQ_MIN_2R)) return ColFamily::StagePipe;
+    if (boxr_pick_ks_t(rad) > 0) return ColFamily::RegRing;
+    return ColFamily::MultiPass;
+}
+
 int launch_colfilter(const Run& r, ColSrc src, float* bufW, float* bufO, const float* srcData,
                      const uint8_t* srcFlags, float* dstW, float* dstO, int n, int C, int rad,
-                     size_t bws, size_t sws, size_t dws, int64_t W, unsigned flags = 0, float* deferred_denom = nullptr) {
+                     size_t bws, size_t sws, size_t dws, int64_t W, unsigned flags = 0, float* deferred_denom = nullptr,
+                     bool panels_out = false) {
     const bool transposed_out = flags & COL_TRANSPOSED_OUT, weights_are_01 = flags & COL_WEIGHTS_01;
     const float denom = box_denominator(rad);
     const int intw = (weights_are_01 && rad <= 31) ? 1 : 0;
@@ -712,14 +730,13 @@
     if (deferred_denom) *deferred_denom = 0.0f;
     const bool regs_ok = !deferred_denom && !transposed_out && weights_are_01 && (uint64_t)n * (uint64_t)C * 4u < (1ull << 31);
     const bool spectrum = regs_ok && src == ColSrc::ByteFlags && W == 1;
-    const bool packed = regs_ok && src == ColSrc::PackedFlags && n % 4 == 0;
+    const ColFamily pfam = (regs_ok && src == ColSrc::PackedFlags) ? colfilter_packed_family(n, C, rad) : ColFamily::MultiPass;
     ColFamily fam;
     if (spectrum && boxp_pick_block(rad, C) > 0 && rad <= 107 && ((uintptr_t)srcData % 16 == 0) && ((uintptr_t)srcFlags % 4 == 0) &&
         ((uintptr_t)dstW % 16 == 0) && ((uintptr_t)dstO % 16 == 0))
         fam = ColFamily::SpecPipe;
     else if (spectrum && boxr_pick_ks(rad) > 0) fam = ColFamily::SpecRing;
-    else if (packed && boxq_pick_ks(rad) > 0 && rad <= 107 && (g_boxq_override == 1 || 2 * rad >= BOXQ_MIN_2R)) fam = ColFamily::StagePipe;
-    else if (packed && boxr_pick_ks_t(rad) > 0) fam = ColFamily::RegRing;
+    else if (pfam != ColFamily::MultiPass) fam = pfam;
     else if (bt > 0 && colfilter_use_lane4(rad) && !transposed_out && src != ColSrc::ByteFlags) fam = ColFamily::Lane4;
     else {
         if (bt > 0 && colfilter_use_lane4(rad) && src == ColSrc::ByteFlags) {
@@ -730,6 +747,9 @@
     }
     if (fam == ColFamily::MultiPass && g_colfilter_unpadded)
         return set_err(TRI_EUNSUPPORTED, "radius %d takes the in-place multi-pass filter, which needs images padded to n + 4r rows", rad);
+    if (panels_out && (C % 64 != 0 || (fam != ColFamily::StagePipe && fam != ColFamily::RegRing)))
+        return set_err(TRI_EUNSUPPORTED, "panel images: packed register-delay-line sweeps over a multiple of 64 columns only");
+    const ImgLayout lay = panels_out ? img_panels(n) : img_rows(C);
     const bool built = src != ColSrc::Images, divide = !deferred_denom;
     const float *const inW = built ? nullptr : bufW, *const inO = built ? nullptr : bufO;
     const size_t in_ws = built ? 0 : bws;
@@ -740,9 +760,9 @@
         case ColFamily::SpecRing:
             return launch_boxt_spec(r, boxr_pick_ks(rad), srcData, srcFlags, dstW, dstO, n, C, rad, denom);
         case ColFamily::StagePipe:
-            return launch_boxq(r, boxq_pick_ks(rad), srcData, srcFlags, dstW, dstO, n, C, rad, denom, sws, dws, W);
+            return launch_boxq(r, boxq_pick_ks(rad), srcData, srcFlags, dstW, dstO, n, C, rad, denom, sws, dws, W, lay);
         case ColFamily::RegRing:
-            return launch_boxt(r, boxr_pick_ks_t(rad), srcData, srcFlags, dstW, dstO, n, C, rad, denom, sws, dws, W);
+            return launch_boxt(r, boxr_pick_ks_t(rad), srcData, srcFlags, dstW, dstO, n, C, rad, denom, sws, dws, W, lay);
         case ColFamily::Lane4: {
             HIPCHK(lds_optin_all(160 * 1024, &k_colfilter_lane4<0, true>, &k_colfilter_lane4<1, true>, &k_colfilter_lane4<1, false>,
                                  &k_colfilter_lane4<2, false>, &k_colfilter_lane4<2, true>));
@@ -938,7 +958,7 @@
 template <int KS, int MODE>
 int launch_boxf_ks(const Run& r, const float* srcW, const float* srcO, float* dstW, float* dstO, const float* data,
                    int n, int C, int ld, int rad, size_t sws_img, size_t dws, size_t ws_data, int64_t W, uint8_t* nanflag,
-                   float* dstP, size_t pws, bool* wroteP) {
+                   float* dstP, size_t pws, bool* wroteP, bool panels_in) {
     const BoxDenom denom = box_reciprocal(box_denominator(rad));
     const int d = 2 * rad - KS;
     if (!(MODE == 2 && boxf_panel_ok(KS, d > 0))) dstP = nullptr;
@@ -953,7 +973,8 @@
     if constexpr (KS == 32) {
         if (d > 14) { k = &k_boxf<KS, true, MODE, 1>; HIPCHK(lds_optin_all(160 * 1024, k)); }
     }
-    hipLaunchKernelGGL(k, grid, dim3(64), lds, r.st, srcW, gap, dstW, dstO, data, n, C, ld, rad, denom, sws_img, dws, ws_data, nanflag, dstP, pws);
+    hipLaunchKernelGGL(k, grid, dim3(64), lds, r.st, srcW, gap, dstW, dstO, data, n, C, ld, rad, denom, sws_img, dws, ws_data, nanflag, dstP, pws,
+                       panels_in ? 64 : ld, panels_in ? 64 * C : 64);
     LAUNCHCHK();
     return TRI_OK;
 }
@@ -972,12 +993,12 @@
 #endif
 template <int KS, int MODE, int B = 16>
 int launch_boxqf_ks(const Run& r, const float* srcW, unsigned gap, float* dstW, float* dstO, const float* data,
-                    int n, int C, int ld, int rad, size_t sws_img, size_t dws, size_t ws_data, int64_t W, uint8_t* nanflag) {
+                    int n, int C, int ld, int rad, size_t sws_img, size_t dws, size_t ws_data, int64_t W, uint8_t* nanflag, bool panels_in) {
     HIPCHK(lds_optin_all(160 * 1024, &k_boxqf<KS, MODE, B>));
     const BoxDenom denom = box_reciprocal(box_denominator(rad));
     dim3 grid((unsigned)cdiv(C, 64), (unsigned)W);
-    hipLaunchKernelGGL((k_boxqf<KS, MODE, B>), grid, dim3(512), boxqf_lds_bytes(B, boxqf_dbl(KS, B)), r.st, srcW, gap, dstW, dstO, data, n, C, ld, rad,
-                       denom, sws_img, dws, ws_data, nanflag);
+    hipLaunchKernelGGL((k_boxqf<KS, MODE, B>), grid, dim3(512), boxqf_lds_bytes(B, boxqf_dbl(KS, B)), r.st, srcW, gap, dstW, dstO, data, n, C,
+                       panels_in ? 64 : ld, rad, denom, sws_img, dws, ws_data, nanflag, panels_in ? 64 * C : 64);
     LAUNCHCHK();
     return TRI_OK;
 }
@@ -985,7 +1006,9 @@
 template <int MODE>
 int launch_boxf(const Run& r, int ks, const float* srcW, const float* srcO, float* dstW, float* dstO, const float* data,
                 int n, int C, int ld, int rad, size_t sws_img, size_t dws, size_t ws_data, int64_t W, uint8_t* nanflag,
-                float* dstP = nullptr, size_t pws = 0, bool* wroteP = nullptr) {
+                float* dstP = nullptr, size_t pws = 0, bool* wroteP = nullptr, bool panels_in = false) {
+    if (panels_in && (n % 64 != 0 || ld != n))
+        return set_err(TRI_EUNSUPPORTED, "panel images: lines of a multiple of 64 positions, no padding");
     if (MODE != 2 || n % 64 != 0) dstP = nullptr;
     {
         static const bool off = is1(getenv("TRI_FILTER_NO_PIPE_F"));
@@ -999,42 +1022,42 @@
             static const int b8 = [] { const char* e = getenv("TRI_FILTER_PIPE_F_B8"); return e ? atoi(e) : BOXQF_B8_DEFAULT; }();
             if (b8 && g_boxq_b8_override != 0 && 2 * rad >= 16 && 2 * rad < BOXQF_B8_MAX2R) {
                 switch (2 * rad / 8 * 8) {
-                    case 16: return launch_boxqf_ks<16, MODE, 8>(r, srcW, gap, dstW, dstO, data, n, C, ld, rad, sws_img, dws, ws_data, W, nanflag);
-                    case 24: return launch_boxqf_ks<24, MODE, 8>(r, srcW, gap, dstW, dstO, data, n, C, ld, rad, sws_img, dws, ws_data, W, nanflag);
-                    case 32: return launch_boxqf_ks<32, MODE, 8>(r, srcW, gap, dstW, dstO, data, n, C, ld, rad, sws_img, dws, ws_data, W, nanflag);
-                    case 40: return launch_boxqf_ks<40, MODE, 8>(r, srcW, gap, dstW, dstO, data, n, C, ld, rad, sws_img, dws, ws_data, W, nanflag);
-                    case 48: return launch_boxqf_ks<48, MODE, 8>(r, srcW, gap, dstW, dstO, data, n, C, ld, rad, sws_img, dws, ws_data, W, nanflag);
+                    case 16: return launch_boxqf_ks<16, MODE, 8>(r, srcW, gap, dstW, dstO, data, n, C, ld, rad, sws_img, dws, ws_data, W, nanflag, panels_in);
+                    case 24: return launch_boxqf_ks<24, MODE, 8>(r, srcW, gap, dstW, dstO, data, n, C, ld, rad, sws_img, dws, ws_data, W, nanflag, panels_in);
+                    case 32: return launch_boxqf_ks<32, MODE, 8>(r, srcW, gap, dstW, dstO, data, n, C, ld, rad, sws_img, dws, ws_data, W, nanflag, panels_in);
+                    case 40: return launch_boxqf_ks<40, MODE, 8>(r, srcW, gap, dstW, dstO, data, n, C, ld, rad, sws_img, dws, ws_data, W, nanflag, panels_in);
+                    case 48: return launch_boxqf_ks<48, MODE, 8>(r, srcW, gap, dstW, dstO, data, n, C, ld, rad, sws_img, dws, ws_data, W, nanflag, panels_in);
 #if BOXQF_B8_MAX2R > 56
-                    case 56: return launch_boxqf_ks<56, MODE, 8>(r, srcW, gap, dstW, dstO, data, n, C, ld, rad, sws_img, dws, ws_data, W, nanflag);
-                    case 64: return launch_boxqf_ks<64, MODE, 8>(r, srcW, gap, dstW, dstO, data, n, C, ld, rad, sws_img, dws, ws_data, W, nanflag);
+                    case 56: return launch_boxqf_ks<56, MODE, 8>(r, srcW, gap, dstW, dstO, data, n, C, ld, rad, sws_img, dws, ws_data, W, nanflag, panels_in);
+                    case 64: return launch_boxqf_ks<64, MODE, 8>(r, srcW, gap, dstW, dstO, data, n, C, ld, rad, sws_img, dws, ws_data, W, nanflag, panels_in);
 #endif
 #if BOXQF_B8_MAX2R > 72
-                    case 72: return launch_boxqf_ks<72, MODE, 8>(r, srcW, gap, dstW, dstO, data, n, C, ld, rad, sws_img, dws, ws_data, W, nanflag);
+                    case 72: return launch_boxqf_ks<72, MODE, 8>(r, srcW, gap, dstW, dstO, data, n, C, ld, rad, sws_img, dws, ws_data, W, nanflag, panels_in);
                     case 80:
-                        if (MODE == 1) return launch_boxqf_ks<80, 1, 8>(r, srcW, gap, dstW, dstO, data, n, C, ld, rad, sws_img, dws, ws_data, W, nanflag);
+                        if (MODE == 1) return launch_boxqf_ks<80, 1, 8>(r, srcW, gap, dstW, dstO, data, n, C, ld, rad, sws_img, dws, ws_data, W, nanflag, panels_in);
                         break;
 #endif
 #if BOXQF_B8_MAX2R > 88
-                    case 96: return launch_boxqf_ks<96, MODE, 8>(r, srcW, gap, dstW, dstO, data, n, C, ld, rad, sws_img, dws, ws_data, W, nanflag);
+                    case 96: return launch_boxqf_ks<96, MODE, 8>(r, srcW, gap, dstW, dstO, data, n, C, ld, rad, sws_img, dws, ws_data, W, nanflag, panels_in);
 #endif
                 }
             }
             switch (kq) {
-                case 16: return launch_boxqf_ks<16, MODE>(r, srcW, gap, dstW, dstO, data, n, C, ld, rad, sws_img, dws, ws_data, W, nanflag);
-                case 32: return launch_boxqf_ks<32, MODE>(r, srcW, gap, dstW, dstO, data, n, C, ld, rad, sws_img, dws, ws_data, W, nanflag);
-                case 48: return launch_boxqf_ks<48, MODE>(r, srcW, gap, dstW, dstO, data, n, C, ld, rad, sws_img, dws, ws_data, W, nanflag);
-                case 64: return launch_boxqf_ks<64, MODE>(r, srcW, gap, dstW, dstO, data, n, C, ld, rad, sws_img, dws, ws_data, W, nanflag);
-                case 80: return launch_boxqf_ks<80, MODE>(r, srcW, gap, dstW, dstO, data, n, C, ld, rad, sws_img, dws, ws_data, W, nanflag);
-                case 96: return launch_boxqf_ks<96, MODE>(r, srcW, gap, dstW, dstO, data, n, C, ld, rad, sws_img, dws, ws_data, W, nanflag);
+                case 16: return launch_boxqf_ks<16, MODE>(r, srcW, gap, dstW, dstO, data, n, C, ld, rad, sws_img, dws, ws_data, W, nanflag, panels_in);
+                case 32: return launch_boxqf_ks<32, MODE>(r, srcW, gap, dstW, dstO, data, n, C, ld, rad, sws_img, dws, ws_data, W, nanflag, panels_in);
+                case 48: return launch_boxqf_ks<48, MODE>(r, srcW, gap, dstW, dstO, data, n, C, ld, rad, sws_img, dws, ws_data, W, nanflag, panels_in);
+                case 64: return launch_boxqf_ks<64, MODE>(r, srcW, gap, dstW, dstO, data, n, C, ld, rad, sws_img, dws, ws_data, W, nanflag, panels_in);
+                case 80: return launch_boxqf_ks<80, MODE>(r, srcW, gap, dstW, dstO, data, n, C, ld, rad, sws_img, dws, ws_data, W, nanflag, panels_in);
+                case 96: return launch_boxqf_ks<96, MODE>(r, srcW, gap, dstW, dstO, data, n, C, ld, rad, sws_img, dws, ws_data, W, nanflag, panels_in);
             }
         }
     }
     switch (ks) {
-        case 8: return launch_boxf_ks<8, MODE>(r, srcW, srcO, dstW, dstO, data, n, C, ld, rad, sws_img, dws, ws_data, W, nanflag, dstP, pws, wroteP);
-        case 16: return launch_boxf_ks<16, MODE>(r, srcW, srcO, dstW, dstO, data, n, C, ld, rad, sws_img, dws, ws_data, W, nanflag, dstP, pws, wroteP);
-        case 32: return launch_boxf_ks<32, MODE>(r, srcW, srcO, dstW, dstO, data, n, C, ld, rad, sws_img, dws, ws_data, W, nanflag, dstP, pws, wroteP);
-        case 64: return launch_boxf_ks<64, MODE>(r, srcW, srcO, dstW, dstO, data, n, C, ld, rad, sws_img, dws, ws_data, W, nanflag, dstP, pws, wroteP);
-        case 80: return launch_boxf_ks<80, MODE>(r, srcW, srcO, dstW, dstO, data, n, C, ld, rad, sws_img, dws, ws_data, W, nanflag, dstP, pws, wroteP);
+        case 8: return launch_boxf_ks<8, MODE>(r, srcW, srcO, dstW, dstO, data, n, C, ld, rad, sws_img, dws, ws_data, W, nanflag, dstP, pws, wroteP, panels_in);
+        case 16: return launch_boxf_ks<16, MODE>(r, srcW, srcO, dstW, dstO, data, n, C, ld, rad, sws_img, dws, ws_data, W, nanflag, dstP, pws, wroteP, panels_in);
+        case 32: return launch_boxf_ks<32, MODE>(r, srcW, srcO, dstW, dstO, data, n, C, ld, rad, sws_img, dws, ws_data, W, nanflag, dstP, pws, wroteP, panels_in);
+        case 64: return launch_boxf_ks<64, MODE>(r, srcW, srcO, dstW, dstO, data, n, C, ld, rad, sws_img, dws, ws_data, W, nanflag, dstP, pws, wroteP, panels_in);
+        case 80: return launch_boxf_ks<80, MODE>(r, srcW, srcO, dstW, dstO, data, n, C, ld, rad, sws_img, dws, ws_data, W, nanflag, dstP, pws, wroteP, panels_in);
     }
     return set_err(TRI_EINVAL, "no register-ring kernel for %d slots", ks);
 }
@@ -1268,6 +1291,7 @@
     TimeStage time;
     bool time_needs_bytes;
     bool time_defers;
+    bool panels;
     FreqPick freq;
     bool freq_transposes;
     Reject reject;
@@ -1298,6 +1322,8 @@
                                                    : pick_freq_stage(s.r1, Fa, T, (size_t)(r.ws.Ao - r.ws.Aw), !r.ampl_cached || r.data_mask);
     s.freq_transposes = s.time != TimeStage::PrebuiltDirectFT;
     s.time_defers = s.freq.route == FreqStage::Transposed;
+    s.panels = TRI_FILTER_PANELS && Fa % 64 == 0 && s.time == TimeStage::PackedSweep && s.freq.route == FreqStage::FusedRing &&
+               colfilter_packed_family(T, Fa, s.r0) != ColFamily::MultiPass;
 
     static const bool no_tfr = is1(getenv("TRI_FILTER_NO_TF_REJECT"));
     const bool vec4 = pl.vec && wsB % 4 == 0;
@@ -1354,7 +1380,7 @@
             LAUNCHCHK();
             return TRI_OK;
         case TimeStage::PackedSweep:
-            return launch_colfilter(r, ColSrc::PackedFlags, im.Aw, im.Ao, im.dataTF, fl, im.Aw, im.Ao, T, Fa, s.r0, im.wsA, N, im.wsA, W, COL_WEIGHTS_01, defer);
+            return launch_colfilter(r, ColSrc::PackedFlags, im.Aw, im.Ao, im.dataTF, fl, im.Aw, im.Ao, T, Fa, s.r0, im.wsA, N, im.wsA, W, COL_WEIGHTS_01, defer, s.panels);
         case TimeStage::Prebuilt:
         case TimeStage::PrebuiltDirectFT:
             if (N % 4 == 0 && im.wsA % 4 == 0)
@@ -1389,7 +1415,7 @@
             return launch_transpose<float>(r, im.rows, im.Bo, T, Fa, im.ws_rows, wsB, W);
         case FreqStage::FusedRing:
             return launch_boxf<MODE>(r, s.freq.ks, im.Aw, im.Ao, im.Bw, im.Bo, im.dataFT, Fa, T, Fa, r1, wsA, wsB, N, W, nan,
-                                     MODE == 2 ? im.residP : nullptr, MODE == 2 ? N : 0, &st.wrote_panel);
+                                     MODE == 2 ? im.residP : nullptr, MODE == 2 ? N : 0, &st.wrote_panel, s.panels);
         case FreqStage::FusedLds:
             return launch_colfilter_tf<MODE>(r, im.Aw, im.Ao, im.Bw, im.Bo, im.dataFT, Fa, T, Fa, r1, wsA, wsB, N, W, nan);
         case FreqStage::LdsDiv:
```

Result: no change. 3139 Mvis/s, median of 6 (+0.9%).
